# yatisht/usher

Measured on AMD Instinct MI355X. Metric: sample placements/sec on 10M-node MAT; bit-exact parsimony score vs reference, higher is better.
Workload: dtype u16 packed (4-bit allele sets, 4-bit SWAR node counters, 16-bit D/cost); 1 GPU; synthetic random MAT 10000000 nodes / 11429716 mutations / 25000 variable sites, L=29903; 16384 queries per GPU per step; nodes=10000000, queries_per_gpu=16384, queries_total=16384, tile=512, tiles=32, waves_per_tile=2050, query_sets_rotated=4, parallelism=queries sharded x1, MAT replicated, RCCL all-gather of results, rccl_ranks=1, devices_visible=1, seed=1

## Files before the change

include/usher_amd.h:

```cpp
#ifndef USHER_AMD_H
#define USHER_AMD_H

#include <stdint.h>

#ifdef __cplusplus
extern "C" {
#endif

#define UGP_OK               0
#define UGP_ERR_INVALID     -1
#define UGP_ERR_UNSUPPORTED -2
#define UGP_ERR_HIP         -3
#define UGP_ERR_NOMEM       -4

typedef struct ugp_mat ugp_mat;
typedef struct ugp_qset ugp_qset;

typedef struct ugp_tree_desc {
    uint64_t n_nodes;
    const uint32_t *parent;
    const uint64_t *mut_off;
    const int32_t *mut_pos;
    const uint8_t *mut_ref;
    const uint8_t *mut_par;
// ... 62 lines not shown
                   uint8_t *tie_has_unique ,
                   uint32_t *tie_count );

#define UGP_ORDER_BFS 0u
#define UGP_ORDER_DFS 1u
typedef struct ugp_place_opts {
    uint32_t order;
    const uint8_t *node_mask;
    const uint32_t *skip_node;
    const uint32_t *distance;
    int32_t *scores;
} ugp_place_opts;
int ugp_place_batch_ex(ugp_mat *mat, const ugp_queries *q, const ugp_place_opts *opts, ugp_result *out );
int ugp_tied_nodes_ex(ugp_mat *mat, const ugp_queries *q, const ugp_place_opts *opts, uint32_t cap, uint32_t *tie_j,
                      uint8_t *tie_has_unique, uint32_t *tie_count);
typedef struct ugp_ex ugp_ex;
int ugp_ex_prepare(ugp_mat *mat, const ugp_place_opts *opts, ugp_ex **out);
void ugp_ex_destroy(ugp_ex *ex);
int ugp_place_batch_prepared(ugp_mat *mat, const ugp_queries *q, const ugp_ex *ex, const uint32_t *skip_node, ugp_result *out ,
                             int32_t *d_scores );
int ugp_uncertainty_attach(ugp_mat *mat, const ugp_tree_desc *tree);
int ugp_uncertainty(ugp_mat *mat, const uint32_t *nodes , uint64_t n, uint32_t cap, uint32_t *epps, uint32_t *nsize,
                    uint32_t *tie_dfs , uint32_t *tie_count);
int ugp_annotate_attach(ugp_mat *mat, const ugp_tree_desc *tree);
int ugp_clade_alleles(ugp_mat *mat, const uint64_t *clade_off , const uint32_t *nodes , uint64_t n_clades,
                      uint64_t *out_off , uint32_t *out_ent, uint32_t *out_cnt, uint64_t cap, uint64_t *n_out);
int ugp_clade_descendants(ugp_mat *mat, const uint64_t *clade_off, const uint32_t *nodes , uint64_t n_clades,
                          const uint32_t *pair_clade, const uint32_t *pair_node , uint64_t n_pairs, uint32_t *out);
int ugp_annotate_search(ugp_mat *mat, const ugp_queries *q, uint32_t cap, int32_t *best , uint32_t *tie_dfs ,
                        uint32_t *tie_count );
typedef struct ugp_nearest_info {
    uint32_t count;
    uint32_t anc;
    uint32_t last_anc;
    uint32_t cut_dist;
    uint32_t n_at_cut;
} ugp_nearest_info;
int ugp_nearest_attach(ugp_mat *mat, const ugp_tree_desc *tree);
int ugp_nearest_k(ugp_mat *mat, uint64_t n_queries, const uint32_t *nodes , const uint32_t *k, uint32_t out_stride,
                  uint32_t *out_nodes , uint32_t *out_dist ,
                  ugp_nearest_info *info );
int ugp_nearest_k_chunked(ugp_mat *mat, uint64_t n_queries, const uint32_t *nodes, const uint32_t *k, uint32_t out_stride,
                          uint32_t *out_nodes, uint32_t *out_dist, ugp_nearest_info *info, uint32_t chunk_queries);
typedef struct ugp_gt_site {
    int32_t pos;
    uint8_t ref, n_alt;
    uint8_t alt[14];
    uint32_t ac[14];
    uint32_t covered;
} ugp_gt_site;
int ugp_genotypes_attach(ugp_mat *mat, const ugp_tree_desc *tree);
int ugp_genotype_select(ugp_mat *mat, const uint32_t *nodes , uint64_t n, uint32_t *n_cols, uint64_t *n_sites);
int ugp_genotype_columns(ugp_mat *mat, uint32_t *nodes );
int ugp_genotype_sites(ugp_mat *mat, uint64_t lo, uint64_t hi, ugp_gt_site *out );
int ugp_genotype_rows(ugp_mat *mat, uint64_t lo, uint64_t hi, uint8_t *codes );
int ugp_genotype_rows_chunked(ugp_mat *mat, uint64_t lo, uint64_t hi, uint8_t *codes, uint64_t chunk_cells);
int ugp_genotype_rows_time(ugp_mat *mat, uint64_t lo, uint64_t hi, uint32_t reps, double *ms);
typedef struct ugp_sm_mutation {
    int32_t pos;
    uint8_t par, nuc;
    uint8_t pad[2];
    uint32_t count;
} ugp_sm_mutation;
typedef struct ugp_sm_roho {
    uint32_t parent, child;
    uint32_t entry;
    uint32_t child_count;
    uint32_t offspring_with;
    uint32_t median_without;
} ugp_sm_roho;
int ugp_summary_attach(ugp_mat *mat, const ugp_tree_desc *tree);
int ugp_summary_mutations(ugp_mat *mat, ugp_sm_mutation *out, uint64_t cap, uint64_t *n_out);
int ugp_summary_mutations_chunked(ugp_mat *mat, ugp_sm_mutation *out, uint64_t cap, uint64_t *n_out, uint64_t chunk_items);
int ugp_summary_roho(ugp_mat *mat, ugp_sm_roho *out, uint64_t cap, uint64_t *n_out);
int ugp_summary_roho_chunked(ugp_mat *mat, ugp_sm_roho *out, uint64_t cap, uint64_t *n_out, uint64_t chunk_items);
int ugp_summary_clades(ugp_mat *mat, const uint64_t *col_off , const uint32_t *nodes , uint64_t n_cols,
                       uint32_t *incl , uint32_t *excl , uint32_t *leaf_clade );
int ugp_summary_time(ugp_mat *mat, uint32_t reps, double *sort_ms, double *roho_ms);
typedef struct ugp_tr_record {
    uint32_t node;
    uint32_t codon;
    uint8_t before[3], after[3];
    uint8_t pad[2];
    uint32_t ent[3];
} ugp_tr_record;
typedef struct ugp_tr_info {
    uint64_t n_records;
    uint64_t n_nodes;
    uint64_t n_inconsistent, n_duplicate;
    uint32_t first_inconsistent;
    uint32_t first_duplicate;
} ugp_tr_info;
int ugp_translate_attach(ugp_mat *mat, const ugp_tree_desc *tree);
int ugp_translate_codons(ugp_mat *mat, uint64_t n_codons, const int32_t *slot_pos , const uint8_t *slot_init );
int ugp_translate(ugp_mat *mat, ugp_tr_record *out, uint64_t cap, uint64_t *n_out, ugp_tr_info *info);
int ugp_translate_chunked(ugp_mat *mat, ugp_tr_record *out, uint64_t cap, uint64_t *n_out, ugp_tr_info *info, uint64_t chunk_items);
int ugp_translate_time(ugp_mat *mat, uint32_t reps, double *ms);
typedef struct ugp_ripples_opts {
    uint32_t branch_len;
    int32_t min_range, max_range;
    int32_t parsimony_improvement;
    uint32_t num_descendants;
} ugp_ripples_opts;
typedef struct ugp_ripples_event {
    uint64_t branch;
    uint32_t i, j;
    uint32_t donor, acceptor;
    uint32_t donor_count, acceptor_count;
    int32_t donor_score, acceptor_score;
    uint8_t donor_sibling, acceptor_sibling;
    uint8_t pad[6];
} ugp_ripples_event;
int ugp_ripples_attach(ugp_mat *mat, const ugp_tree_desc *tree, const uint32_t *name_rank);
int ugp_ripples(ugp_mat *mat, const ugp_ripples_opts *opts, const uint32_t *branches , uint64_t n, ugp_ripples_event *out,
                uint64_t cap, uint64_t *n_out);
int ugp_node_order(ugp_mat *mat, uint32_t order, uint32_t *bfs_of );
int ugp_subtree_mask(ugp_mat *mat, uint32_t order, uint32_t root_j, uint32_t max_levels, uint8_t *mask_out );

int ugp_qset_upload(ugp_mat *mat, const ugp_queries *q, ugp_qset **out);
void ugp_qset_destroy(ugp_qset *qs);
uint64_t ugp_qset_size(const ugp_qset *qs);
int ugp_place_device(ugp_mat *mat, ugp_qset *qs, void *d_out, void *stream);
int ugp_place_device_overlapped(ugp_mat *mat, ugp_qset *qs, void *d_out, void *stream);
int ugp_pipeline_depth(const ugp_mat *mat);

typedef struct ugp_job ugp_job;
int ugp_place_batch_async(ugp_mat *mat, const ugp_queries *q, ugp_result *out , ugp_job **job);
int ugp_job_wait(ugp_job *job);

#define UGP_T_LEAF   1u
#define UGP_T_MASKED 2u
typedef struct ugp_touched {
    uint64_t n;
    const uint32_t *flat_j;
    const uint8_t *flags;
    const uint32_t *n_path;
    const uint64_t *ent_off;
    const int32_t *pos;
    const uint8_t *allele;
    const uint8_t *prev;
    const uint8_t *ref;
} ugp_touched;
int ugp_mat_update(ugp_mat *mat, const ugp_touched *recs, const uint32_t *retired, uint64_t n_retired, uint32_t *first_id);
int ugp_touched_open(ugp_mat *mat, const ugp_queries *batch);
int ugp_touched_score(ugp_mat *mat, uint32_t first_id, uint64_t first_sample);
int ugp_touched_rescore(ugp_mat *mat, uint64_t sample);
int ugp_touched_fetch(ugp_mat *mat, uint64_t first_sample, uint64_t n, uint32_t cap, int32_t *best, uint32_t *count, uint32_t *ids,
                      uint8_t *has_unique);

int ugp_get_timing(ugp_mat *mat, ugp_timing *out);
int ugp_get_timing_sum(ugp_mat *mat, ugp_timing *sum, uint32_t *n_calls);

int ugp_debug_bound3_tables(ugp_mat *mat, uint32_t tile, uint16_t *over, uint16_t *under, uint64_t cap, uint64_t *n_blocks);

const char *ugp_last_error(void);

typedef struct ugp_sites {
    uint64_t n_sites;
    const uint8_t *ref;
    const uint64_t *var_off;
    const uint32_t *var_node;
    const uint8_t *var_nuc;
} ugp_sites;
typedef struct ugp_fitch ugp_fitch;

int ugp_fitch_sankoff(int device, uint64_t n_nodes, const uint32_t *parent, const ugp_sites *sites, ugp_fitch **out);
uint64_t ugp_fitch_count(const ugp_fitch *f);
int ugp_fitch_get(const ugp_fitch *f, uint32_t *site, uint32_t *node, uint8_t *par_nuc , uint8_t *mut_nuc );
void ugp_fitch_destroy(ugp_fitch *f);
void ugp_fitch_release(int device);


int ugp_mat_reload_knobs(ugp_mat *mat);
int ugp_has_experiments(void);

int ugp_mat_create_chunked(const ugp_tree_desc *tree, int device, uint32_t chunk_nodes, ugp_mat **out);

typedef struct ugp_flat ugp_flat;
enum {
    UGP_FLAT_STREAM = 0,
    UGP_FLAT_PRE_STREAM = 1,
    UGP_FLAT_CHUNK_BODY_OFF = 2,
    UGP_FLAT_CHUNK_PRE_OFF = 3,
    UGP_FLAT_CHUNK_NODE_OFF = 4,
    UGP_FLAT_POS2SITE = 5,
    UGP_FLAT_SITE_REF = 6,
    UGP_FLAT_RANK2BFS = 7,
    UGP_FLAT_DFS2BFS = 8,
    UGP_FLAT_MAX_SLOTS = 9,
    UGP_FLAT_STREAM8 = 10,
    UGP_FLAT_PRE8_STREAM = 11,
    UGP_FLAT_CHUNK8_BODY_OFF = 12,
    UGP_FLAT_CHUNK8_PRE_OFF = 13,
    UGP_FLAT_MAX_PATH_MUTS = 14,
    UGP_FLAT_STREAM_T = 15,
    UGP_FLAT_CHUNK_T_OFF = 16,
    UGP_FLAT_LDS_SLOTS = 17,
    UGP_FLAT_B3_GROUP_OFF = 18,
    UGP_FLAT_B3_EVENTS = 19
};
int ugp_flat_create(const ugp_tree_desc *tree, uint32_t chunk_nodes, ugp_flat **out);
void ugp_flat_destroy(ugp_flat *flat);
int ugp_flat_get(const ugp_flat *flat, int which, const void **ptr, uint64_t *count);

#ifdef __cplusplus
}
#endif
#endif
```

usher_amd/_lib.py:

```python
from __future__ import annotations

import ctypes as C
import os
import subprocess

_HERE = os.path.dirname(os.path.abspath(__file__))
LIB_PATH = os.path.join(_HERE, "libusher_amd.so")
EXP_LIB_PATH = os.path.join(_HERE, "libusher_amd_exp.so")
_lib = None
_lib_exp = None


class ugp_tree_desc(C.Structure):
    _fields_ = [("n_nodes", C.c_uint64), ("parent", C.c_void_p), ("mut_off", C.c_void_p), ("mut_pos", C.c_void_p),
                ("mut_ref", C.c_void_p), ("mut_par", C.c_void_p), ("mut_nuc", C.c_void_p)]


class ugp_ripples_opts(C.Structure):
    _fields_ = [("branch_len", C.c_uint32), ("min_range", C.c_int32), ("max_range", C.c_int32),
                ("parsimony_improvement", C.c_int32), ("num_descendants", C.c_uint32)]


class ugp_queries(C.Structure):
    _fields_ = [("n_queries", C.c_uint64), ("ent_off", C.c_void_p), ("pos", C.c_void_p), ("ref", C.c_void_p),
                ("nuc", C.c_void_p), ("is_missing", C.c_void_p)]


class ugp_result(C.Structure):
    _fields_ = [("best_set_difference", C.c_int32), ("num_best", C.c_uint32), ("best_j", C.c_uint32),
                ("best_has_unique", C.c_uint32)]


class ugp_info(C.Structure):
    _fields_ = [("n_nodes", C.c_uint64), ("n_muts", C.c_uint64), ("n_sites", C.c_uint64), ("stream_bytes", C.c_uint64),
                ("algo_tree_bytes", C.c_uint64), ("algo_tile_bytes", C.c_uint64), ("n_chunks", C.c_uint32),
                ("max_slots", C.c_uint32), ("max_position", C.c_uint32), ("device", C.c_uint32)]


class ugp_timing(C.Structure):
    _fields_ = [("table_ms", C.c_float), ("place_ms", C.c_float), ("merge_ms", C.c_float),
                ("place_launches", C.c_uint32), ("n_tiles", C.c_uint32), ("n_groups", C.c_uint32), ("packed_path", C.c_uint32),
                ("reserved", C.c_uint32), ("words_total", C.c_uint64), ("words_skipped", C.c_uint64), ("coarse_ms", C.c_float), ("bound3", C.c_uint32)]


class ugp_place_opts(C.Structure):
    _fields_ = [("order", C.c_uint32), ("node_mask", C.c_void_p), ("skip_node", C.c_void_p), ("distance", C.c_void_p), ("scores", C.c_void_p)]


class ugp_touched(C.Structure):
    _fields_ = [("n", C.c_uint64), ("flat_j", C.c_void_p), ("flags", C.c_void_p), ("n_path", C.c_void_p), ("ent_off", C.c_void_p), ("pos", C.c_void_p),
                ("allele", C.c_void_p), ("prev", C.c_void_p), ("ref", C.c_void_p)]


class ugp_sites(C.Structure):
    _fields_ = [("n_sites", C.c_uint64), ("ref", C.c_void_p), ("var_off", C.c_void_p), ("var_node", C.c_void_p),
                ("var_nuc", C.c_void_p)]


P = C.c_void_p
SYMBOLS = {
    "ugp_mat_create": (C.c_int, [C.POINTER(ugp_tree_desc), C.c_int, C.POINTER(P)]),
    "ugp_mat_create_multi": (C.c_int, [C.POINTER(ugp_tree_desc), C.POINTER(C.c_int), C.c_int, C.POINTER(P)]),
    "ugp_flat_save": (C.c_int, [C.POINTER(ugp_tree_desc), C.c_char_p]),
    "ugp_mat_create_from_flat": (C.c_int, [C.c_char_p, C.c_int, C.POINTER(P)]),
    "ugp_mat_destroy": (None, [P]),
    "ugp_mat_info": (C.c_int, [P, C.POINTER(ugp_info)]),
    "ugp_place_batch": (C.c_int, [P, C.POINTER(ugp_queries), P]),
    "ugp_scores_per_node": (C.c_int, [P, C.POINTER(ugp_queries), P]),
    "ugp_tied_nodes": (C.c_int, [P, C.POINTER(ugp_queries), C.c_uint32, P, P, P]),
    "ugp_place_batch_ex": (C.c_int, [P, C.POINTER(ugp_queries), C.POINTER(ugp_place_opts), P]),
    "ugp_tied_nodes_ex": (C.c_int, [P, C.POINTER(ugp_queries), C.POINTER(ugp_place_opts), C.c_uint32, P, P, P]),
    "ugp_ex_prepare": (C.c_int, [P, C.POINTER(ugp_place_opts), C.POINTER(P)]),
    "ugp_ex_destroy": (None, [P]),
    "ugp_place_batch_prepared": (C.c_int, [P, C.POINTER(ugp_queries), P, P, P, P]),
    "ugp_device_warmup": (C.c_int, [C.c_int]),
    "ugp_node_order": (C.c_int, [P, C.c_uint32, P]),
    "ugp_uncertainty_attach": (C.c_int, [P, C.POINTER(ugp_tree_desc)]),
    "ugp_uncertainty": (C.c_int, [P, P, C.c_uint64, C.c_uint32, P, P, P, P]),
    "ugp_annotate_attach": (C.c_int, [P, C.POINTER(ugp_tree_desc)]),
    "ugp_clade_alleles": (C.c_int, [P, P, P, C.c_uint64, P, P, P, C.c_uint64, C.POINTER(C.c_uint64)]),
    "ugp_clade_descendants": (C.c_int, [P, P, P, C.c_uint64, P, P, C.c_uint64, P]),
    "ugp_annotate_search": (C.c_int, [P, C.POINTER(ugp_queries), C.c_uint32, P, P, P]),
    "ugp_nearest_attach": (C.c_int, [P, C.POINTER(ugp_tree_desc)]),
    "ugp_nearest_k": (C.c_int, [P, C.c_uint64, P, P, C.c_uint32, P, P, P]),
    "ugp_nearest_k_chunked": (C.c_int, [P, C.c_uint64, P, P, C.c_uint32, P, P, P, C.c_uint32]),
    "ugp_genotypes_attach": (C.c_int, [P, C.POINTER(ugp_tree_desc)]),
    "ugp_genotype_select": (C.c_int, [P, P, C.c_uint64, P, P]),
    "ugp_genotype_columns": (C.c_int, [P, P]),
    "ugp_genotype_sites": (C.c_int, [P, C.c_uint64, C.c_uint64, P]),
    "ugp_genotype_rows": (C.c_int, [P, C.c_uint64, C.c_uint64, P]),
    "ugp_genotype_rows_chunked": (C.c_int, [P, C.c_uint64, C.c_uint64, P, C.c_uint64]),
    "ugp_genotype_rows_time": (C.c_int, [P, C.c_uint64, C.c_uint64, C.c_uint32, P]),
    "ugp_summary_attach": (C.c_int, [P, C.POINTER(ugp_tree_desc)]),
    "ugp_summary_mutations": (C.c_int, [P, P, C.c_uint64, C.POINTER(C.c_uint64)]),
    "ugp_summary_mutations_chunked": (C.c_int, [P, P, C.c_uint64, C.POINTER(C.c_uint64), C.c_uint64]),
    "ugp_summary_roho": (C.c_int, [P, P, C.c_uint64, C.POINTER(C.c_uint64)]),
    "ugp_summary_roho_chunked": (C.c_int, [P, P, C.c_uint64, C.POINTER(C.c_uint64), C.c_uint64]),
    "ugp_summary_clades": (C.c_int, [P, P, P, C.c_uint64, P, P, P]),
    "ugp_summary_time": (C.c_int, [P, C.c_uint32, P, P]),
    "ugp_translate_attach": (C.c_int, [P, C.POINTER(ugp_tree_desc)]),
    "ugp_translate_codons": (C.c_int, [P, C.c_uint64, P, P]),
    "ugp_translate": (C.c_int, [P, P, C.c_uint64, C.POINTER(C.c_uint64), P]),
    "ugp_translate_chunked": (C.c_int, [P, P, C.c_uint64, C.POINTER(C.c_uint64), P, C.c_uint64]),
    "ugp_translate_time": (C.c_int, [P, C.c_uint32, P]),
    "ugp_ripples_attach": (C.c_int, [P, C.POINTER(ugp_tree_desc), P]),
    "ugp_ripples": (C.c_int, [P, C.POINTER(ugp_ripples_opts), P, C.c_uint64, P, C.c_uint64, C.POINTER(C.c_uint64)]),
    "ugp_subtree_mask": (C.c_int, [P, C.c_uint32, C.c_uint32, C.c_uint32, P]),
    "ugp_qset_upload": (C.c_int, [P, C.POINTER(ugp_queries), C.POINTER(P)]),
    "ugp_qset_destroy": (None, [P]),
    "ugp_qset_size": (C.c_uint64, [P]),
    "ugp_place_device": (C.c_int, [P, P, P, P]),
    "ugp_place_device_overlapped": (C.c_int, [P, P, P, P]),
    "ugp_pipeline_depth": (C.c_int, [P]),
    "ugp_mat_update": (C.c_int, [P, C.POINTER(ugp_touched), P, C.c_uint64, C.POINTER(C.c_uint32)]),
    "ugp_touched_open": (C.c_int, [P, C.POINTER(ugp_queries)]),
    "ugp_touched_score": (C.c_int, [P, C.c_uint32, C.c_uint64]),
    "ugp_touched_rescore": (C.c_int, [P, C.c_uint64]),
    "ugp_touched_fetch": (C.c_int, [P, C.c_uint64, C.c_uint64, C.c_uint32, P, P, P, P]),
    "ugp_mat_reload_knobs": (C.c_int, [P]),
    "ugp_has_experiments": (C.c_int, []),
    "ugp_place_batch_async": (C.c_int, [P, C.POINTER(ugp_queries), P, C.POINTER(P)]),
    "ugp_job_wait": (C.c_int, [P]),
    "ugp_get_timing": (C.c_int, [P, C.POINTER(ugp_timing)]),
    "ugp_get_timing_sum": (C.c_int, [P, C.POINTER(ugp_timing), C.POINTER(C.c_uint32)]),
    "ugp_debug_bound3_tables": (C.c_int, [P, C.c_uint32, P, P, C.c_uint64, C.POINTER(C.c_uint64)]),
    "ugp_last_error": (C.c_char_p, []),
    "ugp_fitch_sankoff": (C.c_int, [C.c_int, C.c_uint64, P, C.POINTER(ugp_sites), C.POINTER(P)]),
    "ugp_fitch_count": (C.c_uint64, [P]),
    "ugp_fitch_get": (C.c_int, [P, P, P, P, P]),
    "ugp_fitch_destroy": (None, [P]),
    "ugp_fitch_release": (None, [C.c_int]),
    "ugp_mat_create_chunked": (C.c_int, [C.POINTER(ugp_tree_desc), C.c_int, C.c_uint32, C.POINTER(P)]),
    "ugp_flat_create": (C.c_int, [C.POINTER(ugp_tree_desc), C.c_uint32, C.POINTER(P)]),
    "ugp_flat_destroy": (None, [P]),
    "ugp_flat_get": (C.c_int, [P, C.c_int, C.POINTER(P), C.POINTER(C.c_uint64)]),
}


def build_library(force: bool = False) -> str:
    csrc = os.path.join(_HERE, "csrc")
    cmd = ["make", "-s", "-C", csrc]
    if force:
        cmd.append("-B")
    subprocess.check_call(cmd)
    return LIB_PATH


def _load(path):
    if not os.path.exists(path):
        raise RuntimeError(
            "%s is not built (%s); run `python -c 'import __graft_entry__ as g; g.build()'` "
            "or `make -C usher_amd/csrc`. There is no CPU fallback." % (os.path.basename(path), path))
    L = C.CDLL(path)
    for name, (res, args) in SYMBOLS.items():
        fn = getattr(L, name)
        fn.restype = res
        fn.argtypes = args
    return L


def lib(experiments: bool = False):
    global _lib, _lib_exp
    if experiments:
        if _lib_exp is None:
            _lib_exp = _load(EXP_LIB_PATH)
        return _lib_exp
    if _lib is None:
        _lib = _load(os.environ.get("USHER_AMD_LIB") or LIB_PATH)
    return _lib
```

usher_amd/csrc/ugp_capi.cpp:

```cpp
#include <hip/hip_runtime.h>

#include <algorithm>
#include <atomic>
#include <climits>
#include <chrono>
#include <cstdio>
#include <cstdlib>
#include <cstring>
#include <new>
#include <string>
#include <thread>
#include <mutex>
#include <vector>

#include <unistd.h>

#include "ugp_bound3.hpp"
#include "ugp_dense.hpp"
#include "ugp_tuner.hpp"
#include "ugp_plan.hpp"
#include "ugp_flatten.hpp"
#include "ugp_kernels.hpp"
#include "ugp_knobs.hpp"
#include "ugp_ripples.hpp"
#include "ugp_uncertainty.hpp"
#include "ugp_annotate.hpp"
#include "ugp_nearest.hpp"
#include "ugp_genotypes.hpp"
#include "ugp_summary.hpp"
#include "ugp_translate.hpp"
#include "ugp_update.hpp"
#include "usher_amd.h"

namespace {

thread_local std::string g_err;

int fail(int code, const std::string &msg) {
    g_err = msg;
    return code;
}

#define HIP_TRY(expr)                                                                         \
    do {                                                                                      \
        hipError_t e_ = (expr);                                                               \
        if (e_ != hipSuccess)                                                                 \
            return fail(UGP_ERR_HIP, std::string(#expr) + ": " + hipGetErrorString(e_));      \
    } while (0)

}

namespace ugp {
int set_error(int code, const std::string &msg) { return fail(code, msg); }
}

namespace {

template <typename T>
struct DevBuf {
    T *p = nullptr;
    size_t cap = 0;
    ~DevBuf() { release(); }
    void release() {
        if (p) (void)hipFree(p);
        p = nullptr; cap = 0;
    }
    hipError_t reserve(size_t n) {
        if (n <= cap) return hipSuccess;
        release();
        hipError_t e = hipMalloc((void **)&p, std::max<size_t>(n, 1) * sizeof(T));
        if (e == hipSuccess) cap = n; else p = nullptr;
        return e;
    }
    hipError_t grow_keep(size_t n, size_t used) {
        if (n <= cap) return hipSuccess;
        const size_t want = std::max<size_t>(n, cap * 2);
        T *np = nullptr;
        hipError_t e = hipMalloc((void **)&np, std::max<size_t>(want, 1) * sizeof(T));
        if (e != hipSuccess) return e;
        if (p && used) e = hipMemcpy(np, p, used * sizeof(T), hipMemcpyDeviceToDevice);
        if (e != hipSuccess) { (void)hipFree(np); return e; }
        if (p) (void)hipFree(p);
        p = np; cap = want;
        return hipSuccess;
    }
    template <class V>
    hipError_t upload(const V &v) {
        hipError_t e = reserve(v.size());
        if (e != hipSuccess || v.empty()) return e;
        return hipMemcpy(p, v.data(), v.size() * sizeof(T), hipMemcpyHostToDevice);
    }
};

struct PinBuf {
    void *p = nullptr;
    size_t cap = 0;
    ~PinBuf() { if (p) (void)hipHostFree(p); }
    int reserve(size_t n, bool device_writes = false) {
        if (n <= cap) return UGP_OK;
        if (p) (void)hipHostFree(p);
        p = nullptr; cap = 0;
        if (hipHostMalloc(&p, std::max<size_t>(n, 1), device_writes ? (hipHostMallocMapped | hipHostMallocCoherent) : hipHostMallocDefault) != hipSuccess) { p = nullptr; return fail(UGP_ERR_HIP, "hipHostMalloc (staging buffer)"); }
        cap = n;
        return UGP_OK;
    }
};

int copy_d2h_staged(void *dst, const void *src, size_t bytes) {
    constexpr size_t kPiece = 32u << 20;
    if (bytes < 4 * kPiece) {
        if (bytes && hipMemcpy(dst, src, bytes, hipMemcpyDeviceToHost) != hipSuccess) return fail(UGP_ERR_HIP, "copy to the host");
        return UGP_OK;
    }
    PinBuf pin[2];
    hipStream_t st = nullptr;
    hipEvent_t ev[2] = {nullptr, nullptr};
    int rc = UGP_OK;
    if (pin[0].reserve(kPiece) != UGP_OK || pin[1].reserve(kPiece) != UGP_OK) return UGP_ERR_HIP;
    if (hipStreamCreateWithFlags(&st, hipStreamNonBlocking) != hipSuccess || hipEventCreateWithFlags(&ev[0], hipEventDisableTiming) != hipSuccess ||
        hipEventCreateWithFlags(&ev[1], hipEventDisableTiming) != hipSuccess) rc = fail(UGP_ERR_HIP, "staged copy: stream / events");
    const size_t n_pieces = (bytes + kPiece - 1) / kPiece;
    const unsigned n_thr = std::max(1u, std::min(8u, std::thread::hardware_concurrency() / 2));
    auto drain = [&](size_t i) {
        const size_t off = i * kPiece, n = std::min(kPiece, bytes - off);
        const char *from = (const char *)pin[i & 1].p;
        char *to = (char *)dst + off;
        std::vector<std::thread> th;
        const size_t per = ((n + n_thr - 1) / n_thr + 4095) & ~(size_t)4095;
        for (unsigned t = 1; t < n_thr; t++)
            if ((size_t)t * per < n) th.emplace_back([=]() { memcpy(to + (size_t)t * per, from + (size_t)t * per, std::min(per, n - (size_t)t * per)); });
        memcpy(to, from, std::min(per, n));
        for (auto &x : th) x.join();
    };
    for (size_t i = 0; i <= n_pieces && rc == UGP_OK; i++) {
        if (i < n_pieces) {
            const size_t off = i * kPiece, n = std::min(kPiece, bytes - off);
            if (hipMemcpyAsync(pin[i & 1].p, (const char *)src + off, n, hipMemcpyDeviceToHost, st) != hipSuccess || hipEventRecord(ev[i & 1], st) != hipSuccess)
                rc = fail(UGP_ERR_HIP, "staged copy: hipMemcpyAsync");
        }
        if (i > 0 && rc == UGP_OK) {
            if (hipEventSynchronize(ev[(i - 1) & 1]) != hipSuccess) rc = fail(UGP_ERR_HIP, "staged copy: wait");
            else drain(i - 1);
        }
    }
    if (st) { (void)hipStreamSynchronize(st); (void)hipStreamDestroy(st); }
    for (auto e : ev) if (e) (void)hipEventDestroy(e);
    return rc;
}

struct EventSet {
    hipEvent_t ev[4] = {nullptr, nullptr, nullptr, nullptr};
    bool used = false;
    int b3_class = -1;
    bool b3_used = false;
    uint32_t b3_tiles = 0, b3_pos = 0;
    bool b3_first = false;
    uint64_t b3_seq = 0;
};

using ugp::B3Tuner;

using ugp::kMaxSets;

}

struct ugp_mat {
    int device = 0;
    ugp::Knobs knobs;
    ugp::FlatMat flat;
    uint64_t stream_dwords = 0, pre_dwords = 0;
    DevBuf<uint32_t> d_stream, d_pre, d_chunk_body, d_chunk_pre, d_chunk_node, d_rank2bfs, d_dfs2bfs;
    DevBuf<uint32_t> d_stream8, d_pre8, d_chunk8_body, d_chunk8_pre, d_stream_t, d_chunk_t;
    DevBuf<uint32_t> d_node_pos8, d_rank_dfs;
    DevBuf<uint32_t> d_b3_group_off, d_b3_events;
    uint64_t stream8_dwords = 0;
    DevBuf<int32_t> d_pos2site, d_site_pos;
    DevBuf<uint8_t> d_site_ref;
    ugp_mat *coarse = nullptr;
    DevBuf<uint32_t> d_coarse2bfs, d_node_pair, d_parent;
    bool wide_descent = false;
    DevBuf<uint32_t> d_coarse2dfs, d_coarse_bin;
    uint32_t n_coarse_bins = 0;
    std::vector<uint32_t> h_level_off;
    uint32_t max_level_width = 0;
    std::vector<uint32_t> h_parent, h_dfs2bfs, h_bfs2dfs, h_leaves;
    std::vector<uint32_t> h_flat_chunk_node;
    std::vector<uint32_t> h_flat_bfs2dfs;
    DevBuf<uint32_t> d_dfs2bfs_caller;
    DevBuf<uint32_t> d_dfs_rank, d_dfs_rank2out, d_bfs2dfs;
    bool dfs_rank_ready = false;
    ugp_qset *own_qs = nullptr;
    DevBuf<ugp_result> d_own_out;
    size_t occ_lds = ~(size_t)0;
    int occ_per_cu = 0, n_cu = 0, occ_variant = -1;
    struct Work {
        DevBuf<uint32_t> d_table, d_zero, d_part_best, d_part_cnt, d_part_key;
        DevBuf<uint32_t> d_lpos;
        DevBuf<uint32_t> d_tie_units, d_tie_info;
        DevBuf<uint32_t> d_lbest, d_gbest, d_gbest_part, d_items, d_ub, d_gstart, d_hlen, d_cold, d_list, d_units, d_unit_info;
        DevBuf<uint64_t> d_dyn;
        uint32_t dyn_epoch = 0;
        DevBuf<uint32_t> d_b3_pairmask;
        DevBuf<uint8_t> d_b3_over, d_b3_under, d_b3_l1, d_b3_l2, d_b3_l3;
        DevBuf<ugp::B3Dev> d_b3_dev;
        ugp::B3Dev b3_host = {};
        DevBuf<uint64_t> d_stats, d_trace;
        uint64_t last_words_total = 0;
        const uint32_t *last_nitems = nullptr;
        const uint32_t *last_list_n = nullptr;
        uint32_t last_list_tiles = 0;
        DevBuf<uint32_t> d_dnode, d_dres, d_luniq, d_gcnt, d_gcnt_part;
        DevBuf<uint32_t> d_refined, d_keys, d_keys2, d_idx, d_order, d_slot, d_bins;
        DevBuf<ugp_result> d_coarse_res, d_prev_res;
        uint64_t prev_serial = 0;
        DevBuf<uint8_t> d_sort_tmp;
        bool last_used_best8 = false;
        struct Gen {
            std::vector<EventSet> events;
            hipEvent_t ev_coarse[2] = {nullptr, nullptr};
            bool coarse_timed = false;
            size_t events_used = 0;
            ugp_timing last = {};
            bool timing_pending = false;
        } gens[4];
        uint32_t cur = 0;
        ugp_qset *job_qs = nullptr;
        DevBuf<ugp_result> d_job_out;
        PinBuf job_in, job_out;
        bool job_busy = false;
        hipStream_t aux = nullptr;
        hipEvent_t ev_fork = nullptr, ev_fill = nullptr, ev_join = nullptr;
        bool join_pending = false;
        hipStream_t stream = nullptr;
        hipEvent_t done = nullptr;
        hipStream_t done_on = nullptr;
    } work[kMaxSets];
    ugp_timing tsum = {};
    uint32_t tsum_calls = 0;
    int last_work = 0;
    B3Tuner b3_tuner;
    int next_work = 0;
    int next_job = 0;
    uint64_t n_overlapped = 0;
    hipEvent_t entry_ring[kMaxSets] = {};
    int share_sets = 2;
    int share_n = 1;
    uint32_t tie_lists_filled = 0, tie_sub_batches = 0;
    bool sharing = false;
    bool was_busy = false;
    int was_n = 1;
    struct Upd {
        std::vector<uint32_t> hdr8, rec, post, coarse2bfs, excluded_j;
        DevBuf<uint32_t> d_hdr8, d_rec_pos, d_post;
        DevBuf<ugp::TouchedRec> d_rec;
        DevBuf<ugp::TouchedEnt> d_ent;
        DevBuf<uint8_t> d_alive;
        DevBuf<uint32_t> d_tmp;
        uint64_t n_rec = 0, n_ent = 0, n_excluded = 0;
        ugp_qset *qs = nullptr;
        DevBuf<uint8_t> d_dense, d_hu;
        DevBuf<int32_t> d_dbot, d_best, d_list_best;
        DevBuf<uint32_t> d_cnt, d_ids;
        uint32_t n_pos = 0, qpad = 0;
        uint64_t Q = 0;
        bool open = false;
        PinBuf stage_up;
        PinBuf stage;
    } upd;
    ugp::UncState *unc = nullptr;
    ugp::RipState *rip = nullptr;
    ugp::AnnState *ann = nullptr;
    ugp::NearState *near = nullptr;
    ugp::GtState *gt = nullptr;
    ugp::SmState *sm = nullptr;
    ugp::TrState *tr = nullptr;
    ugp::DfsTables *dfs = nullptr;
    hipEvent_t kb_done = nullptr;
    hipStream_t kb_done_on = nullptr;
};

struct ugp_qset {
    int device = 0;
    uint64_t n_queries = 0, n_ent = 0;
    uint64_t max_rows = 0;
    uint64_t serial = 0;
    DevBuf<int32_t> d_pos;
    DevBuf<uint8_t> d_ref, d_nuc, d_missing;
    DevBuf<uint32_t> d_ent_q;
    DevBuf<uint64_t> d_ent_off;
    DevBuf<unsigned long long> d_err;
    DevBuf<uint32_t> d_nmask[2], d_plain_rows, d_n_plain;
    const ugp_mat *nmask_for[2] = {nullptr, nullptr};
    uint32_t nmask_words[2] = {0, 0};
    std::vector<uint64_t> ent_off;
};

namespace ugp { void fitch_drop_streams(int device); }
namespace {

int validate_offsets(const ugp_queries *q, uint64_t &n_ent, uint64_t &max_rows) {
    if (!q || (q->n_queries && !q->ent_off)) return fail(UGP_ERR_INVALID, "null query arrays");
    if (q->n_queries >= (1ull << 31)) return fail(UGP_ERR_UNSUPPORTED, "more than 2^31 queries in one batch");
    n_ent = q->n_queries ? q->ent_off[q->n_queries] : 0;
    if (n_ent && (!q->pos || !q->ref || !q->nuc || !q->is_missing)) return fail(UGP_ERR_INVALID, "null query entry arrays");
    max_rows = 0;
    for (uint64_t s = 0; s < q->n_queries; s++) {
        const uint64_t b = q->ent_off[s], e = q->ent_off[s + 1];
        if (e < b || e > n_ent) return fail(UGP_ERR_INVALID, "ent_off is not monotone");
        max_rows = std::max(max_rows, e - b);
    }
    if (q->n_queries && q->ent_off[0] != 0) return fail(UGP_ERR_INVALID, "ent_off[0] must be 0");
    return UGP_OK;
}

}
static int harvest_timing(ugp_mat *m, ugp_mat::Work &W, ugp_mat::Work::Gen &G);
static void tuner_poll(ugp_mat *m);
namespace {
int ensure_events(ugp_mat::Work::Gen &G, size_t n) {
    while (G.events.size() < n) {
        EventSet es;
        for (int i = 0; i < 4; i++) HIP_TRY(hipEventCreate(&es.ev[i]));
        G.events.push_back(es);
    }
    return UGP_OK;
}

struct ExDev {
    const uint8_t *mask = nullptr; const uint32_t *skip = nullptr, *alt_rank = nullptr, *out_index = nullptr, *rank2out = nullptr;
    const uint32_t *skip_chunk = nullptr;
    int32_t *scores = nullptr;
    bool packed = false;
};

struct PlaceReq {
    int mode = 0;
    ugp_result *out = nullptr;
    int32_t *scores = nullptr;
    const int32_t *best_in = nullptr;
    uint32_t *tie_count = nullptr, *tie_j = nullptr;
    uint8_t *tie_hu = nullptr;
    uint32_t tie_cap = 0;
    hipStream_t stream = nullptr;
    bool coarse_only = false;
    const ExDev *ex = nullptr;
    int wi = 0;
};

struct Finish {
    ugp_mat::Work &W; hipStream_t s;
    ~Finish() {
        if (W.join_pending) { (void)hipStreamWaitEvent(s, W.ev_join, 0); W.join_pending = false; }
        if (!W.done && hipEventCreateWithFlags(&W.done, hipEventDisableTiming) != hipSuccess) { W.done = nullptr; return; }
        (void)hipEventRecord(W.done, s);
        W.done_on = s;
    }
};

struct PlaceCall {
    ugp_mat *m; ugp_qset *qs; const PlaceReq &r;
    ugp_mat::Work &W;
    hipStream_t s;
    ugp_mat::Work::Gen *TG;
    ugp::PlanTree tree;
    ugp::PlanCall call;
    ugp::CallPlan cp;
    const uint32_t *ex_skip;
};

struct SubBatch {
    uint64_t q0 = 0, nq = 0, e0 = 0, e1 = 0;
    ugp::SubPlan p;
    ugp::ZeroLayout z;
    uint64_t table_dwords = 0, pairs = 0;
    EventSet *es = nullptr;
    uint32_t *d_dbottom = nullptr, *d_active = nullptr, *d_queue = nullptr, *d_list_n = nullptr, *d_nitems = nullptr, *d_cnt = nullptr, *d_key = nullptr,
             *d_useful = nullptr;
    const uint32_t *slot_of = nullptr, *order = nullptr;
    ugp::Phase2Uniq uq{};
    ugp::PlaceArgs a;
    ugp::Best8Args b8;
    uint32_t blocks = 0;
};

int nmask_index(const ugp_qset *qs, const ugp_mat *m) {
    int nmi = -1;
    for (int i = 0; i < 2; i++) if (qs->nmask_for[i] == m) nmi = i;
    return nmi;
}

ugp::PlanTree plan_tree(const ugp_mat *m) {
    const auto &f = m->flat;
    ugp::PlanTree t;
    t.n_nodes = f.n_nodes; t.n_sites = f.n_sites; t.n_chunks = f.n_chunks; t.max_chunk8_words = f.max_chunk8_words;
    t.max_path_muts = f.max_path_muts; t.lds_slots = f.lds_slots; t.mask_not_first = f.mask_not_first;
    t.coarse = m->coarse != nullptr; t.b3_events = m->d_b3_events.p != nullptr; t.wide_descent = m->wide_descent;
    return t;
}

ugp::PlanCall plan_call_facts(const ugp_mat *m, const ugp_qset *qs, const PlaceReq &r) {
    ugp::PlanCall c;
    c.Q = qs->n_queries; c.max_rows = qs->max_rows; c.mode = r.mode; c.coarse_only = r.coarse_only; c.ties = r.tie_count != nullptr;
    c.nmask = nmask_index(qs, m) >= 0; c.sharing = m->sharing; c.share_sets = m->share_sets;
    if (const ExDev *ex = r.ex) {
        c.ex.given = true; c.ex.packed = ex->packed; c.ex.mask = ex->mask != nullptr; c.ex.skip = ex->skip != nullptr;
        c.ex.skip_chunk = ex->skip_chunk != nullptr; c.ex.scores = ex->scores != nullptr;
    }
    return c;
}

int run_place(ugp_mat *m, ugp_qset *qs, const PlaceReq &r);

int open_timing(PlaceCall &c) {
    ugp_mat::Work &W = c.W;
    W.cur = (W.cur + 1u) & 3u;
    c.TG = &W.gens[W.cur];
    if (int rc = harvest_timing(c.m, W, *c.TG)) return rc;
    c.TG->events_used = 0;
    c.TG->last = {};
    c.TG->timing_pending = true;
    return UGP_OK;
}

int side_fill(PlaceCall &c) {
    ugp_mat::Work &W = c.W;
    if (!c.cp.can_fork) return UGP_OK;
    if (!W.aux) {
        HIP_TRY(hipStreamCreateWithFlags(&W.aux, hipStreamNonBlocking));
        HIP_TRY(hipEventCreateWithFlags(&W.ev_fork, hipEventDisableTiming)); HIP_TRY(hipEventCreateWithFlags(&W.ev_fill, hipEventDisableTiming));
        HIP_TRY(hipEventCreateWithFlags(&W.ev_join, hipEventDisableTiming));
    }
    if (!c.cp.fill_ahead) return UGP_OK;
    const uint64_t dw = (uint64_t)((c.call.Q + 511) / 512) * (c.cp.n_sites + ugp::TABLE_CONST_ROWS) * 64;
    HIP_TRY(W.d_table.reserve(dw));
    HIP_TRY(hipEventRecord(W.ev_fork, c.s));
    HIP_TRY(hipStreamWaitEvent(W.aux, W.ev_fork, 0));
    HIP_TRY(ugp::launch_fill_table(W.d_table.p, c.m->d_site_ref.p, c.cp.n_sites, dw, W.aux));
    HIP_TRY(hipEventRecord(W.ev_fill, W.aux));
    return UGP_OK;
}

int coarse_pass(PlaceCall &c) {
    ugp_mat *m = c.m;
    ugp_mat::Work &W = c.W;
    ugp_mat::Work::Gen &TG = *c.TG;
    HIP_TRY(W.d_coarse_res.reserve(c.call.Q));
    if (!TG.ev_coarse[0]) { HIP_TRY(hipEventCreate(&TG.ev_coarse[0])); HIP_TRY(hipEventCreate(&TG.ev_coarse[1])); }
    HIP_TRY(hipEventRecord(TG.ev_coarse[0], c.s));
    m->coarse->sharing = m->sharing; m->coarse->share_n = m->share_n; m->coarse->share_sets = m->share_sets;
    PlaceReq cr;
    cr.out = W.d_coarse_res.p; cr.stream = c.s; cr.wi = c.r.wi;
    cr.coarse_only = m->coarse->d_node_pos8.p && m->coarse->flat.max_chunk8_words < 65536u && !m->knobs.coarse_phase2;
    if (int rc = run_place(m->coarse, c.qs, cr)) return rc;
    HIP_TRY(hipSetDevice(m->device));
    HIP_TRY(hipEventRecord(TG.ev_coarse[1], c.s));
    TG.coarse_timed = true;
    return UGP_OK;
}

int sub_begin(PlaceCall &c, SubBatch &sb, uint64_t q0) {
    ugp_mat *m = c.m;
    ugp_mat::Work &W = c.W;
    ugp_mat::Work::Gen &TG = *c.TG;
    const auto &f = m->flat;
    sb.q0 = q0; sb.nq = std::min<uint64_t>(c.call.Q - q0, c.cp.sub_tiles * 64);
    if (c.r.mode == 0 && c.r.tie_count) m->tie_sub_batches++;
    sb.e0 = c.qs->ent_off[q0]; sb.e1 = c.qs->ent_off[q0 + sb.nq];
    sb.p = ugp::plan_sub(c.tree, m->knobs, c.call, c.cp, sb.nq, sb.e1 - sb.e0);
    const uint32_t n_tiles512 = sb.p.n_tiles512;
    sb.table_dwords = (uint64_t)n_tiles512 * (c.cp.n_sites + ugp::TABLE_CONST_ROWS) * 64;
    HIP_TRY(W.d_table.reserve(sb.table_dwords));
    uint32_t b3_pos = 0;
    uint64_t b3_seq = 0;
    if (sb.p.b3_tuned) { tuner_poll(m); sb.p.b3_want = m->b3_tuner.next(sb.p.b3_class, &b3_pos, &b3_seq); }
    sb.pairs = (uint64_t)f.n_chunks * n_tiles512 * 8;
    sb.z = ugp::zero_layout(n_tiles512, c.cp.active_words, c.cp.useful_words, sb.p.b3_want);
    HIP_TRY(W.d_zero.reserve(sb.z.z_end));
    sb.d_dbottom = W.d_zero.p + sb.z.z_dbottom; sb.d_active = W.d_zero.p + sb.z.z_active; sb.d_queue = W.d_zero.p + sb.z.z_queue;
    sb.d_list_n = W.d_zero.p + sb.z.z_list_n; sb.d_nitems = W.d_zero.p + sb.z.z_nitems; sb.d_cnt = W.d_zero.p + sb.z.z_cnt;
    sb.d_key = W.d_zero.p + sb.z.z_key; sb.d_useful = sb.p.b3_want ? W.d_zero.p + sb.z.z_useful : nullptr;
    if (c.cp.packed_ok) {
        HIP_TRY(W.d_lbest.reserve((size_t)f.n_chunks * n_tiles512 * 256));
        HIP_TRY(W.d_list.reserve((size_t)f.n_chunks * n_tiles512));
        HIP_TRY(W.d_ub.reserve((size_t)n_tiles512 * 256));
        if (!c.r.coarse_only) {
            HIP_TRY(W.d_gbest.reserve((size_t)n_tiles512 * 256));
            HIP_TRY(W.d_gbest_part.reserve((size_t)ugp::GBEST_SLICES * n_tiles512 * 256));
            HIP_TRY(W.d_items.reserve(sb.pairs));
        }
    } else if (c.r.mode == 0) {
        const size_t np = (size_t)sb.p.n_tiles * sb.p.G * 64;
        HIP_TRY(W.d_part_best.reserve(np));
        HIP_TRY(W.d_part_cnt.reserve(np));
        HIP_TRY(W.d_part_key.reserve(np));
    }
    if (int rc = ensure_events(TG, TG.events_used + 1)) return rc;
    EventSet &es = TG.events[TG.events_used++];
    sb.es = &es;
    es.b3_class = -1;
    es.b3_used = sb.p.b3_want; es.b3_tiles = n_tiles512; es.b3_pos = b3_pos; es.b3_seq = b3_seq; es.b3_first = m->b3_tuner.first;
    HIP_TRY(hipEventRecord(es.ev[0], c.s));
    return UGP_OK;
}

int locality_sort(PlaceCall &c, SubBatch &sb) {
    ugp_mat *m = c.m;
    ugp_mat::Work &W = c.W;
    const uint64_t nq = sb.nq;
    HIP_TRY(W.d_keys.reserve(nq)); HIP_TRY(W.d_keys2.reserve(nq)); HIP_TRY(W.d_idx.reserve(nq));
    HIP_TRY(W.d_order.reserve(nq)); HIP_TRY(W.d_slot.reserve(nq)); HIP_TRY(W.d_bins.reserve(std::max<uint32_t>(m->n_coarse_bins, 1)));
    size_t tmp_bytes = 0;
    HIP_TRY(ugp::launch_locality_sort(nullptr, nullptr, (uint32_t)nq, W.d_keys.p, W.d_keys2.p, W.d_idx.p, W.d_order.p,
                                      W.d_slot.p, nullptr, &tmp_bytes, nullptr, 0, nullptr, c.s));
    HIP_TRY(W.d_sort_tmp.reserve(tmp_bytes));
    HIP_TRY(ugp::launch_locality_sort(W.d_coarse_res.p + sb.q0, m->d_coarse2dfs.p, (uint32_t)nq, W.d_keys.p, W.d_keys2.p,
                                      W.d_idx.p, W.d_order.p, W.d_slot.p, W.d_sort_tmp.p, &tmp_bytes, m->knobs.radix_sort ? nullptr : m->d_coarse_bin.p, m->n_coarse_bins, W.d_bins.p, c.s));
    sb.slot_of = W.d_slot.p; sb.order = W.d_order.p;
    return UGP_OK;
}

int build_tiles(PlaceCall &c, SubBatch &sb) {
    ugp_mat *m = c.m;
    ugp_qset *qs = c.qs;
    ugp_mat::Work &W = c.W;
    hipStream_t s = c.s;
    const auto &f = m->flat;
    const uint32_t n_sites = c.cp.n_sites, active_words = c.cp.active_words, useful_words = c.cp.useful_words, n_tiles512 = sb.p.n_tiles512;
    const uint32_t q0 = (uint32_t)sb.q0, nq = (uint32_t)sb.nq;
    HIP_TRY(hipMemsetAsync(W.d_zero.p, 0, sb.z.z_end * sizeof(uint32_t), s));
    if (sb.p.nmask) {
        const int nmi = nmask_index(qs, m);
        HIP_TRY(ugp::launch_ntiles(W.d_table.p, sb.d_active, active_words, n_tiles512, qs->d_nmask[nmi].p, qs->nmask_words[nmi], sb.order, q0, nq,
                                   m->d_site_ref.p, n_sites, s));
        HIP_TRY(ugp::launch_scatter_list(W.d_table.p, sb.d_dbottom, qs->d_pos.p, qs->d_ref.p, qs->d_nuc.p, qs->d_missing.p, qs->d_ent_q.p, m->d_pos2site.p,
                                         f.max_pos, n_sites, q0, nq, sb.d_active, active_words, sb.slot_of, qs->d_plain_rows.p, qs->d_n_plain.p, qs->d_err.p,
                                         sb.d_useful, useful_words, s));
    } else if (sb.p.lds_build)
        HIP_TRY(ugp::launch_build_tiles(W.d_table.p, sb.d_active, active_words, n_tiles512, qs->d_ent_off.p, q0, sb.order, nq, qs->d_pos.p,
                                        qs->d_ref.p, qs->d_nuc.p, qs->d_missing.p, m->d_pos2site.p, m->d_site_pos.p, m->d_site_ref.p, n_sites, f.max_pos,
                                        sb.d_dbottom, qs->d_err.p, s));
    else {
        const uint64_t e0 = sb.e0, e1 = sb.e1;
        if (c.cp.fill_ahead && sb.q0 == 0) HIP_TRY(hipStreamWaitEvent(s, W.ev_fill, 0));
        else HIP_TRY(ugp::launch_fill_table(W.d_table.p, m->d_site_ref.p, n_sites, sb.table_dwords, s));
        HIP_TRY(ugp::launch_scatter(W.d_table.p, sb.d_dbottom, qs->d_pos.p + e0, qs->d_ref.p + e0,
                                    qs->d_nuc.p + e0, qs->d_missing.p + e0, qs->d_ent_q.p + e0, m->d_pos2site.p,
                                    f.max_pos, n_sites, e1 - e0, q0, sb.d_active, active_words, sb.slot_of, qs->d_err.p, sb.d_useful, useful_words, s));
    }
    return UGP_OK;
}

int b3_tables(PlaceCall &c, SubBatch &sb) {
    ugp_mat *m = c.m;
    ugp_mat::Work &W = c.W;
    hipStream_t s = c.s;
    const uint32_t n_sites = c.cp.n_sites, n_tiles512 = sb.p.n_tiles512;
    const uint32_t nb = ugp::b3_blocks(m->stream8_dwords), n_l1 = ugp::b3_div64(nb), n_l2 = ugp::b3_div64(n_l1), n_l3 = ugp::b3_div64(n_l2);
    HIP_TRY(W.d_b3_pairmask.reserve((size_t)((n_tiles512 + 31) / 32) * n_sites * 4));
    HIP_TRY(W.d_b3_over.reserve((size_t)n_tiles512 * nb)); HIP_TRY(W.d_b3_under.reserve((size_t)n_tiles512 * nb));
    HIP_TRY(W.d_b3_l1.reserve((size_t)n_tiles512 * n_l1)); HIP_TRY(W.d_b3_l2.reserve((size_t)n_tiles512 * n_l2)); HIP_TRY(W.d_b3_l3.reserve((size_t)n_tiles512 * n_l3));
    HIP_TRY(W.d_b3_dev.reserve(1));
    const ugp::B3Dev hd{W.d_b3_over.p, W.d_b3_under.p, W.d_b3_l1.p, W.d_b3_l2.p, W.d_b3_l3.p, nb, n_l1, n_l2, n_l3};
    if (memcmp(&hd, &W.b3_host, sizeof hd) != 0) {
        HIP_TRY(hipStreamSynchronize(s));
        HIP_TRY(hipMemcpy(W.d_b3_dev.p, &hd, sizeof hd, hipMemcpyHostToDevice));
        W.b3_host = hd;
    }
    hipStream_t on = s;
    if (c.cp.can_fork) {
        HIP_TRY(hipEventRecord(W.ev_fork, s));
        HIP_TRY(hipStreamWaitEvent(W.aux, W.ev_fork, 0));
        on = W.aux;
    }
    HIP_TRY(ugp::launch_b3_tables(sb.d_useful, c.cp.useful_words, n_sites, n_tiles512, m->d_b3_group_off.p, m->d_b3_events.p, nb, W.d_b3_pairmask.p,
                                  W.d_b3_over.p, W.d_b3_under.p, W.d_b3_l1.p, W.d_b3_l2.p, W.d_b3_l3.p, on));
    if (c.cp.can_fork) { HIP_TRY(hipEventRecord(W.ev_join, W.aux)); W.join_pending = true; }
    return UGP_OK;
}

#ifdef UGP_EXPERIMENTS
int seed_check_report(PlaceCall &c, SubBatch &sb) {
    ugp_mat *m = c.m;
    ugp_mat::Work &W = c.W;
    const uint64_t nq = sb.nq, q0 = sb.q0;
    std::vector<uint32_t> ref(nq), ord(nq);
    std::vector<ugp_result> prev(nq), coarse(nq);
    HIP_TRY(hipStreamSynchronize(c.s));
    HIP_TRY(hipMemcpy(ref.data(), W.d_refined.p, nq * 4, hipMemcpyDeviceToHost));
    HIP_TRY(hipMemcpy(ord.data(), sb.order, nq * 4, hipMemcpyDeviceToHost));
    HIP_TRY(hipMemcpy(prev.data(), W.d_prev_res.p + q0, nq * sizeof(ugp_result), hipMemcpyDeviceToHost));
    HIP_TRY(hipMemcpy(coarse.data(), W.d_coarse_res.p + q0, nq * sizeof(ugp_result), hipMemcpyDeviceToHost));
    uint64_t hist_r[18] = {0}, hist_c[18] = {0}, miss_anc = 0, miss_other = 0, miss_depth = 0;
    std::vector<uint32_t> c2b(m->coarse ? m->coarse->flat.n_nodes : 0);
    if (!c2b.empty()) HIP_TRY(hipMemcpy(c2b.data(), m->d_coarse2bfs.p, c2b.size() * 4, hipMemcpyDeviceToHost));
    for (uint64_t k = 0; k < nq; k++) {
        const int exact = prev[ord[k]].best_set_difference;
        hist_r[std::min(17, std::max(0, (int)ref[k] - exact))]++;
        hist_c[std::min(17, std::max(0, coarse[ord[k]].best_set_difference - exact))]++;
        if ((int)ref[k] > exact && !c2b.empty() && coarse[ord[k]].best_j < c2b.size()) {
            const uint32_t j0 = c2b[coarse[ord[k]].best_j];
            uint32_t x = prev[ord[k]].best_j, depth = 0;
            while (x != UINT32_MAX && x != j0 && x != 0) { x = m->h_parent[x]; depth++; }
            if (x == j0) { miss_anc++; miss_depth += depth; } else {
                miss_other++;
                if (miss_other <= 12) {
                    auto depth_of = [&](uint32_t v) { uint32_t d = 0; while (v != 0 && v != UINT32_MAX) { v = m->h_parent[v]; d++; } return d; };
                    uint32_t a = j0, b = prev[ord[k]].best_j;
// ... 116 lines not shown
    }
    b.ub_every = w.ub_every;
    b.freeze_ub = c.ex_skip ? 1u : 0u;
    b.refill_all_rows = K.refill_all ? 1u : 0u;
    b.heavy_prio = K.heavy_prio;
    b.no_pre_records = w.no_pre_records;
    HIP_TRY(W.d_units.reserve((size_t)n_tiles512 * w.per_tile_cap * 4));
    HIP_TRY(W.d_unit_info.reserve(32 + 96));
    constexpr uint32_t kDynCap = 1u << 17;
    if (!W.d_dyn.p) {
        HIP_TRY(W.d_dyn.reserve(kDynCap));
        W.dyn_epoch = 2047;
    }
    if (++W.dyn_epoch >= 2048u) { HIP_TRY(hipMemsetAsync(W.d_dyn.p, 0, (size_t)kDynCap * 8, s)); W.dyn_epoch = 1; }
    uint32_t *dyn_ctl = W.d_unit_info.p + 32;
    b.dyn_ctl = dyn_ctl; b.dyn_units = (unsigned long long *)W.d_dyn.p; b.dyn_cap = kDynCap; b.dyn_epoch = W.dyn_epoch;
    b.split_cycles = w.split_cycles; b.split_heavy = w.split_heavy; b.split_dense = w.split_dense; b.split_many = w.split_many;
    HIP_TRY(ugp::launch_build_units(hstart, hlen, n_tiles512, f.n_chunks, w.unit_chunks, w.heavy_chunks, w.grow_every, w.unit_max, w.light_order, w.per_tile_cap,
                                    W.d_units.p, W.d_unit_info.p, W.d_unit_info.p + 8, dyn_ctl, s));
    b.units = (const uint4 *)W.d_units.p; b.unit_base = W.d_unit_info.p; b.unit_count = W.d_unit_info.p + 8;
    HIP_TRY(W.d_stats.reserve(96));
    if (sb.q0 == 0) { if (K.stats) HIP_TRY(hipMemsetAsync(W.d_stats.p, 0, 96 * sizeof(uint64_t), s)); W.last_words_total = 0; }
    b.stats = K.stats ? W.d_stats.p : nullptr;
    if (b.stats && !K.trace.empty() && !coarse_only) {
        constexpr size_t kTraceCap = 1u << 20;
        HIP_TRY(W.d_trace.reserve(8 + kTraceCap * 6));
        HIP_TRY(hipMemsetAsync(W.d_trace.p, 0, 64, s));
        b.trace = W.d_trace.p; b.trace_cap = kTraceCap;
    }
    W.last_words_total += (uint64_t)n_tiles512 * m->stream8_dwords;
    b.max_slots = f.max_slots;
    b.lds_slots = f.lds_slots;
    b.lds_bits = w.lds_bits;
    b.b3 = w.b3 ? W.d_b3_dev.p : nullptr;
    if (b.b3) c.TG->last.bound3 = 1;
    if (m->occ_lds != w.lds_bytes || m->occ_variant != w.variant) {
        HIP_TRY(hipDeviceGetAttribute(&m->n_cu, hipDeviceAttributeMultiprocessorCount, m->device));
        HIP_TRY(ugp::best8_occupancy(w.lds_bytes, w.variant, &m->occ_per_cu));
        m->occ_lds = w.lds_bytes; m->occ_variant = w.variant;
    }
    const uint64_t blocks = ugp::plan_grid(c.tree, K, c.call, c.cp, sb.p, m->occ_per_cu, m->n_cu).blocks;
    sb.blocks = (uint32_t)blocks;
    HIP_TRY(W.d_cold.reserve((size_t)blocks * std::max<uint32_t>(f.max_slots - b.lds_slots, 1) * 512));
    b.cold = W.d_cold.p;
    b.active = sb.d_active; b.active_words = c.cp.active_words;
    const bool exclusive = K.kbest_exclusive;
    if (exclusive && !coarse_only && m->kb_done && m->kb_done_on != s) HIP_TRY(hipStreamWaitEvent(s, m->kb_done, 0));
    if (W.join_pending) { HIP_TRY(hipStreamWaitEvent(s, W.ev_join, 0)); W.join_pending = false; }
    HIP_TRY(ugp::launch_best8(b, (uint32_t)blocks, s));
    if (exclusive && !coarse_only) {
        if (!m->kb_done) HIP_TRY(hipEventCreateWithFlags(&m->kb_done, hipEventDisableTiming));
        HIP_TRY(hipEventRecord(m->kb_done, s));
        m->kb_done_on = s;
    }
    HIP_TRY(hipEventRecord(sb.es->ev[2], s));
    return UGP_OK;
}

int packed_result(PlaceCall &c, SubBatch &sb) {
    ugp_mat *m = c.m;
    ugp_mat::Work &W = c.W;
    hipStream_t s = c.s;
    const PlaceReq &r = c.r;
    const auto &f = m->flat;
    const uint32_t n_tiles512 = sb.p.n_tiles512;
    const uint64_t q0 = sb.q0, nq = sb.nq;
    if (c.ex_skip && !r.coarse_only)
        HIP_TRY(ugp::launch_fix_skip(sb.a, W.d_lbest.p, r.ex->skip_chunk + q0, n_tiles512, m->d_rank2bfs.p, sb.order, f.max_slots, s));
    if (r.coarse_only)
        HIP_TRY(ugp::launch_coarse_result(W.d_lbest.p, W.d_lpos.p, W.d_list.p, sb.d_list_n, f.n_chunks, n_tiles512, (uint32_t)nq, m->d_chunk_node.p,
                                          m->d_chunk8_body.p, m->d_node_pos8.p, m->d_dfs2bfs.p, r.out + q0, s));
#ifdef UGP_EXPERIMENTS
    else if (!r.tie_count && m->d_node_pos8.p && m->d_rank_dfs.p && sb.b8.ub && !sb.b8.stats && m->knobs.phase2_packed) {
        HIP_TRY(W.d_tie_units.reserve((size_t)((n_tiles512 + 7) / 8) * 8 * f.n_chunks * 4));
        HIP_TRY(W.d_tie_info.reserve(128));
        HIP_TRY(ugp::launch_phase2_packed(sb.b8, W.d_list.p, sb.d_list_n, W.d_gbest_part.p, W.d_gbest.p, n_tiles512, W.d_tie_units.p, W.d_tie_info.p, sb.d_cnt, sb.d_key,
                                          m->d_node_pos8.p, m->d_rank_dfs.p, m->d_chunk_node.p, m->d_rank2bfs.p, (uint32_t)nq, r.out + q0, sb.order,
                                          sb.blocks, s));
    }
#endif
    else
        HIP_TRY(ugp::launch_phase2(sb.a, W.d_lbest.p, W.d_list.p, sb.d_list_n, W.d_gbest_part.p, W.d_gbest.p, n_tiles512, W.d_items.p, sb.d_nitems,
                                   (uint32_t)std::min<uint64_t>(sb.pairs, 0xFFFFFFFFull), sb.d_cnt, sb.d_key,
                                   m->d_rank2bfs.p, r.ex ? r.ex->rank2out : nullptr, r.out + q0, sb.order, f.max_slots, r.tie_count != nullptr,
                                   sb.uq.luniq ? &sb.uq : nullptr, s));
    if (r.tie_count) m->tie_lists_filled++;
    return UGP_OK;
}

int level_scores(PlaceCall &c, SubBatch &sb) {
    ugp_mat *m = c.m;
    ugp_mat::Work &W = c.W;
    const auto &f = m->flat;
    const uint64_t nq = sb.nq;
    const uint32_t qpad = (uint32_t)((nq + 7) / 8 * 8);
    const bool d16 = c.qs->max_rows + f.max_path_muts + 2 < 0xFFFFull;
    const size_t d_words = ((size_t)m->max_level_width * ((qpad + ugp::SCORES_SB - 1) / ugp::SCORES_SB * ugp::SCORES_SB) * (d16 ? 2 : 4) + 3) / 4;
    HIP_TRY(W.d_part_best.reserve(d_words)); HIP_TRY(W.d_part_cnt.reserve(d_words));
    HIP_TRY(ugp::launch_scores_levels(m->d_node_pair.p, m->d_parent.p, m->d_stream.p, W.d_table.p, c.cp.n_sites, sb.d_dbottom, m->h_level_off.data(),
                                      (uint32_t)m->h_level_off.size() - 1, W.d_part_best.p, W.d_part_cnt.p, d16, m->max_level_width, qpad, (uint32_t)nq, f.n_nodes,
                                      sb.a.scores, m->knobs.scores_block, c.s));
    HIP_TRY(hipEventRecord(sb.es->ev[2], c.s));
    return UGP_OK;
}

int lane_walk(PlaceCall &c, SubBatch &sb) {
    ugp_mat *m = c.m;
    ugp_mat::Work &W = c.W;
    const PlaceReq &r = c.r;
    HIP_TRY(ugp::launch_place(sb.a, r.ex ? r.mode + 4 : r.mode, m->flat.max_slots, c.s));
    HIP_TRY(hipEventRecord(sb.es->ev[2], c.s));
    if (r.mode == 0)
        HIP_TRY(ugp::launch_merge(W.d_part_best.p, W.d_part_cnt.p, W.d_part_key.p, (r.ex && r.ex->rank2out) ? r.ex->rank2out : m->d_rank2bfs.p, sb.p.G,
                                  (uint32_t)sb.nq, r.out + sb.q0, c.s));
    return UGP_OK;
}

int sub_end(PlaceCall &c, SubBatch &sb) {
    ugp_mat *m = c.m;
    ugp_mat::Work &W = c.W;
    ugp_mat::Work::Gen &TG = *c.TG;
    const ugp::Knobs &K = m->knobs;
    const bool packed = c.cp.packed_ok;
    if ((K.seed_prev || K.seed_check) && packed && !c.r.coarse_only && c.r.mode == 0) {
        HIP_TRY(W.d_prev_res.reserve(c.call.Q));
        HIP_TRY(hipMemcpyAsync(W.d_prev_res.p + sb.q0, c.r.out + sb.q0, sb.nq * sizeof(ugp_result), hipMemcpyDeviceToDevice, c.s));
        W.prev_serial = (sb.q0 + sb.nq >= c.call.Q) ? c.qs->serial : 0;
    }
    HIP_TRY(hipEventRecord(sb.es->ev[3], c.s));
    if (sb.p.b3_tuned) sb.es->b3_class = sb.p.b3_class;
    W.last_used_best8 = packed;
    TG.last.packed_path = packed ? 1u : 0u;
    sb.es->used = true;
    TG.last.place_launches++;
    TG.last.n_tiles += packed ? sb.p.n_tiles512 : sb.p.n_tiles;
    TG.last.n_groups = sb.p.G;
    return UGP_OK;
}

int run_place(ugp_mat *m, ugp_qset *qs, const PlaceReq &r) {
    HIP_TRY(hipSetDevice(m->device));
    hipStream_t s = r.stream;
    PlaceCall c{m, qs, r, m->work[r.wi], s, nullptr, {}, {}, {}, nullptr};
    m->last_work = r.wi;
    if (c.W.done && c.W.done_on != s) HIP_TRY(hipStreamWaitEvent(s, c.W.done, 0));
    Finish finish{c.W, s};
    if (int rc = open_timing(c)) return rc;
    if (qs->n_queries == 0) return UGP_OK;
    c.tree = plan_tree(m);
    c.call = plan_call_facts(m, qs, r);
    c.cp = ugp::plan_call(c.tree, m->knobs, c.call);
    c.ex_skip = c.cp.ex_skip ? r.ex->skip : nullptr;
    c.TG->coarse_timed = false;
    if (int rc = side_fill(c)) return rc;
    if (c.cp.sorted) if (int rc = coarse_pass(c)) return rc;
    for (uint64_t q0 = 0; q0 < c.call.Q; q0 += c.cp.sub_tiles * 64) {
        SubBatch sb;
        if (int rc = sub_begin(c, sb, q0)) return rc;
        if (c.cp.sorted) if (int rc = locality_sort(c, sb)) return rc;
        if (int rc = build_tiles(c, sb)) return rc;
        if (sb.p.b3_want) if (int rc = b3_tables(c, sb)) return rc;
        if (c.cp.packed_ok) if (int rc = seed_bounds(c, sb)) return rc;
        HIP_TRY(hipEventRecord(sb.es->ev[1], s));
        place_args(c, sb);
        if (c.cp.packed_ok) {
            if (int rc = packed_walk(c, sb)) return rc;
            if (int rc = packed_result(c, sb)) return rc;
        } else if (r.mode == 1 && !r.ex && !m->h_level_off.empty() && !m->knobs.scores_dfs) {
            if (int rc = level_scores(c, sb)) return rc;
        } else if (int rc = lane_walk(c, sb)) return rc;
        if (int rc = sub_end(c, sb)) return rc;
    }
    return UGP_OK;
}

}

extern "C" {

const char *ugp_last_error(void) { return g_err.c_str(); }

int ugp_device_warmup(int device) {
    HIP_TRY(hipSetDevice(device));
    HIP_TRY(hipFree(nullptr));
    return UGP_OK;
}

struct HostFlat {
    ugp::FlatMat f;
    std::vector<uint32_t> parent;
    std::vector<uint32_t> coarse2dfs, coarse2bfs;
    ugp::UVec<uint32_t> node_pair;
    bool wide_descent = false;
    HostFlat *coarse = nullptr;
    ~HostFlat() { delete coarse; }
};

static int host_flatten(const ugp_tree_desc *tree, const ugp::Options &opt, bool with_coarse, HostFlat &hf);

static int build_coarse(const ugp_tree_desc *t, const ugp::Options &opt, ugp::FlatExtras &ex, HostFlat &hf) {
    const uint64_t N = t->n_nodes;
    uint64_t min_nodes = 1u << 18;
    if (const char *e = getenv("UGP_COARSE_MIN_NODES")) min_nodes = (uint64_t)atoll(e);
    if (N < min_nodes || N < 64 || getenv("UGP_NO_SORT")) return UGP_OK;
    const uint32_t *sub = ex.sub.data();
    uint64_t div = 4096;
    if (const char *e = getenv("UGP_COARSE_DIV")) div = (uint64_t)std::max(2, atoi(e));
    uint64_t floor_n = 4096;
    if (const char *e = getenv("UGP_COARSE_FLOOR")) floor_n = (uint64_t)std::max(16, atoi(e));
    const uint64_t target = std::min<uint64_t>(N / 2, std::max<uint64_t>(N / div, std::min<uint64_t>(floor_n, N / 4)));
    uint32_t S = 0;
    {
        constexpr uint32_t CAP = 1u << 16;
        const ugp::Par par = ugp::flatten_par(opt);
        std::vector<uint64_t> hist((size_t)par.T * (CAP + 1), 0);
        par.run(N, [&](uint64_t b, uint64_t e, unsigned tid) {
            uint64_t *h = &hist[(size_t)tid * (CAP + 1)];
            for (uint64_t j = b; j < e; j++) h[std::min<uint32_t>(sub[j], CAP)]++;
        }, 1u << 16);
        uint64_t below = 0;
        uint32_t v = 0;
        for (; v < CAP; v++) {
            uint64_t c = 0;
            for (unsigned th = 0; th < par.T; th++) c += hist[(size_t)th * (CAP + 1) + v];
            if (below + c > N - target) break;
            below += c;
        }
        if (v < CAP) S = v;
        else {
            std::vector<uint32_t> sorted_sub(sub, sub + N);
            std::nth_element(sorted_sub.begin(), sorted_sub.begin() + (N - target), sorted_sub.end());
            S = sorted_sub[N - target];
        }
        S = std::max<uint32_t>(2, S);
    }
    std::vector<uint32_t> keep;
    for (uint64_t j = 0; j < N; j++) if (sub[j] >= S || j == 0) keep.push_back((uint32_t)j);
    std::vector<uint32_t> parent(keep.size());
    std::vector<uint64_t> mut_off(keep.size() + 1, 0);
    std::vector<int32_t> pos; std::vector<uint8_t> ref, par, nuc;
    for (size_t k = 0; k < keep.size(); k++) {
        const uint32_t j = keep[k];
        parent[k] = j ? (uint32_t)(std::lower_bound(keep.begin(), keep.begin() + k, t->parent[j]) - keep.begin()) : UINT32_MAX;
        for (uint64_t i = t->mut_off[j]; i < t->mut_off[j + 1]; i++) {
            pos.push_back(t->mut_pos[i]); ref.push_back(t->mut_ref[i]);
            par.push_back(t->mut_par ? t->mut_par[i] : 0); nuc.push_back(t->mut_nuc[i]);
        }
        mut_off[k + 1] = pos.size();
    }
    ugp_tree_desc d{keep.size(), parent.data(), mut_off.data(), pos.data(), ref.data(), par.data(), nuc.data()};
    ugp::Options copt;
    copt.chunk_nodes = 256;
    copt.keep_node_pos8 = true;
    copt.keep_update_maps = opt.keep_update_maps;
    copt.keep_b3_events = false;
    if (const char *e = getenv("UGP_LDS_SLOTS")) copt.lds_slots = (uint32_t)std::max(1, std::min(60, atoi(e)));
    if (const char *e = getenv("UGP_COARSE_CHUNK_NODES")) copt.chunk_nodes = (uint32_t)std::max(1, atoi(e));
    hf.coarse = new HostFlat();
    if (int rc = host_flatten(&d, copt, false, *hf.coarse)) return rc;
    hf.coarse2dfs.resize(keep.size());
    for (size_t k = 0; k < keep.size(); k++) hf.coarse2dfs[k] = ex.dfsidx[keep[k]];
    hf.coarse2bfs = keep;
    return UGP_OK;
}

static int host_flatten(const ugp_tree_desc *tree, const ugp::Options &opt, bool with_coarse, HostFlat &hf) {
    std::string err;
    int rc;
    try {
        ugp::FlatExtras ex;
        rc = ugp::flatten(*tree, opt, hf.f, err, with_coarse ? &ex : nullptr);
        if (rc == UGP_OK && with_coarse) hf.parent.assign(tree->parent, tree->parent + tree->n_nodes);
        if (rc == UGP_OK && with_coarse) {
            rc = build_coarse(tree, opt, ex, hf);
            if (rc != UGP_OK) return rc;
            hf.node_pair.swap(ex.node_pair);
            if (hf.coarse) hf.wide_descent = ex.children_of_wide_nodes * 20 > tree->n_nodes;
        }
    } catch (const std::bad_alloc &) {
        return fail(UGP_ERR_NOMEM, "out of host memory while flattening the tree");
    }
    if (rc != UGP_OK) return fail(rc, err);
    return UGP_OK;
}

static int upload_flat(const HostFlat &hf, int device, ugp_mat **out) {
    *out = nullptr;
    ugp_mat *m = new (std::nothrow) ugp_mat();
    if (!m) return fail(UGP_ERR_NOMEM, "out of host memory");
    m->device = device;
    m->knobs = ugp::Knobs::from_env();
    auto bail = [&](hipError_t e, const char *what) {
        std::string msg = std::string(what) + ": " + hipGetErrorString(e);
        ugp_mat_destroy(m);
        return fail(UGP_ERR_HIP, msg);
    };
    hipError_t e;
    if ((e = hipSetDevice(device)) != hipSuccess) return bail(e, "hipSetDevice");
    const auto &f = hf.f;
    {
        auto &g = m->flat;
        g.n_nodes = f.n_nodes; g.n_muts = f.n_muts; g.n_sites = f.n_sites; g.max_pos = f.max_pos; g.max_slots = f.max_slots;
        g.n_chunks = f.n_chunks; g.max_path_muts = f.max_path_muts; g.max_chunk8_words = f.max_chunk8_words; g.mask_not_first = f.mask_not_first; g.lds_slots = f.lds_slots;
    }
    m->upd.hdr8.assign(f.hdr8_of_bfs.begin(), f.hdr8_of_bfs.end());
    m->upd.rec.assign(f.rec_of_bfs.begin(), f.rec_of_bfs.end());
    m->upd.post.assign(f.post_of_bfs.begin(), f.post_of_bfs.end());
    m->upd.coarse2bfs = hf.coarse2bfs;
    if ((e = m->d_stream.upload(f.stream)) != hipSuccess) return bail(e, "upload stream");
    if ((e = m->d_pre.upload(f.pre_stream)) != hipSuccess) return bail(e, "upload preambles");
    if ((e = m->d_chunk_body.upload(f.chunk_body_off)) != hipSuccess) return bail(e, "upload chunk table");
    if ((e = m->d_chunk_pre.upload(f.chunk_pre_off)) != hipSuccess) return bail(e, "upload chunk table");
    if ((e = m->d_chunk_node.upload(f.chunk_node_off)) != hipSuccess) return bail(e, "upload chunk table");
    if ((e = m->d_rank2bfs.upload(f.rank2bfs)) != hipSuccess) return bail(e, "upload rank table");
    if ((e = m->d_dfs2bfs.upload(f.dfs2bfs)) != hipSuccess) return bail(e, "upload dfs table");
    if ((e = m->d_pos2site.upload(f.pos2site)) != hipSuccess) return bail(e, "upload site table");
    {
        std::vector<int32_t> sp(std::max<size_t>(f.n_sites, 1), 0);
        for (size_t p = 0; p < f.pos2site.size(); p++) if (f.pos2site[p] >= 0) sp[(size_t)f.pos2site[p]] = (int32_t)p;
        if ((e = m->d_site_pos.upload(sp)) != hipSuccess) return bail(e, "upload site table");
    }
    {
        std::vector<uint8_t> sr(f.site_ref);
        if (sr.empty()) sr.push_back(1);
        if ((e = m->d_site_ref.upload(sr)) != hipSuccess) return bail(e, "upload site table");
    }
    if ((e = m->d_stream8.upload(f.stream8)) != hipSuccess) return bail(e, "upload packed stream");
    if ((e = m->d_pre8.upload(f.pre8_stream)) != hipSuccess) return bail(e, "upload packed preambles");
    if ((e = m->d_chunk8_body.upload(f.chunk8_body_off)) != hipSuccess) return bail(e, "upload chunk table");
    if ((e = m->d_chunk8_pre.upload(f.chunk8_pre_off)) != hipSuccess) return bail(e, "upload chunk table");
    if ((e = m->d_stream_t.upload(f.stream_t)) != hipSuccess) return bail(e, "upload tie stream");
    if ((e = m->d_chunk_t.upload(f.chunk_t_off)) != hipSuccess) return bail(e, "upload chunk table");
    if (!f.node_pos8.empty() && (e = m->d_node_pos8.upload(f.node_pos8)) != hipSuccess) return bail(e, "upload node positions");
    if (!f.rank_dfs.empty() && (e = m->d_rank_dfs.upload(f.rank_dfs)) != hipSuccess) return bail(e, "upload node ranks");
    if (!f.b3_events.empty()) {
        if ((e = m->d_b3_group_off.upload(f.b3_group_off)) != hipSuccess) return bail(e, "upload event lists");
        if ((e = m->d_b3_events.upload(f.b3_events)) != hipSuccess) return bail(e, "upload event lists");
    }
    m->stream8_dwords = f.stream8.size();
    m->stream_dwords = f.stream.size();
    m->pre_dwords = f.pre_stream.size();
    m->h_parent = hf.parent;
    if (!hf.node_pair.empty()) {
        if ((e = m->d_node_pair.upload(hf.node_pair)) != hipSuccess) return bail(e, "upload node table");
        if ((e = m->d_parent.upload(hf.parent)) != hipSuccess) return bail(e, "upload parent table");
        const uint64_t N = f.n_nodes;
        std::vector<uint32_t> level(N, 0);
        m->h_level_off.assign(1, 0);
        for (uint64_t j = 1; j < N; j++) {
            level[j] = level[hf.parent[j]] + 1;
            if (level[j] != level[j - 1]) m->h_level_off.push_back((uint32_t)j);
        }
        m->h_level_off.push_back((uint32_t)N);
        m->max_level_width = 0;
        for (size_t l = 0; l + 1 < m->h_level_off.size(); l++) m->max_level_width = std::max(m->max_level_width, m->h_level_off[l + 1] - m->h_level_off[l]);
    }
    if (hf.coarse) {
        if (int rc = upload_flat(*hf.coarse, device, &m->coarse)) { ugp_mat_destroy(m); return rc; }
        if ((e = m->d_coarse2dfs.upload(hf.coarse2dfs)) != hipSuccess) return bail(e, "upload coarse table");
        {
            std::vector<uint32_t> by_rank(hf.coarse2dfs.size()), bin(hf.coarse2dfs.size());
            for (uint32_t i = 0; i < by_rank.size(); i++) by_rank[i] = i;
            std::sort(by_rank.begin(), by_rank.end(), [&](uint32_t a, uint32_t b) { return hf.coarse2dfs[a] < hf.coarse2dfs[b]; });
            for (uint32_t i = 0; i < by_rank.size(); i++) bin[by_rank[i]] = i;
            if ((e = m->d_coarse_bin.upload(bin)) != hipSuccess) return bail(e, "upload coarse table");
            m->n_coarse_bins = (uint32_t)bin.size();
        }
        if ((e = m->d_coarse2bfs.upload(hf.coarse2bfs)) != hipSuccess) return bail(e, "upload coarse table");
        if (!hf.node_pair.empty()) {
            m->wide_descent = getenv("UGP_DESCENT_LANES") ? atoi(getenv("UGP_DESCENT_LANES")) > 16 : hf.wide_descent;
        }
    }
    *out = m;
    return UGP_OK;
}

static ugp::Options default_options() {
    ugp::Options opt;
    opt.keep_update_maps = !getenv("UGP_NO_UPDATE_MAPS");
    if (const char *e = getenv("UGP_CHUNK_NODES")) opt.chunk_nodes = (uint32_t)std::max(1, atoi(e));
    if (const char *e = getenv("UGP_PRUNE_MIN_WORDS")) opt.prune_min_words = (uint32_t)std::max(1, atoi(e));
    if (getenv("UGP_NO_SIB")) opt.sibling_records = false;
#ifdef UGP_EXPERIMENTS
    opt.keep_node_pos8 = getenv("UGP_PHASE2_PACKED") != nullptr;
#endif
    if (getenv("UGP_NO_BOUND2")) opt.second_bound = false;
    opt.keep_b3_events = !getenv("UGP_NO_BOUND3");
    if (const char *e = getenv("UGP_LDS_SLOTS")) opt.lds_slots = (uint32_t)std::max(1, std::min(60, atoi(e)));
    if (const char *e = getenv("UGP_PRE_WEIGHT")) opt.pre_weight = (uint32_t)std::max(0, atoi(e));
    return opt;
}

static int mat_create_impl(const ugp_tree_desc *tree, int device, const ugp::Options &opt, ugp_mat **out) {
    if (!tree || !out) return fail(UGP_ERR_INVALID, "null argument");
    *out = nullptr;
    HostFlat hf;
    const bool verbose = getenv("UGP_FLATTEN_VERBOSE") != nullptr;
    const auto t0 = std::chrono::steady_clock::now();
    if (int rc = host_flatten(tree, opt, true, hf)) return rc;
    const auto t1 = std::chrono::steady_clock::now();
    const int rc = upload_flat(hf, device, out);
    if (verbose)
        fprintf(stderr, "[ugp mat_create] flatten + coarse MAT %.1f ms, upload %.1f ms\n", std::chrono::duration<double, std::milli>(t1 - t0).count(),
                std::chrono::duration<double, std::milli>(std::chrono::steady_clock::now() - t1).count());
    return rc;
}

int ugp_mat_create_multi(const ugp_tree_desc *tree, const int *devices, int n_devices, ugp_mat **out) {
    if (!tree || !devices || !out || n_devices < 1) return fail(UGP_ERR_INVALID, "null argument");
    for (int i = 0; i < n_devices; i++) out[i] = nullptr;
    HostFlat hf;
    if (int rc = host_flatten(tree, default_options(), true, hf)) return rc;
    for (int i = 0; i < n_devices; i++) {
        if (int rc = upload_flat(hf, devices[i], &out[i])) {
            const std::string msg = g_err;
            for (int k = 0; k < i; k++) { ugp_mat_destroy(out[k]); out[k] = nullptr; }
            return fail(rc, msg);
        }
    }
    return UGP_OK;
}

int ugp_mat_create(const ugp_tree_desc *tree, int device, ugp_mat **out) {
    return mat_create_impl(tree, device, default_options(), out);
}

}
namespace {
constexpr uint64_t kFlatMagic = 0x3154414C46504755ull;
uint64_t flat_signature() {
    uint64_t h = 1469598103934665603ull;
    auto mix = [&](const char *p) { for (; p && *p; p++) { h ^= (uint8_t)*p; h *= 1099511628211ull; } h ^= 0xFF; h *= 1099511628211ull; };
    mix(__DATE__ " " __TIME__);
    const uint64_t fmt[] = {ugp::FLAT_FORMAT_VERSION, ugp::B3_BLOCK_SHIFT, ugp::B3_GROUP_SHIFT, ugp::T_PRUNE_MIN_DWORDS, ugp::PRUNE_MIN_WORDS, ugp::LDS_SLOTS, ugp::MAX_HOT_SLOTS,
                            ugp::INFO_JUMP_MASK, sizeof(ugp::FlatMat), sizeof(HostFlat), sizeof(ugp_result)};
    for (uint64_t v : fmt) { h ^= v; h *= 1099511628211ull; }
    for (const char *k : {"UGP_CHUNK_NODES", "UGP_PRUNE_MIN_WORDS", "UGP_NO_SIB", "UGP_NO_BOUND2", "UGP_LDS_SLOTS", "UGP_PRE_WEIGHT", "UGP_NO_UPDATE_MAPS",
                          "UGP_COARSE_MIN_NODES", "UGP_NO_SORT", "UGP_COARSE_DIV", "UGP_COARSE_FLOOR", "UGP_COARSE_CHUNK_NODES", "UGP_NO_BOUND3"}) { mix(k); mix(getenv(k)); }
    return h;
}
struct FlatWriter {
    FILE *f; bool ok = true;
    void raw(const void *p, size_t n) { if (ok && n && fwrite(p, 1, n, f) != n) ok = false; }
    template <class T> void pod(const T &v) { raw(&v, sizeof v); }
    template <class V> void vec(const V &v) { const uint64_t n = v.size(); pod(n); raw(v.data(), n * sizeof(typename V::value_type)); }
};
struct FlatReader {
    const uint8_t *p, *e; bool ok = true;
    void raw(void *d, size_t n) { if (!ok || (size_t)(e - p) < n) { ok = false; return; } memcpy(d, p, n); p += n; }
    template <class T> void pod(T &v) { raw(&v, sizeof v); }
    template <class V> void vec(V &v) {
        uint64_t n = 0; pod(n);
        if (!ok || n > (uint64_t)(e - p) / sizeof(typename V::value_type)) { ok = false; return; }
        v.resize(n); raw(v.data(), n * sizeof(typename V::value_type));
    }
};
template <class IO> void flat_io(IO &io, HostFlat &hf) {
    auto &f = hf.f;
    io.pod(f.n_nodes); io.pod(f.n_muts); io.pod(f.n_sites); io.pod(f.max_pos); io.pod(f.max_slots); io.pod(f.n_chunks);
    io.pod(f.max_path_muts); io.pod(f.max_chunk8_words); io.pod(f.lds_slots); io.pod(f.mask_not_first);
    io.vec(f.stream); io.vec(f.pre_stream); io.vec(f.chunk_body_off); io.vec(f.chunk_pre_off); io.vec(f.chunk_node_off); io.vec(f.pos2site);
    io.vec(f.site_ref); io.vec(f.rank2bfs); io.vec(f.dfs2bfs); io.vec(f.stream8); io.vec(f.pre8_stream); io.vec(f.chunk8_body_off); io.vec(f.chunk8_pre_off);
    io.vec(f.stream_t); io.vec(f.chunk_t_off); io.vec(f.rank_dfs); io.vec(f.node_pos8); io.vec(f.hdr8_of_bfs); io.vec(f.rec_of_bfs); io.vec(f.post_of_bfs);
    io.vec(f.b3_group_off); io.vec(f.b3_events);
    io.vec(hf.parent); io.vec(hf.coarse2dfs); io.vec(hf.coarse2bfs); io.vec(hf.node_pair); io.pod(hf.wide_descent);
}
}
extern "C" {

int ugp_flat_save(const ugp_tree_desc *tree, const char *path) {
    if (!tree || !path) return fail(UGP_ERR_INVALID, "null argument");
    HostFlat hf;
    if (int rc = host_flatten(tree, default_options(), true, hf)) return rc;
    const std::string tmp = std::string(path) + ".tmp." + std::to_string((unsigned long long)getpid());
    FILE *fp = fopen(tmp.c_str(), "wb");
    if (!fp) return fail(UGP_ERR_INVALID, std::string("cannot write ") + tmp);
    FlatWriter w{fp};
    w.pod(kFlatMagic); const uint64_t sig = flat_signature(); w.pod(sig);
    const uint8_t has_coarse = hf.coarse ? 1 : 0;
    w.pod(has_coarse);
    flat_io(w, hf);
    if (hf.coarse) flat_io(w, *hf.coarse);
    const bool ok = (fclose(fp) == 0) && w.ok;
    if (!ok || rename(tmp.c_str(), path) != 0) { (void)remove(tmp.c_str()); return fail(UGP_ERR_INVALID, std::string("short write to ") + path); }
    return UGP_OK;
}

int ugp_mat_create_from_flat(const char *path, int device, ugp_mat **out) {
    if (!path || !out) return fail(UGP_ERR_INVALID, "null argument");
    *out = nullptr;
    FILE *fp = fopen(path, "rb");
    if (!fp) return fail(UGP_ERR_INVALID, std::string("cannot read ") + path);
    std::vector<uint8_t> buf;
    try {
        if (fseek(fp, 0, SEEK_END) != 0) { fclose(fp); return fail(UGP_ERR_INVALID, "cannot size the flattening file"); }
        const long sz = ftell(fp);
        rewind(fp);
        buf.resize(sz > 0 ? (size_t)sz : 0);
        const bool ok = buf.empty() || fread(buf.data(), 1, buf.size(), fp) == buf.size();
        fclose(fp);
        if (!ok) return fail(UGP_ERR_INVALID, std::string("short read from ") + path);
        FlatReader r{buf.data(), buf.data() + buf.size()};
        uint64_t magic = 0, sig = 0; uint8_t has_coarse = 0;
        r.pod(magic); r.pod(sig); r.pod(has_coarse);
        if (!r.ok || magic != kFlatMagic) return fail(UGP_ERR_INVALID, "not a flattening written by ugp_flat_save");
        if (sig != flat_signature()) return fail(UGP_ERR_UNSUPPORTED, "the flattening was written by another library build or under other flattening switches");
        HostFlat hf;
        flat_io(r, hf);
        if (has_coarse) { hf.coarse = new HostFlat(); flat_io(r, *hf.coarse); }
        if (!r.ok || r.p != r.e) return fail(UGP_ERR_INVALID, "truncated or oversized flattening file");
        for (const HostFlat *x : {(const HostFlat *)&hf, (const HostFlat *)hf.coarse}) {
            if (!x) continue;
            const auto &g = x->f;
            if (g.site_ref.size() != g.n_sites || g.pos2site.size() != (size_t)g.max_pos + 1 || g.chunk8_body_off.size() != (size_t)g.n_chunks + 1 ||
                g.chunk_body_off.size() != (size_t)g.n_chunks + 1 || g.rank2bfs.size() != g.n_nodes || g.dfs2bfs.size() != g.n_nodes)
                return fail(UGP_ERR_INVALID, "inconsistent flattening file (array sizes)");
            for (int32_t v : g.pos2site) if (v >= (int64_t)g.n_sites) return fail(UGP_ERR_INVALID, "inconsistent flattening file (site index out of range)");
        }
        return upload_flat(hf, device, out);
    } catch (const std::bad_alloc &) { return fail(UGP_ERR_NOMEM, "out of host memory"); }
}

void ugp_mat_destroy(ugp_mat *m) {
    if (!m) return;
    (void)hipSetDevice(m->device);
    if (m->knobs.stats || getenv("UGP_BOUND3_VERBOSE"))
        for (int c = 0; c < B3Tuner::kClasses; c++)
            if (m->b3_tuner.blocks[c])
                fprintf(stderr, "[ugp stats] third bound, batches of class %d: %u blocks; ms per tile with %.5f (%u blocks measured), without %.5f (%u)\n", c, m->b3_tuner.blocks[c],
                        m->b3_tuner.ema[c][1], m->b3_tuner.n[c][1], m->b3_tuner.ema[c][0], m->b3_tuner.n[c][0]);
    for (auto &W : m->work) {
        if (W.aux) { (void)hipStreamSynchronize(W.aux); (void)hipStreamDestroy(W.aux); }
        for (hipEvent_t e : {W.ev_fork, W.ev_fill, W.ev_join}) if (e) (void)hipEventDestroy(e);
        if (W.stream) { (void)hipStreamSynchronize(W.stream); (void)hipStreamDestroy(W.stream); }
        if (W.done) { (void)hipEventSynchronize(W.done); (void)hipEventDestroy(W.done); }
        for (auto &G : W.gens) {
            for (auto &es : G.events)
                for (int i = 0; i < 4; i++)
                    if (es.ev[i]) (void)hipEventDestroy(es.ev[i]);
            for (int i = 0; i < 2; i++) if (G.ev_coarse[i]) (void)hipEventDestroy(G.ev_coarse[i]);
        }
    }
    for (auto &W : m->work) delete W.job_qs;
    delete m->upd.qs;
    for (hipEvent_t e : m->entry_ring) if (e) (void)hipEventDestroy(e);
    if (m->kb_done) (void)hipEventDestroy(m->kb_done);
    if (m->coarse) ugp_mat_destroy(m->coarse);
    delete m->own_qs;
    ugp::unc_free(m->unc);
    ugp::rip_free(m->rip);
    ugp::ann_free(m->ann);
    ugp::nk_free(m->near);
    ugp::gt_free(m->gt);
    ugp::sm_free(m->sm);
    ugp::tr_free(m->tr);
    ugp::dfs_tables_free(m->dfs);
    delete m;
}

int ugp_mat_info(const ugp_mat *m, ugp_info *out) {
    if (!m || !out) return fail(UGP_ERR_INVALID, "null argument");
    const auto &f = m->flat;
    out->n_nodes = f.n_nodes;
    out->n_muts = f.n_muts;
    out->n_sites = f.n_sites;
    out->stream_bytes = m->stream8_dwords * 4;
    out->algo_tree_bytes = 4 * f.n_muts + 8 * f.n_nodes;
    out->algo_tile_bytes = (uint64_t)f.max_pos / 2 + 16;
    out->n_chunks = f.n_chunks;
    out->max_slots = f.max_slots;
    out->max_position = f.max_pos;
    out->device = (uint32_t)m->device;
    return UGP_OK;
}

static int rows_error(const ugp_qset *qs, const ugp_queries *q, unsigned long long err) {
    if (err == ~0ull) return UGP_OK;
    const uint64_t row = err >> 3;
    const uint64_t smp = (uint64_t)(std::upper_bound(qs->ent_off.begin(), qs->ent_off.end(), row) - qs->ent_off.begin()) - 1;
    switch ((int)(err & 7)) {
        case ugp::ROWS_UNSORTED:
            return fail(UGP_ERR_UNSUPPORTED, "rows of sample " + std::to_string(smp) + " are not sorted by position / contain a duplicate position");
        case ugp::ROWS_BAD_REF: return fail(UGP_ERR_UNSUPPORTED, "VCF REF base of a row is not one of A,C,G,T");
        case ugp::ROWS_BAD_MASK: return fail(UGP_ERR_INVALID, "allele mask out of range");
        default:
            return fail(UGP_ERR_UNSUPPORTED, "VCF REF differs from the tree's reference base at position " + (q ? std::to_string(q->pos[row]) : std::string("of row ") + std::to_string(row)));
    }
}

static int qset_fill(ugp_mat *m, const ugp_queries *q, ugp_qset *qs, hipStream_t s = nullptr, PinBuf *stage = nullptr) {
    uint64_t n_ent = 0, max_rows = 0;
    if (int rc = validate_offsets(q, n_ent, max_rows)) return rc;
    HIP_TRY(hipSetDevice(m->device));
    qs->device = m->device;
    qs->n_queries = q->n_queries;
    qs->n_ent = n_ent;
    qs->max_rows = max_rows;
    {
        static std::atomic<uint64_t> next_serial{0};
        qs->serial = ++next_serial;
    }
    try {
        if (q->n_queries) qs->ent_off.assign(q->ent_off, q->ent_off + q->n_queries + 1);
        else qs->ent_off.assign(1, 0);
    } catch (const std::bad_alloc &) {
        return fail(UGP_ERR_NOMEM, "out of host memory");
    }
    if (n_ent == 0) return UGP_OK;
    const auto &f = m->flat;
    HIP_TRY(qs->d_pos.reserve(n_ent)); HIP_TRY(qs->d_ref.reserve(n_ent)); HIP_TRY(qs->d_nuc.reserve(n_ent));
    HIP_TRY(qs->d_missing.reserve(n_ent)); HIP_TRY(qs->d_ent_q.reserve(n_ent));
    HIP_TRY(qs->d_ent_off.reserve(q->n_queries + 1)); HIP_TRY(qs->d_err.reserve(1));
    const void *h_pos = q->pos, *h_ref = q->ref, *h_nuc = q->nuc, *h_mis = q->is_missing, *h_off = q->ent_off;
    if (stage) {
        const size_t o_ref = n_ent * 4, o_nuc = o_ref + n_ent, o_mis = o_nuc + n_ent, o_off = (o_mis + n_ent + 7) & ~(size_t)7,
                     total = o_off + (q->n_queries + 1) * 8;
        if (int rc = stage->reserve(total)) return rc;
        char *b = (char *)stage->p;
        memcpy(b, q->pos, n_ent * 4); memcpy(b + o_ref, q->ref, n_ent); memcpy(b + o_nuc, q->nuc, n_ent); memcpy(b + o_mis, q->is_missing, n_ent);
        memcpy(b + o_off, q->ent_off, (q->n_queries + 1) * 8);
        h_pos = b; h_ref = b + o_ref; h_nuc = b + o_nuc; h_mis = b + o_mis; h_off = b + o_off;
    }
    HIP_TRY(hipMemcpyAsync(qs->d_pos.p, h_pos, n_ent * 4, hipMemcpyHostToDevice, s));
    HIP_TRY(hipMemcpyAsync(qs->d_ref.p, h_ref, n_ent, hipMemcpyHostToDevice, s));
    HIP_TRY(hipMemcpyAsync(qs->d_nuc.p, h_nuc, n_ent, hipMemcpyHostToDevice, s));
    HIP_TRY(hipMemcpyAsync(qs->d_missing.p, h_mis, n_ent, hipMemcpyHostToDevice, s));
    HIP_TRY(hipMemcpyAsync(qs->d_ent_off.p, h_off, (q->n_queries + 1) * 8, hipMemcpyHostToDevice, s));
    HIP_TRY(hipMemsetAsync(qs->d_err.p, 0xFF, sizeof(unsigned long long), s));
    HIP_TRY(ugp::launch_rows_prepare(qs->d_ent_off.p, (uint32_t)q->n_queries, n_ent, qs->d_pos.p, qs->d_ref.p, qs->d_nuc.p, qs->d_missing.p,
                                     m->d_pos2site.p, m->d_site_ref.p, f.max_pos, (uint32_t)f.n_sites, qs->d_ent_q.p, qs->d_err.p, s));
    qs->nmask_for[0] = qs->nmask_for[1] = nullptr;
    {
        bool want = n_ent >= (uint64_t)q->n_queries * 128 && n_ent < (1ull << 32) && q->n_queries < (1ull << 32);
        if (m->knobs.nmask >= 0) want = m->knobs.nmask != 0 && n_ent < (1ull << 32);
        const ugp_mat *trees[2] = {m, m->coarse};
        for (int i = 0; want && i < 2; i++) {
            const ugp_mat *t = trees[i];
            if (!t || !t->flat.n_sites) continue;
            const uint32_t words = (uint32_t)(((t->flat.n_sites + 31) / 32 + 15) & ~(uint64_t)15);
            if ((size_t)words * 4 > 65536) continue;
            HIP_TRY(qs->d_nmask[i].reserve((size_t)q->n_queries * words));
            if (i == 0) { HIP_TRY(qs->d_plain_rows.reserve(n_ent)); HIP_TRY(qs->d_n_plain.reserve(1)); HIP_TRY(hipMemsetAsync(qs->d_n_plain.p, 0, 4, s)); }
            HIP_TRY(ugp::launch_nmask_build(qs->d_ent_off.p, (uint32_t)q->n_queries, qs->d_pos.p, qs->d_missing.p, t->d_pos2site.p, t->flat.max_pos, words,
                                            qs->d_nmask[i].p, i == 0 ? qs->d_plain_rows.p : nullptr, qs->d_n_plain.p, s));
            qs->nmask_for[i] = t; qs->nmask_words[i] = words;
        }
        if (!qs->nmask_for[0]) qs->nmask_for[1] = nullptr;
    }
    if (stage) return UGP_OK;
    unsigned long long err = ~0ull;
    HIP_TRY(hipMemcpy(&err, qs->d_err.p, sizeof err, hipMemcpyDeviceToHost));
    if (int rc = rows_error(qs, q, err)) return rc;
    return UGP_OK;
}

int ugp_qset_upload(ugp_mat *m, const ugp_queries *q, ugp_qset **out) {
    if (!m || !q || !out) return fail(UGP_ERR_INVALID, "null argument");
    *out = nullptr;
    ugp_qset *qs = new (std::nothrow) ugp_qset();
    if (!qs) return fail(UGP_ERR_NOMEM, "out of host memory");
    if (int rc = qset_fill(m, q, qs)) { (void)hipSetDevice(m->device); delete qs; return rc; }
    *out = qs;
    return UGP_OK;
}

void ugp_qset_destroy(ugp_qset *qs) {
    if (!qs) return;
    (void)hipSetDevice(qs->device);
    delete qs;
}

// ... 418 lines not shown

int ugp_translate(ugp_mat *m, ugp_tr_record *out, uint64_t cap, uint64_t *n_out, ugp_tr_info *info) {
    return ugp_translate_chunked(m, out, cap, n_out, info, 0);
}

int ugp_translate_time(ugp_mat *m, uint32_t reps, double *ms) {
    if (!m) return fail(UGP_ERR_INVALID, "null argument");
    return ugp::tr_time(m->tr, reps, ms);
}


int ugp_ripples_attach(ugp_mat *m, const ugp_tree_desc *tree, const uint32_t *name_rank) {
    if (!m || !tree || !tree->parent || !name_rank) return fail(UGP_ERR_INVALID, "null argument");
    if (int rc = check_handle_tree(m, tree)) return rc;
    return ugp::rip_attach(tree, name_rank, m->h_bfs2dfs, m->device, &m->rip);
}

int ugp_ripples(ugp_mat *m, const ugp_ripples_opts *opts, const uint32_t *branches, uint64_t n, ugp_ripples_event *out, uint64_t cap,
                uint64_t *n_out) {
    if (!m) return fail(UGP_ERR_INVALID, "null argument");
    return ugp::rip_run(m->rip, opts, branches, n, out, cap, n_out);
}

namespace {
struct ExHost {
    DevBuf<uint8_t> d_mask;
    DevBuf<uint32_t> d_skip, d_skip_chunk, d_rank, d_rank2out, d_out_index;
    DevBuf<int32_t> d_scores;
    ExDev dev;
};

int prepare_samples(ugp_mat *m, uint64_t Q, uint32_t order, const uint32_t *skip_node, ExHost &x) {
    const uint64_t N = m->flat.n_nodes;
    const bool dfs = order == UGP_ORDER_DFS;
    HIP_TRY(hipSetDevice(m->device));
    try {
        if (dfs) ensure_dfs_order(m);
        auto to_bfs = [&](uint64_t k) -> uint32_t { return dfs ? m->h_dfs2bfs[k] : (uint32_t)k; };
        const ugp_place_opts oo{order, nullptr, skip_node, nullptr, nullptr};
        const ugp_place_opts *o = &oo;
        if (o->skip_node) {
            std::vector<uint32_t> sk(Q);
            for (uint64_t i = 0; i < Q; i++) {
                if (o->skip_node[i] != UINT32_MAX && o->skip_node[i] >= N) return fail(UGP_ERR_INVALID, "skip_node out of range");
                sk[i] = o->skip_node[i] == UINT32_MAX ? UINT32_MAX : to_bfs(o->skip_node[i]);
            }
            HIP_TRY(x.d_skip.upload(sk));
            x.dev.skip = x.d_skip.p;
            if (m->d_dfs2bfs.p && m->d_chunk_node.p) {
                if (m->h_flat_bfs2dfs.size() != N) {
                    std::vector<uint32_t> d2b(N);
                    m->h_flat_chunk_node.resize((size_t)m->flat.n_chunks + 1);
                    HIP_TRY(hipMemcpy(d2b.data(), m->d_dfs2bfs.p, N * sizeof(uint32_t), hipMemcpyDeviceToHost));
                    HIP_TRY(hipMemcpy(m->h_flat_chunk_node.data(), m->d_chunk_node.p, m->h_flat_chunk_node.size() * sizeof(uint32_t), hipMemcpyDeviceToHost));
                    m->h_flat_bfs2dfs.resize(N);
                    for (uint64_t d = 0; d < N; d++) m->h_flat_bfs2dfs[d2b[d]] = (uint32_t)d;
                }
                std::vector<uint32_t> sc(Q, UINT32_MAX);
                const auto &cno = m->h_flat_chunk_node;
                for (uint64_t i = 0; i < Q; i++)
                    if (sk[i] != UINT32_MAX) sc[i] = (uint32_t)(std::upper_bound(cno.begin(), cno.end(), m->h_flat_bfs2dfs[sk[i]]) - cno.begin()) - 1u;
                HIP_TRY(x.d_skip_chunk.upload(sc));
                x.dev.skip_chunk = x.d_skip_chunk.p;
            }
        }
    } catch (const std::bad_alloc &) { return fail(UGP_ERR_NOMEM, "out of host memory"); }
    return UGP_OK;
}

int prepare_nodes(ugp_mat *m, const ugp_place_opts *o, ExHost &x) {
    const uint64_t N = m->flat.n_nodes;
    if (o->order > UGP_ORDER_DFS) return fail(UGP_ERR_INVALID, "unknown node order");
    if (m->h_parent.size() != N) return fail(UGP_ERR_INVALID, "this handle has no host topology (created from a coarse tree?)");
    const bool dfs = o->order == UGP_ORDER_DFS;
    HIP_TRY(hipSetDevice(m->device));
    try {
        if (dfs) ensure_dfs_order(m);
        auto to_bfs = [&](uint64_t k) -> uint32_t { return dfs ? m->h_dfs2bfs[k] : (uint32_t)k; };
        if (o->node_mask) {
            std::vector<uint8_t> mk(N);
            for (uint64_t k = 0; k < N; k++) mk[to_bfs(k)] = o->node_mask[k] ? 1 : 0;
            HIP_TRY(x.d_mask.upload(mk));
            x.dev.mask = x.d_mask.p;
        }
        if (dfs || o->distance) {
            const bool cached = dfs && !o->distance && m->dfs_rank_ready;
            if (!cached) {
                if (m->h_leaves.size() != N) {
                    std::vector<uint32_t> nch(N, 0);
                    m->h_leaves.assign(N, 0);
                    for (uint64_t j = 1; j < N; j++) nch[m->h_parent[j]]++;
                    for (uint64_t j = N; j-- > 0;) { if (!nch[j]) m->h_leaves[j] = 1; if (j) m->h_leaves[m->h_parent[j]] += m->h_leaves[j]; }
                }
                const std::vector<uint32_t> &leaves = m->h_leaves;
                const uint32_t *dist = o->distance;
                std::vector<uint64_t> keys(N);
                for (uint64_t k = 0; k < N; k++) keys[k] = ((uint64_t)(dist ? 0xFFFFFFFFu - dist[k] : 0u) << 32) | leaves[to_bfs(k)];
                DevBuf<uint32_t> &dr = (dfs && !dist) ? m->d_dfs_rank : x.d_rank, &d2o = (dfs && !dist) ? m->d_dfs_rank2out : x.d_rank2out;
                DevBuf<uint64_t> d_keys, d_keys2;
                DevBuf<uint32_t> d_iota;
                DevBuf<uint8_t> d_tmp;
                HIP_TRY(d_keys.upload(keys)); HIP_TRY(d_keys2.reserve(N)); HIP_TRY(d_iota.reserve(N)); HIP_TRY(dr.reserve(N)); HIP_TRY(d2o.reserve(N));
                if (dfs && !m->d_dfs2bfs_caller.p) HIP_TRY(m->d_dfs2bfs_caller.upload(m->h_dfs2bfs));
                size_t tmp_bytes = 0;
                HIP_TRY(ugp::launch_rank_sort(nullptr, &tmp_bytes, d_keys.p, d_keys2.p, d_iota.p, d2o.p, (uint32_t)N, nullptr, nullptr, nullptr));
                HIP_TRY(d_tmp.reserve(tmp_bytes));
                HIP_TRY(ugp::launch_rank_sort(d_tmp.p, &tmp_bytes, d_keys.p, d_keys2.p, d_iota.p, d2o.p, (uint32_t)N, dfs ? m->d_dfs2bfs_caller.p : nullptr, dr.p, nullptr));
                HIP_TRY(hipStreamSynchronize(nullptr));
                if (dfs && !dist) m->dfs_rank_ready = true;
            }
            const bool use_cache = dfs && !o->distance;
            x.dev.alt_rank = use_cache ? m->d_dfs_rank.p : x.d_rank.p;
            x.dev.rank2out = use_cache ? m->d_dfs_rank2out.p : x.d_rank2out.p;
        }
        if (dfs) {
            if (!m->d_bfs2dfs.p) HIP_TRY(m->d_bfs2dfs.upload(m->h_bfs2dfs));
            x.dev.out_index = m->d_bfs2dfs.p;
        }
    } catch (const std::bad_alloc &) { return fail(UGP_ERR_NOMEM, "out of host memory"); }
    return UGP_OK;
}

int prepare_ex(ugp_mat *m, const ugp_queries *q, const ugp_place_opts *o, ExHost &x, bool want_scores) {
    const uint64_t N = m->flat.n_nodes, Q = q->n_queries;
    if (int rc = prepare_nodes(m, o, x)) return rc;
    if (int rc = prepare_samples(m, Q, o->order, o->skip_node, x)) return rc;
    if (want_scores && o->scores && Q) {
        HIP_TRY(x.d_scores.reserve((size_t)Q * N));
        HIP_TRY(hipMemset(x.d_scores.p, 0, (size_t)Q * N * sizeof(int32_t)));
        x.dev.scores = x.d_scores.p;
    }
    return UGP_OK;
}
}

namespace {
int drain(ugp_mat *m);
bool ex_packs(const ugp_mat *m, const ugp_place_opts *o) {
    if (o->scores || m->knobs.ex_slow) return false;
    if (o->node_mask && (!o->node_mask[0] || m->upd.rec.size() != m->flat.n_nodes || m->upd.n_excluded || m->flat.n_nodes >= (1ull << 30))) return false;
    return true;
}
int mask_words(ugp_mat *m, const uint8_t *d_mask, bool set) {
    if (m->upd.n_excluded) return fail(UGP_ERR_UNSUPPORTED, "node masks on the packed path need a handle without ugp_mat_update exclusions");
    ugp_mat *trees[2] = {m, m->coarse};
    for (ugp_mat *t : trees) {
        if (!t) continue;
        auto &U = t->upd;
        if (U.rec.size() != t->flat.n_nodes) { if (t == m) return fail(UGP_ERR_UNSUPPORTED, "no update maps"); continue; }
        if (!U.d_rec_pos.p) { HIP_TRY(U.d_hdr8.upload(U.hdr8)); HIP_TRY(U.d_rec_pos.upload(U.rec)); HIP_TRY(U.d_post.upload(U.post)); }
        HIP_TRY(ugp::launch_mask_words(d_mask, t == m ? nullptr : m->d_coarse2bfs.p, (uint32_t)t->flat.n_nodes, U.d_hdr8.p, U.d_rec_pos.p, U.d_post.p,
                                       t->d_stream8.p, t->d_stream.p, t->d_stream_t.p, ugp::H_NOSCORE, set, nullptr));
    }
    return UGP_OK;
}
}

int ugp_place_batch_ex(ugp_mat *m, const ugp_queries *q, const ugp_place_opts *opts, ugp_result *out) {
    if (!m || !q || !opts || (!out && q->n_queries)) return fail(UGP_ERR_INVALID, "null argument");
    if (q->n_queries == 0) return UGP_OK;
    ugp_qset *qs = nullptr;
    if (int rc = ugp_qset_upload(m, q, &qs)) return rc;
    ExHost x;
    DevBuf<ugp_result> d_out;
    int rc = prepare_ex(m, q, opts, x, true);
    if (rc == UGP_OK && d_out.reserve(q->n_queries) != hipSuccess) rc = fail(UGP_ERR_HIP, "hipMalloc results");
    ugp_place_opts no_scores = *opts;
    no_scores.scores = nullptr;
    const bool scores_by_levels = rc == UGP_OK && opts->scores && opts->order == UGP_ORDER_BFS && !m->h_level_off.empty() && !m->knobs.scores_dfs &&
                                  !m->knobs.ex_slow && !m->knobs.force_v1 && !m->upd.n_excluded;
    const ugp_place_opts *popts = scores_by_levels ? &no_scores : opts;
    const bool pack = rc == UGP_OK && ex_packs(m, popts) && (!m->coarse || m->d_coarse2bfs.p || !opts->node_mask);
    if (pack) {
        if (rc == UGP_OK) rc = drain(m);
        ExDev xd = x.dev;
        if (rc == UGP_OK && xd.mask) rc = mask_words(m, xd.mask, true);
        const uint8_t *masked = xd.mask;
        xd.mask = nullptr; xd.packed = true; xd.scores = nullptr;
        PlaceReq r;
        r.out = d_out.p; r.ex = &xd;
        if (rc == UGP_OK) rc = run_place(m, qs, r);
        if (masked) { const int rc2 = mask_words(m, masked, false); if (rc == UGP_OK) rc = rc2; }
        if (rc == UGP_OK && scores_by_levels) {
            PlaceReq sr;
            sr.mode = 1; sr.scores = x.d_scores.p;
            rc = run_place(m, qs, sr);
            if (rc == UGP_OK && ugp::launch_scores_mask(x.d_scores.p, q->n_queries, m->flat.n_nodes, x.dev.mask, x.dev.skip, nullptr) != hipSuccess)
                rc = fail(UGP_ERR_HIP, "masking the scores");
        }
    } else if (rc == UGP_OK) {
        PlaceReq r;
        r.out = d_out.p; r.ex = &x.dev;
        rc = run_place(m, qs, r);
    }
    if (rc == UGP_OK && hipMemcpy(out, d_out.p, q->n_queries * sizeof(ugp_result), hipMemcpyDeviceToHost) != hipSuccess)
        rc = fail(UGP_ERR_HIP, "copy results");
    if (rc == UGP_OK && opts->scores) rc = copy_d2h_staged(opts->scores, x.d_scores.p, (size_t)q->n_queries * m->flat.n_nodes * sizeof(int32_t));
    if (rc == UGP_OK) {
        for (uint64_t i = 0; i < q->n_queries; i++)
            if (out[i].num_best == 0) { out[i].best_set_difference = INT32_MAX; out[i].best_j = UINT32_MAX; out[i].best_has_unique = 0; }
    }
    ugp_qset_destroy(qs);
    return rc;
}

struct ugp_ex {
    ugp_mat *m = nullptr;
    uint32_t order = UGP_ORDER_BFS;
    bool has_mask = false, mask_keeps_root = true;
    ExHost x;
};

int ugp_ex_prepare(ugp_mat *m, const ugp_place_opts *opts, ugp_ex **out) {
    if (!m || !opts || !out) return fail(UGP_ERR_INVALID, "null argument");
    *out = nullptr;
    ugp_ex *e = new (std::nothrow) ugp_ex();
    if (!e) return fail(UGP_ERR_NOMEM, "out of host memory");
    e->m = m; e->order = opts->order;
    e->has_mask = opts->node_mask != nullptr;
    e->mask_keeps_root = !opts->node_mask || opts->node_mask[0] != 0;
    if (int rc = prepare_nodes(m, opts, e->x)) { delete e; return rc; }
    *out = e;
    return UGP_OK;
}
void ugp_ex_destroy(ugp_ex *e) { delete e; }

int ugp_place_batch_prepared(ugp_mat *m, const ugp_queries *q, const ugp_ex *e, const uint32_t *skip_node, ugp_result *out, int32_t *d_scores) {
    if (!m || !q || !e || (!out && q->n_queries)) return fail(UGP_ERR_INVALID, "null argument");
    if (e->m != m) return fail(UGP_ERR_INVALID, "the prepared options belong to another handle");
    if (q->n_queries == 0) return UGP_OK;
    const uint64_t N = m->flat.n_nodes, Q = q->n_queries;
    if (!m->own_qs) { m->own_qs = new (std::nothrow) ugp_qset(); if (!m->own_qs) return fail(UGP_ERR_NOMEM, "out of host memory"); }
    ugp_qset *qs = m->own_qs;
    if (int rc = qset_fill(m, q, qs)) return rc;
    HIP_TRY(m->d_own_out.reserve(Q));
    ExHost y;
    if (int rc = prepare_samples(m, Q, e->order, skip_node, y)) return rc;
    ExDev xd = e->x.dev;
    xd.skip = y.dev.skip; xd.skip_chunk = y.dev.skip_chunk; xd.scores = nullptr;
    const bool by_levels = d_scores && e->order == UGP_ORDER_BFS && !m->h_level_off.empty() && !m->knobs.scores_dfs && !m->knobs.ex_slow && !m->knobs.force_v1 &&
                           !m->upd.n_excluded;
    const bool packs = !m->knobs.ex_slow && (!d_scores || by_levels) &&
                       (!e->has_mask || (e->mask_keeps_root && m->upd.rec.size() == N && !m->upd.n_excluded && N < (1ull << 30) && (!m->coarse || m->d_coarse2bfs.p)));
    int rc = UGP_OK;
    if (packs) {
        rc = drain(m);
        const uint8_t *masked = xd.mask;
        if (rc == UGP_OK && masked) rc = mask_words(m, masked, true);
        ExDev xp = xd;
        xp.mask = nullptr; xp.packed = true;
        PlaceReq r;
        r.out = m->d_own_out.p; r.ex = &xp;
        if (rc == UGP_OK) rc = run_place(m, qs, r);
        if (masked) { const int rc2 = mask_words(m, masked, false); if (rc == UGP_OK) rc = rc2; }
        if (rc == UGP_OK && d_scores) {
            PlaceReq sr;
            sr.mode = 1; sr.scores = d_scores;
            rc = run_place(m, qs, sr);
            if (rc == UGP_OK && ugp::launch_scores_mask(d_scores, Q, N, xd.mask, xd.skip, nullptr) != hipSuccess) rc = fail(UGP_ERR_HIP, "masking the scores");
        }
    } else {
        if (d_scores) { HIP_TRY(hipMemsetAsync(d_scores, 0, (size_t)Q * N * sizeof(int32_t), nullptr)); xd.scores = d_scores; }
        PlaceReq r;
        r.out = m->d_own_out.p; r.ex = &xd;
        rc = run_place(m, qs, r);
    }
    if (rc == UGP_OK && hipMemcpy(out, m->d_own_out.p, Q * sizeof(ugp_result), hipMemcpyDeviceToHost) != hipSuccess) rc = fail(UGP_ERR_HIP, "copy results");
    if (rc == UGP_OK)
        for (uint64_t i = 0; i < Q; i++)
            if (out[i].num_best == 0) { out[i].best_set_difference = INT32_MAX; out[i].best_j = UINT32_MAX; out[i].best_has_unique = 0; }
    return rc;
}

int ugp_tied_nodes_ex(ugp_mat *m, const ugp_queries *q, const ugp_place_opts *opts, uint32_t cap, uint32_t *tie_j, uint8_t *tie_has_unique,
                      uint32_t *tie_count) {
    if (!m || !q || !opts || !tie_count || (cap && (!tie_j || !tie_has_unique))) return fail(UGP_ERR_INVALID, "null argument");
    const uint64_t Q = q->n_queries;
    if (Q == 0) return UGP_OK;
    ugp_qset *qs = nullptr;
    if (int rc = ugp_qset_upload(m, q, &qs)) return rc;
    ExHost x;
    DevBuf<ugp_result> d_res;
    DevBuf<int32_t> d_best;
    DevBuf<uint32_t> d_cnt, d_j;
    DevBuf<uint8_t> d_hu;
    const uint64_t padded = ((Q + 63) / 64) * 64;
    int rc = prepare_ex(m, q, opts, x, false);
    auto chk = [&](hipError_t e, const char *what) {
        if (rc == UGP_OK && e != hipSuccess) rc = fail(UGP_ERR_HIP, std::string(what) + ": " + hipGetErrorString(e));
    };
    chk(d_res.reserve(Q), "hipMalloc"); chk(d_best.reserve(Q), "hipMalloc"); chk(d_cnt.reserve(padded), "hipMalloc");
    chk(d_j.reserve((size_t)Q * std::max<uint32_t>(cap, 1)), "hipMalloc"); chk(d_hu.reserve((size_t)Q * std::max<uint32_t>(cap, 1)), "hipMalloc");
    bool listed = false;
    if (rc == UGP_OK && ex_packs(m, opts) && (!m->coarse || m->d_coarse2bfs.p || !opts->node_mask)) {
        rc = drain(m);
        ExDev xd = x.dev;
        if (rc == UGP_OK && xd.mask) rc = mask_words(m, xd.mask, true);
        const uint8_t *masked = xd.mask;
        xd.mask = nullptr; xd.packed = true;
        if (rc == UGP_OK) chk(hipMemsetAsync(d_cnt.p, 0, padded * sizeof(uint32_t), nullptr), "memset");
        m->tie_lists_filled = m->tie_sub_batches = 0;
        PlaceReq r;
        r.out = d_res.p; r.tie_count = d_cnt.p; r.tie_j = d_j.p; r.tie_hu = d_hu.p; r.tie_cap = cap; r.ex = &xd;
        if (rc == UGP_OK) rc = run_place(m, qs, r);
        listed = rc == UGP_OK && m->tie_sub_batches > 0 && m->tie_lists_filled == m->tie_sub_batches;
        if (masked) { const int rc2 = mask_words(m, masked, false); if (rc == UGP_OK) rc = rc2; }
// ... 228 lines not shown
        if (k == cap) { memcpy(ids, st + o_ids, n * (size_t)k * 4); memcpy(has_unique, st + o_hu, n * (size_t)k); }
        else for (uint64_t i = 0; i < n; i++) {
            memcpy(ids + i * cap, st + o_ids + i * (size_t)k * 4, (size_t)k * 4);
            memcpy(has_unique + i * cap, st + o_hu + i * (size_t)k, k);
        }
    }
    return UGP_OK;
}

static void tuner_poll(ugp_mat *m) {
    B3Tuner &T = m->b3_tuner;
    for (;;) {
        EventSet *hit = nullptr;
        for (auto &W : m->work)
            for (auto &G : W.gens)
                if (G.timing_pending)
                    for (size_t i = 0; i < G.events_used; i++)
                        if (G.events[i].b3_class >= 0 && G.events[i].b3_seq == T.next_seq) hit = &G.events[i];
        if (!hit && T.seq > T.next_seq + 16) { T.resync(T.next_seq + 1); continue; }
        if (!hit || hipEventQuery(hit->ev[3]) != hipSuccess) break;
        if (hit->b3_pos == 0) { T.acc = 0; T.acc_n = 0; }
        float gap = 0;
        if (T.prev_done && hit->b3_pos >= B3Tuner::kSkip && hit->b3_tiles && hipEventElapsedTime(&gap, (hipEvent_t)T.prev_done, hit->ev[3]) == hipSuccess && gap > 0) {
            T.acc += (double)gap / hit->b3_tiles; T.acc_n++;
        }
        if (hit->b3_pos == B3Tuner::kBlock - 1 && T.acc_n && !hit->b3_first) T.record(hit->b3_class, hit->b3_used, T.acc / T.acc_n);
        T.prev_done = (void *)hit->ev[3];
        T.next_seq++;
        hit->b3_class = -1;
    }
    (void)hipGetLastError();
}
static void tuner_release(ugp_mat *m, ugp_mat::Work::Gen &G) {
    tuner_poll(m);
    B3Tuner &T = m->b3_tuner;
    for (size_t i = 0; i < G.events_used; i++) {
        EventSet &es = G.events[i];
        if (es.b3_class >= 0) { T.resync(es.b3_seq + 1); es.b3_class = -1; }
        if (T.prev_done == (void *)es.ev[3]) T.prev_done = nullptr;
    }
}

static int harvest_timing(ugp_mat *m, ugp_mat::Work &W, ugp_mat::Work::Gen &G) {
    if (G.timing_pending) {
        float table = 0, place = 0, merge = 0;
        for (size_t i = 0; i < G.events_used; i++) {
            EventSet &es = G.events[i];
            HIP_TRY(hipEventSynchronize(es.ev[3]));
            float t;
            HIP_TRY(hipEventElapsedTime(&t, es.ev[0], es.ev[1])); table += t;
            HIP_TRY(hipEventElapsedTime(&t, es.ev[1], es.ev[2])); place += t;
            HIP_TRY(hipEventElapsedTime(&t, es.ev[2], es.ev[3])); merge += t;
        }
        G.last.table_ms = table; G.last.place_ms = place; G.last.merge_ms = merge;
        G.last.coarse_ms = 0;
        if (G.coarse_timed) { HIP_TRY(hipEventSynchronize(G.ev_coarse[1])); HIP_TRY(hipEventElapsedTime(&G.last.coarse_ms, G.ev_coarse[0], G.ev_coarse[1])); }
        G.last.words_total = W.last_words_total;
        G.last.words_skipped = 0;
        if (W.last_used_best8 && W.d_stats.p && m->knobs.stats) {
            uint64_t v[96] = {0};
            HIP_TRY(hipMemcpy(v, W.d_stats.p, sizeof v, hipMemcpyDeviceToHost));
            G.last.words_skipped = v[0];
            G.last.reserved = (uint32_t)std::min<uint64_t>(v[1], 0xFFFFFFFFull);
            if (const char *tf = m->knobs.trace.empty() ? nullptr : m->knobs.trace.c_str()) {
                if (W.d_trace.p) {
                    uint64_t n = 0;
                    HIP_TRY(hipMemcpy(&n, W.d_trace.p, 8, hipMemcpyDeviceToHost));
                    n = std::min<uint64_t>(n, 1u << 20);
                    std::vector<uint64_t> rec(n * 6);
                    if (n) HIP_TRY(hipMemcpy(rec.data(), W.d_trace.p + 8, n * 48, hipMemcpyDeviceToHost));
                    if (FILE *fp = fopen(tf, "wb")) { fwrite(rec.data(), 8, rec.size(), fp); fclose(fp); }
                    fprintf(stderr, "[ugp stats] %llu unit records written to %s\n", (unsigned long long)n, tf);
                }
            }
            {
                fprintf(stderr, "[ugp stats] restarts=%llu restart_cycles=%llu wave_cycles=%llu max_wave=%llu hist:", (unsigned long long)v[1],
                        (unsigned long long)v[2], (unsigned long long)v[3], (unsigned long long)v[4]);
                for (int i = 0; i < 16; i++) fprintf(stderr, " %llu", (unsigned long long)v[5 + i]);
                fprintf(stderr, "\n[ugp stats] jumps decided by the first node after a restart=%llu", (unsigned long long)v[26]);
                fprintf(stderr, "\n[ugp stats] own-region units=%llu cycles=%llu   other units=%llu cycles=%llu\n", (unsigned long long)v[29],
                        (unsigned long long)v[27], (unsigned long long)v[30], (unsigned long long)v[28]);
                fprintf(stderr, "[ugp stats] other units by what the preamble records decided: whole unit skipped %llu (cycles %llu), body entered late %llu (cycles %llu), "
                                "nothing %llu (cycles %llu)\n[ugp stats] units skipped whole: cycles pulling %llu, replaying the preamble %llu, closing %llu\n", (unsigned long long)v[32], (unsigned long long)v[33],
                        (unsigned long long)v[34], (unsigned long long)v[35], (unsigned long long)v[36], (unsigned long long)v[37], (unsigned long long)v[38],
                        (unsigned long long)v[39], (unsigned long long)v[40]);
                fprintf(stderr, "[ugp stats] restarts by cause (own-region / other units): jump %llu / %llu, sibling jump %llu / %llu, chunk end %llu / %llu, slow header %llu / %llu\n",
                        (unsigned long long)v[48], (unsigned long long)v[49], (unsigned long long)v[50], (unsigned long long)v[51], (unsigned long long)v[52],
                        (unsigned long long)v[53], (unsigned long long)v[54], (unsigned long long)v[55]);
                fprintf(stderr, "[ugp stats] units split while running: %llu\n", (unsigned long long)v[31]);
                fprintf(stderr, "[ugp stats] nodes evaluated: %llu in unit bodies = %.3f %% of nodes x tiles (%llu x %u), %llu in preamble replays\n", (unsigned long long)v[66],
                        G.last.n_tiles ? 100.0 * (double)v[66] / ((double)m->flat.n_nodes * G.last.n_tiles) : 0.0, (unsigned long long)m->flat.n_nodes, G.last.n_tiles,
                        (unsigned long long)v[67]);
                fprintf(stderr, "[ugp stats] third bound: asked at a restart %llu times, decided the jump %llu times\n", (unsigned long long)v[64], (unsigned long long)v[65]);
                fprintf(stderr, "[ugp stats] third bound by the record's hsub - hsec (1 2 3 more), decided/asked: %llu/%llu %llu/%llu %llu/%llu %llu/%llu\n", (unsigned long long)v[92],
                        (unsigned long long)v[88], (unsigned long long)v[93], (unsigned long long)v[89], (unsigned long long)v[94], (unsigned long long)v[90], (unsigned long long)v[95],
                        (unsigned long long)v[91]);
                fprintf(stderr, "[ugp stats] third bound by jump length (<16 <32 <64 <128 <256 <512 <1024 more), decided/asked:");
                for (int i = 0; i < 8; i++) fprintf(stderr, " %llu/%llu", (unsigned long long)v[80 + i], (unsigned long long)v[72 + i]);
                fprintf(stderr, "\n");
                fprintf(stderr, "[ugp stats] jump lengths in words (<8 <16 <32 <64 <128 <512 <4096 more):");
                for (int i = 0; i < 8; i++) fprintf(stderr, " %llu", (unsigned long long)v[56 + i]);
                fprintf(stderr, "\n");
                if (W.last_nitems) {
                    uint32_t ni = 0;
                    HIP_TRY(hipMemcpy(&ni, W.last_nitems, 4, hipMemcpyDeviceToHost));
                    fprintf(stderr, "[ugp stats] phase 2: %u (chunk, 64-sample sub-tile) pairs walked by k_ties\n", ni);
                }
                if (W.last_list_n && W.last_list_tiles) {
                    std::vector<uint32_t> ln(W.last_list_tiles);
                    HIP_TRY(hipMemcpy(ln.data(), W.last_list_n, ln.size() * sizeof(uint32_t), hipMemcpyDeviceToHost));
                    uint64_t rec = 0;
                    for (uint32_t x : ln) rec += x;
                    fprintf(stderr, "[ugp stats] chunk records stored by phase 1: %llu of %llu (chunk, tile) pairs = %.1f MB\n", (unsigned long long)rec,
                            (unsigned long long)m->flat.n_chunks * W.last_list_tiles, rec * 1024.0 / 1e6);
                }
            }
        }
        m->tsum.table_ms += G.last.table_ms; m->tsum.place_ms += G.last.place_ms; m->tsum.merge_ms += G.last.merge_ms;
        m->tsum.coarse_ms += G.last.coarse_ms; m->tsum.place_launches += G.last.place_launches; m->tsum.bound3 += G.last.bound3;
        m->tsum_calls++;
        tuner_release(m, G);
        G.timing_pending = false;
    }
    return UGP_OK;
}

int ugp_get_timing(ugp_mat *m, ugp_timing *out) {
    if (!m || !out) return fail(UGP_ERR_INVALID, "null argument");
    HIP_TRY(hipSetDevice(m->device));
    ugp_mat::Work &W = m->work[m->last_work];
    if (int rc = harvest_timing(m, W, W.gens[W.cur])) return rc;
    *out = W.gens[W.cur].last;
    return UGP_OK;
}

int ugp_debug_bound3_tables(ugp_mat *m, uint32_t tile, uint16_t *over, uint16_t *under, uint64_t cap, uint64_t *n_blocks) {
    if (!m || !n_blocks) return fail(UGP_ERR_INVALID, "null argument");
    HIP_TRY(hipSetDevice(m->device));
    ugp_mat::Work &W = m->work[m->last_work];
    *n_blocks = W.b3_host.n_blocks;
    if (!W.b3_host.over) { *n_blocks = 0; return UGP_OK; }
    if (!over || !under) return UGP_OK;
    if (cap < W.b3_host.n_blocks) return fail(UGP_ERR_INVALID, "buffer too small");
    HIP_TRY(hipDeviceSynchronize());
    const size_t nb = W.b3_host.n_blocks;
    std::vector<uint8_t> tmp(nb);
    HIP_TRY(hipMemcpy(tmp.data(), W.b3_host.over + (uint64_t)tile * nb, nb, hipMemcpyDeviceToHost));
    for (size_t i = 0; i < nb; i++) over[i] = tmp[i];
    HIP_TRY(hipMemcpy(tmp.data(), W.b3_host.under + (uint64_t)tile * nb, nb, hipMemcpyDeviceToHost));
    for (size_t i = 0; i < nb; i++) under[i] = tmp[i];
    return UGP_OK;
}

int ugp_get_timing_sum(ugp_mat *m, ugp_timing *sum, uint32_t *n_calls) {
    if (!m || !sum || !n_calls) return fail(UGP_ERR_INVALID, "null argument");
    HIP_TRY(hipSetDevice(m->device));
    for (auto &W : m->work)
        for (auto &G : W.gens)
            if (int rc = harvest_timing(m, W, G)) return rc;
    const ugp_timing &l = m->work[m->last_work].gens[m->work[m->last_work].cur].last;
    *sum = l;
    sum->table_ms = m->tsum.table_ms; sum->place_ms = m->tsum.place_ms; sum->merge_ms = m->tsum.merge_ms; sum->coarse_ms = m->tsum.coarse_ms;
    sum->place_launches = m->tsum.place_launches;
    sum->bound3 = m->tsum.bound3;
    *n_calls = m->tsum_calls;
    m->tsum = {};
    m->tsum_calls = 0;
    return UGP_OK;
}

int ugp_mat_reload_knobs(ugp_mat *m) {
    if (!m) return fail(UGP_ERR_INVALID, "null argument");
    m->knobs = ugp::Knobs::from_env();
    if (m->coarse) m->coarse->knobs = m->knobs;
    return UGP_OK;
}

int ugp_has_experiments(void) {
#ifdef UGP_EXPERIMENTS
    return 1;
#else
    return 0;
#endif
}

int ugp_mat_create_chunked(const ugp_tree_desc *tree, int device, uint32_t chunk_nodes, ugp_mat **out) {
    ugp::Options opt = default_options();
    opt.chunk_nodes = chunk_nodes;
    return mat_create_impl(tree, device, opt, out);
}

struct ugp_flat { ugp::FlatMat f; };

int ugp_flat_create(const ugp_tree_desc *tree, uint32_t chunk_nodes, ugp_flat **out) {
    if (!tree || !out) return fail(UGP_ERR_INVALID, "null argument");
    *out = nullptr;
    ugp_flat *fl = new (std::nothrow) ugp_flat();
    if (!fl) return fail(UGP_ERR_NOMEM, "out of host memory");
    ugp::Options opt = default_options();
    opt.chunk_nodes = chunk_nodes;
    std::string err;
    int rc;
    try {
        rc = ugp::flatten(*tree, opt, fl->f, err);
    } catch (const std::bad_alloc &) {
        delete fl;
        return fail(UGP_ERR_NOMEM, "out of host memory while flattening the tree");
    }
    if (rc != UGP_OK) { delete fl; return fail(rc, err); }
    *out = fl;
    return UGP_OK;
}

void ugp_flat_destroy(ugp_flat *fl) { delete fl; }

int ugp_flat_get(const ugp_flat *fl, int which, const void **ptr, uint64_t *count) {
    if (!fl || !ptr || !count) return fail(UGP_ERR_INVALID, "null argument");
    const auto &f = fl->f;
    switch (which) {
        case UGP_FLAT_STREAM: *ptr = f.stream.data(); *count = f.stream.size(); break;
        case UGP_FLAT_PRE_STREAM: *ptr = f.pre_stream.data(); *count = f.pre_stream.size(); break;
        case UGP_FLAT_CHUNK_BODY_OFF: *ptr = f.chunk_body_off.data(); *count = f.chunk_body_off.size(); break;
        case UGP_FLAT_CHUNK_PRE_OFF: *ptr = f.chunk_pre_off.data(); *count = f.chunk_pre_off.size(); break;
        case UGP_FLAT_CHUNK_NODE_OFF: *ptr = f.chunk_node_off.data(); *count = f.chunk_node_off.size(); break;
        case UGP_FLAT_POS2SITE: *ptr = f.pos2site.data(); *count = f.pos2site.size(); break;
        case UGP_FLAT_SITE_REF: *ptr = f.site_ref.data(); *count = f.site_ref.size(); break;
        case UGP_FLAT_RANK2BFS: *ptr = f.rank2bfs.data(); *count = f.rank2bfs.size(); break;
        case UGP_FLAT_DFS2BFS: *ptr = f.dfs2bfs.data(); *count = f.dfs2bfs.size(); break;
        case UGP_FLAT_MAX_SLOTS: *ptr = nullptr; *count = f.max_slots; break;
        case UGP_FLAT_STREAM8: *ptr = f.stream8.data(); *count = f.stream8.size(); break;
        case UGP_FLAT_PRE8_STREAM: *ptr = f.pre8_stream.data(); *count = f.pre8_stream.size(); break;
        case UGP_FLAT_CHUNK8_BODY_OFF: *ptr = f.chunk8_body_off.data(); *count = f.chunk8_body_off.size(); break;
        case UGP_FLAT_CHUNK8_PRE_OFF: *ptr = f.chunk8_pre_off.data(); *count = f.chunk8_pre_off.size(); break;
        case UGP_FLAT_STREAM_T: *ptr = f.stream_t.data(); *count = f.stream_t.size(); break;
        case UGP_FLAT_CHUNK_T_OFF: *ptr = f.chunk_t_off.data(); *count = f.chunk_t_off.size(); break;
        case UGP_FLAT_MAX_PATH_MUTS: *ptr = nullptr; *count = f.max_path_muts; break;
        case UGP_FLAT_LDS_SLOTS: *ptr = nullptr; *count = f.lds_slots; break;
        case UGP_FLAT_B3_GROUP_OFF: *ptr = f.b3_group_off.data(); *count = f.b3_group_off.size(); break;
        case UGP_FLAT_B3_EVENTS: *ptr = f.b3_events.data(); *count = f.b3_events.size(); break;
        default: return fail(UGP_ERR_INVALID, "unknown array id");
    }
    return UGP_OK;
}

}
```

usher_amd/csrc/ugp_flatten.hpp:

```cpp
#pragma once
#include <cstdint>
#include <memory>
#include <new>
#include <algorithm>
#include <string>
#include <thread>
#include <utility>
#include <vector>

#include "usher_amd.h"

namespace ugp {

constexpr uint32_t RS_REG = 63, RS_BOTTOM = 62, WS_NONE = 63;
constexpr uint32_t F_LEAF = 1u << 28, F_NOSCORE = 1u << 29, F_ROOT = 1u << 30, F_MASKED = 1u << 31;
constexpr uint32_t M_AFTER_MASK = 1u << 31;
constexpr uint32_t MAX_SLOTS = 40;

constexpr uint32_t T_INFO_MARK = 0xFFFFu;
constexpr uint32_t T_PRUNE_MIN_DWORDS = 8;

constexpr uint32_t H_TAG = 1u << 31, H_INFO = 1u << 30, H_RARE = 1u << 29, H_SIB = 1u << 21;
constexpr uint32_t H_REG = 1u << 0, H_STORE = 1u << 1, H_NOSCORE = 1u << 2, H_END = 1u << 3, H_FREE = 1u << 4,
                   H_SKIPD = 1u << 5,  H_SLOW = 1u << 7, H_CHUNK_END = 1u << 8, H_NOP = 1u << 9;
constexpr uint32_t H_RSLOT_SHIFT = 10, H_WSLOT_SHIFT = 20;
constexpr uint32_t CE_LEN_SHIFT = 10, CE_LEN_MASK = (1u << 19) - 1u;
constexpr uint32_t INFO_JUMP_MASK = (1u << 18) - 1u, INFO_HS_SHIFT = 22, INFO_HS_MAX = 127;
constexpr uint32_t INFO_HR_SHIFT = 18, INFO_HR_NONE = 7;
constexpr uint32_t PRE_HS_NONE = 127;
constexpr uint32_t PRUNE_MIN_WORDS = 4;
#ifndef UGP_HOT_SLOTS
#define UGP_HOT_SLOTS 16
#endif
constexpr uint32_t MAX_HOT_SLOTS = UGP_HOT_SLOTS;
constexpr uint32_t LDS_SLOTS = 9;
constexpr uint32_t M_FLUSH = 1u << 28, M_END = 1u << 30;
constexpr uint32_t B3_BLOCK_SHIFT = 4, B3_BLOCK_WORDS = 1u << B3_BLOCK_SHIFT;
constexpr uint32_t B3_GROUP_SHIFT = 8, B3_GROUP_BLOCKS = 1u << B3_GROUP_SHIFT;
inline uint32_t b3_blocks(uint64_t stream8_words) { return (uint32_t)((((stream8_words + B3_BLOCK_WORDS - 1) >> B3_BLOCK_SHIFT) + 1u + B3_GROUP_BLOCKS - 1u) & ~(uint64_t)(B3_GROUP_BLOCKS - 1u)); }
constexpr uint32_t MAX_SITES = 1u << 22;
constexpr uint32_t FLAT_FORMAT_VERSION = 6;
constexpr uint32_t MAX_NODE_MUTS = 65534;

struct Options {
    uint32_t chunk_nodes = 0;
    uint32_t prune_min_words = PRUNE_MIN_WORDS;
    bool sibling_records = true;
    bool second_bound = true;
    bool keep_node_pos8 = false;
    uint32_t lds_slots = LDS_SLOTS;
    uint32_t pre_weight = 32;
    bool keep_update_maps = false;
    bool keep_b3_events = false;
    uint32_t threads = 0;
};

template <class T>
struct DefaultInit : std::allocator<T> {
    template <class U> struct rebind { using other = DefaultInit<U>; };
    using std::allocator<T>::allocator;
    template <class U> void construct(U *p) noexcept { ::new (static_cast<void *>(p)) U; }
    template <class U, class... A> void construct(U *p, A &&...a) { ::new (static_cast<void *>(p)) U(std::forward<A>(a)...); }
};
template <class T> using UVec = std::vector<T, DefaultInit<T>>;

struct FlatMat {
    uint64_t n_nodes = 0, n_muts = 0, n_sites = 0;
    uint32_t max_pos = 0, max_slots = 0, n_chunks = 0;
    UVec<uint32_t> stream;
    UVec<uint32_t> pre_stream;
    std::vector<uint32_t> chunk_body_off;
    std::vector<uint32_t> chunk_pre_off;
    std::vector<uint32_t> chunk_node_off;
    std::vector<int32_t> pos2site;
    std::vector<uint8_t> site_ref;
    UVec<uint32_t> rank2bfs;
    UVec<uint32_t> dfs2bfs;
    UVec<uint32_t> stream8, pre8_stream;
    std::vector<uint32_t> chunk8_body_off, chunk8_pre_off;
    UVec<uint32_t> stream_t, chunk_t_off;
    uint32_t max_path_muts = 0;
    std::vector<uint32_t> rank_dfs;
    std::vector<uint32_t> node_pos8;
    UVec<uint32_t> hdr8_of_bfs, rec_of_bfs, post_of_bfs;
    std::vector<uint32_t> b3_group_off;
    UVec<uint32_t> b3_events;
    uint32_t max_chunk8_words = 0;
    uint32_t lds_slots = 0;
    bool mask_not_first = false;
};

struct FlatExtras {
    UVec<uint32_t> sub, dfsidx;
    UVec<uint32_t> node_pair;
    uint64_t children_of_wide_nodes = 0;
};

int flatten(const ugp_tree_desc &t, const Options &opt, FlatMat &out, std::string &err, FlatExtras *extras = nullptr);

struct Par {
    unsigned T;
    uint64_t grain = 0;
    template <class F>
    void run(uint64_t n, F fn, uint64_t min_per_thread = 8192) const;
    uint64_t exclusive_scan(uint32_t *a, uint64_t n) const;
};
unsigned flatten_threads(const Options &opt);
Par flatten_par(const Options &opt);

template <class F>
void Par::run(uint64_t n, F fn, uint64_t min_per_thread) const {
    if (grain) min_per_thread = grain;
    const unsigned t = (unsigned)std::min<uint64_t>(T, std::max<uint64_t>(1, n / std::max<uint64_t>(1, min_per_thread)));
    if (t <= 1) { fn((uint64_t)0, n, 0u); return; }
    std::vector<std::thread> th;
    th.reserve(t - 1);
    for (unsigned i = 1; i < t; i++) th.emplace_back([&fn, n, t, i] { fn(n * i / t, n * (i + 1) / t, i); });
    fn((uint64_t)0, n / t, 0u);
    for (auto &x : th) x.join();
}

}
```

usher_amd/csrc/ugp_kernels.hpp:

```cpp
#pragma once
#include <hip/hip_runtime.h>
#include <stdint.h>

#include "ugp_flatten.hpp"
#include "usher_amd.h"

namespace ugp {

constexpr uint32_t TABLE_CONST_ROWS = 4;

struct PlaceArgs {
    const uint32_t *stream, *pre_stream;
    const uint32_t *chunk_body_off, *chunk_pre_off, *chunk_node_off;
    const uint32_t *stream_t, *chunk_t_off;
    const uint32_t *table;
    const uint32_t *dbottom;
    uint32_t n_sites, n_chunks, n_groups, n_tiles, n_queries;
    uint32_t *part_best, *part_cnt, *part_key;
    const uint32_t *dfs2bfs;
    uint64_t n_nodes;
    int32_t *scores;
    const int32_t *best_in;
    uint32_t *tie_count;
    uint32_t *tie_j;
    uint8_t *tie_hu;
    uint32_t tie_cap;
    const uint8_t *node_mask;
    const uint32_t *skip;
    const uint32_t *alt_rank;
    const uint32_t *out_index;
};

struct Best8Args {
    const uint32_t *stream8, *pre8;
    const uint32_t *chunk8_body_off, *chunk8_pre_off;
    const uint32_t *table;
    const uint32_t *dbottom;
    uint32_t n_sites, n_chunks, n_groups, n_tiles;
    uint32_t max_slots;
    uint32_t lds_slots;
    uint32_t *cold;
    const uint32_t *active;
    uint32_t active_words;
    uint32_t *lbest;
    uint32_t *luniq;
    uint32_t *lpos;
    uint32_t *list, *list_n;
    uint32_t *queue;
    const uint4 *units;
    const uint32_t *unit_base, *unit_count;
    uint32_t *dyn_ctl;
    unsigned long long *dyn_units;
    uint32_t dyn_cap, dyn_epoch;
    uint32_t lds_bits;
    uint32_t no_pre_records;
    uint32_t split_heavy;
    uint32_t split_dense;
    uint32_t split_many;
    uint32_t split_cycles;
    uint32_t ub_every;
    uint32_t freeze_ub;
    uint32_t refill_all_rows;
    uint32_t heavy_prio;
    uint64_t *trace;
    uint64_t trace_cap;
    uint64_t *stats;
    uint32_t *ub;
    uint32_t *tie_cnt, *tie_key;
    const uint32_t *node_pos8;
    const uint32_t *rank_dfs;
    const uint32_t *chunk_node_off;
    uint32_t n_queries;
    const struct B3Dev *b3;
};

hipError_t launch_build_units(const uint32_t *hstart, const uint32_t *hlen, uint32_t n_tiles512, uint32_t n_chunks, uint32_t unit_chunks, uint32_t heavy_chunks,
                              uint32_t grow_every, uint32_t unit_max, uint32_t light_order, uint32_t per_tile_cap, void *units, uint32_t *unit_base,
                              uint32_t *unit_count, uint32_t *dyn_ctl, hipStream_t s);
constexpr uint32_t SCORES_SB = 32;
hipError_t launch_scores_levels(const uint32_t *node_pair, const uint32_t *parent, const uint32_t *stream, const uint32_t *table, uint32_t n_sites,
                                const uint32_t *dbottom, const uint32_t *level_off, uint32_t n_levels, void *d_a, void *d_b, bool d16, uint32_t d_stride,
                                uint32_t qpad, uint32_t n_queries, uint64_t n_nodes, int32_t *scores, uint32_t block , hipStream_t s);
hipError_t best8_occupancy(size_t lds_bytes, int variant , int *per_cu);
hipError_t launch_best8(const Best8Args &a, uint32_t blocks, hipStream_t s);
constexpr uint32_t GBEST_SLICES = 64;
hipError_t launch_coarse_result(const uint32_t *lbest, const uint32_t *lpos, const uint32_t *list, const uint32_t *list_n, uint32_t n_chunks, uint32_t n_tiles512,
                                uint32_t n_queries, const uint32_t *chunk_node_off, const uint32_t *chunk8_body_off, const uint32_t *node_pos8,
                                const uint32_t *dfs2bfs, ugp_result *out, hipStream_t s);
hipError_t launch_phase2_packed(const Best8Args &b1, const uint32_t *list, const uint32_t *list_n, uint32_t *gbest_part, uint32_t *gbest, uint32_t n_tiles512,
                                void *units, uint32_t *info, uint32_t *cnt, uint32_t *key, const uint32_t *node_pos8, const uint32_t *rank_dfs,
                                const uint32_t *chunk_node_off, const uint32_t *rank2bfs, uint32_t n_queries, ugp_result *out, const uint32_t *order,
                                uint32_t blocks, hipStream_t s);
struct Phase2Uniq {
    const uint32_t *luniq, *dnode, *refined, *dres;
    uint32_t *gcnt , *gcnt_part ;
};
hipError_t launch_phase2(const PlaceArgs &a, const uint32_t *lbest, const uint32_t *list, const uint32_t *list_n, uint32_t *gbest_part,
                         uint32_t *gbest, uint32_t n_tiles512,
                         uint32_t *items, uint32_t *n_items, uint32_t cap, uint32_t *cnt, uint32_t *key,
                         const uint32_t *rank2bfs, const uint32_t *rank2out ,
                         ugp_result *out, const uint32_t *order, uint32_t max_slots, bool lists ,
                         const Phase2Uniq *uniq , hipStream_t s);

enum { ROWS_UNSORTED = 1, ROWS_BAD_REF = 2, ROWS_BAD_MASK = 3, ROWS_REF_MISMATCH = 4 };
hipError_t launch_rows_prepare(const uint64_t *ent_off, uint32_t n_queries, uint64_t n_ent, const int32_t *pos, const uint8_t *ref,
                               const uint8_t *nuc, const uint8_t *is_missing, const int32_t *pos2site, const uint8_t *site_ref,
                               uint32_t max_pos, uint32_t n_sites, uint32_t *ent_q, unsigned long long *err, hipStream_t s);
hipError_t launch_fill_table(uint32_t *table, const uint8_t *site_ref, uint32_t n_sites, uint64_t total_dwords,
                             hipStream_t s);
hipError_t launch_build_tiles(uint32_t *table, uint32_t *active, uint32_t active_words, uint32_t n_tiles512, const uint64_t *ent_off, uint32_t q0,
                              const uint32_t *order , uint32_t nq, const int32_t *pos, const uint8_t *ref,
                              const uint8_t *nuc, const uint8_t *is_missing, const int32_t *pos2site, const int32_t *site_pos, const uint8_t *site_ref,
                              uint32_t n_sites, uint32_t max_pos, uint32_t *dbottom, const unsigned long long *err ,
                              hipStream_t s);
hipError_t launch_scatter(uint32_t *table, uint32_t *dbottom, const int32_t *pos, const uint8_t *ref,
                          const uint8_t *nuc, const uint8_t *is_missing, const uint32_t *ent_q,
                          const int32_t *pos2site, uint32_t max_pos, uint32_t n_sites, uint64_t n_ent, uint32_t q_base,
                          uint32_t *active, uint32_t active_words, const uint32_t *slot_of, const unsigned long long *err,
                          uint32_t *useful , uint32_t useful_words, hipStream_t s);
hipError_t launch_nmask_build(const uint64_t *ent_off, uint32_t n_queries, const int32_t *pos, const uint8_t *is_missing, const int32_t *pos2site,
                              uint32_t max_pos, uint32_t words, uint32_t *nmask, uint32_t *plain_rows , uint32_t *n_plain, hipStream_t s);
hipError_t launch_ntiles(uint32_t *table, uint32_t *active, uint32_t active_words, uint32_t n_tiles512, const uint32_t *nmask, uint32_t words,
                         const uint32_t *order, uint32_t q0, uint32_t nq, const uint8_t *site_ref, uint32_t n_sites, hipStream_t s);
hipError_t launch_scatter_list(uint32_t *table, uint32_t *dbottom, const int32_t *pos, const uint8_t *ref, const uint8_t *nuc, const uint8_t *is_missing,
                               const uint32_t *ent_q, const int32_t *pos2site, uint32_t max_pos, uint32_t n_sites, uint32_t q_base, uint32_t n_q,
                               uint32_t *active, uint32_t active_words, const uint32_t *slot_of, const uint32_t *row_list, const uint32_t *n_listed,
                               const unsigned long long *err, uint32_t *useful, uint32_t useful_words, hipStream_t s);
hipError_t launch_tile_ranges(const uint32_t *keys_sorted, uint32_t n_queries, uint32_t n_tiles512, const uint32_t *chunk_node_off,
                              uint32_t n_chunks, uint32_t align, uint32_t *hstart, uint32_t *hlen, hipStream_t s);
hipError_t launch_descend(const ugp_result *coarse_res, const uint32_t *order, uint32_t n_queries, const uint32_t *coarse2bfs,
                          const uint32_t *node_pair , const uint32_t *parent, const uint32_t *stream,
                          const uint32_t *table, uint32_t n_sites, uint32_t *refined, bool wide ,
                          uint32_t max_expansions , int slack, const uint32_t *skip ,
                          uint32_t *dnode ,
                          hipStream_t s);
hipError_t launch_seed_ub(const ugp_result *coarse_res, const uint32_t *order, uint32_t n_queries, uint32_t n_tiles512, uint32_t *ub,
                          const uint32_t *refined ,
                          uint32_t *dbottom , uint32_t pad_d,
                          const uint32_t *skip , const uint32_t *coarse2bfs,
                          const uint32_t *dnode , uint32_t *dres ,
                          hipStream_t s);
hipError_t launch_fix_skip(const PlaceArgs &a, uint32_t *lbest, const uint32_t *skip_chunk , uint32_t n_tiles512, const uint32_t *rank2bfs,
                           const uint32_t *order, uint32_t max_slots, hipStream_t s);
hipError_t launch_locality_sort(const ugp_result *coarse_res, const uint32_t *coarse2dfs, uint32_t n, uint32_t *keys,
                                uint32_t *keys_sorted, uint32_t *idx, uint32_t *order, uint32_t *slot_of, void *temp,
                                size_t *temp_bytes, const uint32_t *coarse_bin, uint32_t n_bins, uint32_t *bins, hipStream_t s);
hipError_t launch_extract_best(const ugp_result *res, uint32_t n, int32_t *best, hipStream_t s);
hipError_t launch_place(const PlaceArgs &a, int mode, uint32_t max_slots, hipStream_t s);
hipError_t launch_merge(const uint32_t *part_best, const uint32_t *part_cnt, const uint32_t *part_key,
                        const uint32_t *rank2bfs, uint32_t n_groups, uint32_t n_queries, ugp_result *out,
                        hipStream_t s);

}
```

usher_amd/csrc/ugp_plan.hpp:

```cpp
#pragma once
#include <stdint.h>

#include <algorithm>

#include "ugp_flatten.hpp"
#include "ugp_knobs.hpp"
#include "ugp_tuner.hpp"

namespace ugp {

constexpr uint32_t kMaxTilesPerLaunch = 4096;

struct PlanTree {
    uint64_t n_nodes = 0, n_sites = 0;
    uint32_t n_chunks = 0, max_chunk8_words = 0, max_path_muts = 0, lds_slots = 0;
    bool mask_not_first = false;
    bool coarse = false;
    bool b3_events = false;
    bool wide_descent = false;
};
struct PlanEx {
    bool given = false, packed = false, mask = false, skip = false, skip_chunk = false, scores = false;
};
struct PlanCall {
    uint64_t Q = 0, max_rows = 0;
    int mode = 0;
    bool coarse_only = false;
    bool ties = false;
    bool nmask = false;
    bool sharing = false;
    int share_sets = 2;
    PlanEx ex;
};

struct CallPlan {
    uint32_t n_sites = 1, active_words = 1, useful_words = 1;
    bool ex_packable = false, ex_skip = false, packed_ok = false, sorted = false, can_fork = false, fill_ahead = false;
    uint64_t sub_tiles = kMaxTilesPerLaunch;
};

inline CallPlan plan_call(const PlanTree &t, const Knobs &K, const PlanCall &c) {
    CallPlan p;
    p.n_sites = std::max<uint32_t>((uint32_t)t.n_sites, 1u);
    p.active_words = (p.n_sites + 31) / 32;
    p.useful_words = (p.n_sites + 7) / 8;
    p.ex_packable = c.ex.given && c.ex.packed && !c.ex.mask && (!c.ex.skip || c.ex.skip_chunk) && !c.ex.scores;
    p.ex_skip = p.ex_packable && c.ex.skip;
    p.packed_ok = (c.mode == 0) && (!c.ex.given || p.ex_packable) && !K.force_v1 && !t.mask_not_first && (c.max_rows + t.max_path_muts + 2 < 0x7F7Full);
    p.sorted = p.packed_ok && t.coarse && c.Q > 512 && !K.no_sort && !K.no_prune;
    p.can_fork = p.sorted && !c.coarse_only && !K.no_fork && !c.sharing;
    p.fill_ahead = p.can_fork && !(c.nmask && p.n_sites) && K.tile_build <= 0 && t.n_sites && std::min<uint64_t>(c.Q, (uint64_t)kMaxTilesPerLaunch * 64) == c.Q;
    if (t.n_chunks) p.sub_tiles = std::min<uint64_t>(p.sub_tiles, std::max<uint64_t>(8, ((K.lbest_gib ? (uint64_t)K.lbest_gib : 24ull) << 30) / ((uint64_t)t.n_chunks * 128) & ~7ull));
    return p;
}

inline uint32_t pick_groups(const PlanTree &t, const Knobs &K, uint32_t n_tiles, uint32_t target_waves = 4096) {
    if (K.target_waves) target_waves = K.target_waves;
    uint32_t g = (target_waves + n_tiles - 1) / n_tiles;
    if (K.groups) g = K.groups;
    g = std::min<uint32_t>(g, t.n_chunks);
    g = std::max<uint32_t>(g, 1);
    if (g >= 8) g &= ~7u;
    return g;
}

struct SubPlan {
    uint32_t n_tiles = 0, n_tiles512 = 0, G = 1;
    bool nmask = false;
    bool lds_build = false;
    uint32_t lds_bits_plan = 0;
    bool b3_can = false, b3_tuned = false;
    bool b3_want = false;
    int b3_class = 0;
    bool uniq_ok = false;
};

inline SubPlan plan_sub(const PlanTree &t, const Knobs &K, const PlanCall &c, const CallPlan &cp, uint64_t nq, uint64_t rows) {
    SubPlan p;
    p.n_tiles = (uint32_t)((nq + 63) / 64);
    p.n_tiles512 = (uint32_t)((nq + 511) / 512);
    p.G = pick_groups(t, K, p.n_tiles);
    if (cp.packed_ok) {
        uint32_t unit_chunks = 16;
        if (K.unit_chunks) unit_chunks = K.unit_chunks;
        p.G = std::max<uint32_t>(1, (t.n_chunks + unit_chunks - 1) / unit_chunks);
        while (p.G < t.n_chunks && (uint64_t)p.G * p.n_tiles512 < 4096) p.G = std::min<uint32_t>(t.n_chunks, p.G * 2);
        if (K.groups) p.G = std::min<uint32_t>(t.n_chunks, K.groups);
    }
    p.nmask = c.nmask && cp.packed_ok && cp.n_sites;
    p.lds_build = cp.packed_ok && cp.n_sites && !cp.sorted && rows >= (uint64_t)nq * 128;
    if (K.tile_build >= 0) p.lds_build = cp.packed_ok && cp.n_sites && K.tile_build != 0;
    if (cp.packed_ok) {
        const bool stats_on = K.stats;
        p.lds_bits_plan = (!stats_on && (size_t)cp.active_words * 4 <= 4096 && p.n_tiles512 >= 64 && !c.sharing) ? 1u : 0u;
        if (p.nmask && !stats_on) p.lds_bits_plan = 2u;
        if (K.lds_bits >= 0) p.lds_bits_plan = stats_on ? 0u : (K.lds_bits == 2 ? 2u : (((size_t)cp.active_words * 4 <= 4096 && K.lds_bits != 0) ? 1u : 0u));
    }
    p.b3_can = cp.packed_ok && !c.coarse_only && cp.sorted && t.b3_events && !K.no_bound3 && K.bound3 != 0 && !K.no_prune && p.n_tiles512 <= 256 && K.tile_build <= 0 &&
               p.lds_bits_plan != 1u && !(p.lds_build && !p.nmask);
    p.b3_want = p.b3_can;
    p.b3_class = B3Tuner::class_of(rows, nq);
    p.b3_tuned = p.b3_can && K.bound3 == -1;
    if (!p.b3_tuned && p.b3_can && K.bound3 < -1) p.b3_want = b3_static_choice(t.wide_descent, p.b3_class, t.n_nodes);
    p.uniq_ok = cp.packed_ok && cp.sorted && !c.coarse_only && c.mode == 0 && !c.ex.given && !c.ties && t.n_nodes < (1ull << 31) && !K.no_uniq;
    return p;
}

struct ZeroLayout {
    size_t z_dbottom = 0, z_active = 0, z_queue = 0, z_list_n = 0, z_nitems = 0, z_cnt = 0, z_key = 0, z_useful = 0, z_end = 0;
};
inline ZeroLayout zero_layout(uint32_t n_tiles512, uint32_t active_words, uint32_t useful_words, bool b3_want) {
    ZeroLayout z;
    z.z_dbottom = 0; z.z_active = z.z_dbottom + (size_t)n_tiles512 * 512; z.z_queue = z.z_active + (size_t)n_tiles512 * active_words;
    z.z_list_n = z.z_queue + 8; z.z_nitems = z.z_list_n + n_tiles512; z.z_cnt = z.z_nitems + 8; z.z_key = z.z_cnt + (size_t)n_tiles512 * 512;
    z.z_useful = z.z_key + (size_t)n_tiles512 * 512; z.z_end = z.z_useful + (b3_want ? (size_t)n_tiles512 * useful_words : 0);
    return z;
}

inline uint32_t seed_pad_d(const PlanTree &t, const Knobs &K) {
    return K.no_pad_fix ? 0u : (uint32_t)std::min<uint64_t>(4096, 0x7F7Eu - 2u - std::min<uint64_t>(t.max_path_muts, 0x7F00u));
}

struct UnitCaps { uint32_t n_side = 0, per_tile_cap = 0; };
inline UnitCaps unit_caps(uint32_t n_chunks, uint32_t unit_chunks, uint32_t heavy_chunks, uint32_t grow_every, uint32_t unit_max) {
    auto len_of = [&](uint32_t i) -> uint64_t {
        if (!grow_every) return unit_chunks;
        return std::min<uint64_t>((uint64_t)unit_chunks << std::min<uint32_t>(i / grow_every, 16u), std::max(unit_max, unit_chunks));
    };
    UnitCaps u;
    for (uint64_t done = 0; done < n_chunks; u.n_side++) done += len_of(u.n_side);
    u.per_tile_cap = (n_chunks + heavy_chunks - 1) / heavy_chunks + 2u * u.n_side + 2u;
    return u;
}

struct WalkPlan {
    bool tile_ranges = false;
    bool bounds = false;
    uint32_t unit_chunks = 1, heavy_chunks = 16, light_order = 0, grow_every = 0, unit_max = 0, no_pre_records = 0;
    uint32_t n_side = 0, per_tile_cap = 0;
    uint32_t split_cycles = 0, split_heavy = 0, split_dense = 0, split_many = 0, ub_every = 128;
    uint32_t lds_bits = 0;
    size_t lds_bytes = 0;
    bool b3 = false;
    int variant = 0;
};

inline WalkPlan plan_walk(const PlanTree &t, const Knobs &K, const PlanCall &c, const CallPlan &cp, const SubPlan &sp) {
    WalkPlan w;
    w.bounds = !K.no_prune;
    w.tile_ranges = cp.sorted && !K.no_lpt;
    w.unit_chunks = std::max<uint32_t>(1, (t.n_chunks + sp.G - 1) / sp.G);
    if (K.ub_every) w.ub_every = K.ub_every;
    w.light_order = K.light_order >= 0 ? (uint32_t)K.light_order : (t.wide_descent ? 1u : 0u);
    if (K.heavy_chunks) w.heavy_chunks = K.heavy_chunks;
    w.grow_every = (w.tile_ranges && w.bounds) ? 8u : 0u; w.unit_max = w.unit_chunks * 16u;
    if (K.unit_grow >= 0) w.grow_every = (w.tile_ranges && w.bounds) ? (uint32_t)K.unit_grow : 0u;
    if (K.unit_max) w.unit_max = K.unit_max;
    {
        const uint64_t reach = INFO_JUMP_MASK - 1u, cw = std::max<uint32_t>(1, t.max_chunk8_words);
        w.unit_max = (uint32_t)std::max<uint64_t>(w.unit_chunks, std::min<uint64_t>(w.unit_max, reach / cw));
        w.no_pre_records = ((uint64_t)std::max(w.unit_chunks, w.heavy_chunks) * cw > reach) ? 1u : 0u;
    }
    const UnitCaps u = unit_caps(t.n_chunks, w.unit_chunks, w.heavy_chunks, w.grow_every, w.unit_max);
    w.n_side = u.n_side; w.per_tile_cap = u.per_tile_cap;
    w.split_cycles = 400000; w.split_heavy = 400000;
    if (K.split_cycles >= 0) w.split_cycles = (uint32_t)K.split_cycles;
    if (K.split_heavy >= 0) w.split_heavy = (uint32_t)K.split_heavy;
    if (!w.split_heavy) w.split_heavy = 0xFFFFFFFFu;
    if (!w.split_cycles || t.n_chunks >= (1u << 20) || sp.n_tiles512 > 4096) w.split_cycles = w.split_heavy = 0xFFFFFFFFu;
    w.split_dense = K.split_dense >= 0 ? (uint32_t)K.split_dense : 0xFFFFFFFFu;
    w.split_many = K.split_many ? ((K.split_many & 0xFFFFu) | (std::max(1u, K.split_many_heavy ? K.split_many_heavy : K.split_many) << 16)) : 0u;
    w.lds_bits = sp.lds_bits_plan;
    w.lds_bytes = (size_t)t.lds_slots * 64 * 16 + (w.lds_bits == 1 ? (((size_t)cp.active_words * 4 + 15) & ~(size_t)15) : 0);
    w.b3 = sp.b3_want && w.bounds && w.lds_bits != 1;
    w.variant = c.coarse_only ? (w.lds_bits == 2 ? 4 : 2) : (w.b3 ? (w.lds_bits == 2 ? 6 : 5) : (w.lds_bits == 2 ? 3 : (w.lds_bits ? 1 : 0)));
    return w;
}

struct GridPlan { int waves_cu = 1; uint64_t blocks = 8; };
inline GridPlan plan_grid(const PlanTree &t, const Knobs &K, const PlanCall &c, const CallPlan &cp, const SubPlan &sp, int occ_per_cu, int n_cu) {
    GridPlan g;
    g.waves_cu = std::max(occ_per_cu, 1);
    if (c.sharing) g.waves_cu = std::max(1, K.shared_waves ? (int)K.shared_waves : (c.share_sets >= 3 ? g.waves_cu * 5 / 16 : g.waves_cu / 2));
    else if (!c.coarse_only && cp.sorted && sp.b3_class == 0 && sp.n_tiles512 <= 32 && !t.wide_descent && g.waves_cu >= 16) g.waves_cu = g.waves_cu * 3 / 4;
    if (K.waves_per_cu) g.waves_cu = std::max(1, std::min(std::max(occ_per_cu, 1), (int)K.waves_per_cu));
    g.blocks = (uint64_t)g.waves_cu * std::max(n_cu, 1);
    g.blocks = std::min<uint64_t>(g.blocks, (uint64_t)sp.n_tiles512 * sp.G);
    g.blocks = ((g.blocks + 7) / 8) * 8;
    return g;
}

constexpr int kMaxSets = 4;
inline int pipeline_depth(const Knobs &K) { return std::max(2, std::min(kMaxSets, (int)K.depth)); }
inline int sets_in_use(const Knobs &K, uint64_t n_queries, uint64_t n_rows) {
    return (n_queries > 32768 || n_rows > n_queries * 128) ? 2 : pipeline_depth(K);
}

}
```

usher_amd/placement.py:

```python
from __future__ import annotations

import ctypes as C
from typing import Dict, List, Optional, Sequence

import numpy as np

from . import _lib
from ._lib import build_library

RESULT_DTYPE = np.dtype([("best_set_difference", np.int32), ("num_best", np.uint32), ("best_j", np.uint32),
                         ("best_has_unique", np.uint32)])


class UgpError(RuntimeError):
    def __init__(self, code: int, msg: str):
        super().__init__("ugp error %d: %s" % (code, msg))
        self.code = code


def _check(rc: int) -> None:
    if rc != 0:
        raise UgpError(rc, (_lib.lib().ugp_last_error() or b"").decode())


# ... 367 lines not shown
        return self._sm_records(self._L.ugp_summary_roho_chunked, self.SM_ROHO, chunk_items, cap)

    def summary_clades(self, columns):
        if not getattr(self, "_sm_ready", False):
            self.summary_attach()
        off, nodes = self._clades_csr(columns)
        n_leaves = self._t.n - len(np.unique(self._t.parent[1:]))
        per = np.zeros(len(nodes), self.SM_CLADE)
        per["column"] = np.repeat(np.arange(len(columns), dtype=np.uint32), np.diff(off).astype(np.int64))
        per["node"] = nodes
        incl = np.zeros(len(nodes), np.uint32); excl = np.zeros(len(nodes), np.uint32)
        leaf_clade = np.zeros((len(columns), n_leaves), np.uint32)
        self._ck(self._L.ugp_summary_clades(self._h, _ptr(off), _ptr(nodes), len(columns), _ptr(incl), _ptr(excl), _ptr(leaf_clade)))
        per["inclusive"] = incl
        per["exclusive"] = excl
        return per, leaf_clade

    def summary_time(self, reps: int = 5):
        if not getattr(self, "_sm_ready", False):
            self.summary_attach()
        a, b = C.c_double(0), C.c_double(0)
        self._ck(self._L.ugp_summary_time(self._h, int(reps), C.byref(a), C.byref(b)))
        return float(a.value), float(b.value)

    TR_RECORD = np.dtype([("node", np.uint32), ("codon", np.uint32), ("before", np.uint8, (3,)), ("after", np.uint8, (3,)),
                          ("pad", np.uint8, (2,)), ("ent", np.uint32, (3,))])
    TR_INFO = np.dtype([("n_records", np.uint64), ("n_nodes", np.uint64), ("n_inconsistent", np.uint64), ("n_duplicate", np.uint64),
                        ("first_inconsistent", np.uint32), ("first_duplicate", np.uint32)])

    def translate_attach(self, arrays: Optional[Dict] = None):
        t = self._t if arrays is None else _TreeArrays(arrays)
        self._ck(self._L.ugp_translate_attach(self._h, C.byref(t.desc)))
        self._tr_ready = True

    def translate_codons(self, slot_pos, slot_init):
        if not getattr(self, "_tr_ready", False):
            self.translate_attach()
        pos = np.ascontiguousarray(slot_pos, dtype=np.int32).reshape(-1)
        if isinstance(slot_init, str):
            slot_init = slot_init.encode()
        init = (np.frombuffer(slot_init, np.uint8) if isinstance(slot_init, (bytes, bytearray))
                else np.ascontiguousarray(slot_init, dtype=np.uint8).reshape(-1))
        init = np.ascontiguousarray(init)
        if len(pos) % 3 or len(pos) != len(init):
            raise UgpError(-1, "slot_pos and slot_init hold three values per codon")
        self._ck(self._L.ugp_translate_codons(self._h, len(pos) // 3, _ptr(pos), _ptr(init)))

    def translate(self, chunk_items: int = 0, cap: Optional[int] = None):
        info = np.zeros(1, self.TR_INFO)
        self._tr_info = None
        n_out = C.c_uint64(0)
        fn = self._L.ugp_translate_chunked

        def call(buf, room):
            rc = fn(self._h, _ptr(buf) if room else None, int(room), C.byref(n_out), _ptr(info), int(chunk_items))
            if rc != -1:
                self._tr_info = info[0].copy()
            self._ck(rc)

        if cap is None:
            call(None, 0)
            cap = int(n_out.value)
        out = np.zeros(int(cap), self.TR_RECORD)
        call(out, cap)
        self._tr_n_out = int(n_out.value)
        return out[:min(int(cap), self._tr_n_out)], info[0].copy()

    def translate_time(self, reps: int = 5) -> float:
        ms = C.c_double(0)
        self._ck(self._L.ugp_translate_time(self._h, int(reps), C.byref(ms)))
        return float(ms.value)

    RIPPLES_EVENT = np.dtype([("branch", np.uint64), ("i", np.uint32), ("j", np.uint32), ("donor", np.uint32), ("acceptor", np.uint32),
                              ("donor_count", np.uint32), ("acceptor_count", np.uint32), ("donor_score", np.int32),
                              ("acceptor_score", np.int32), ("donor_sibling", np.uint8), ("acceptor_sibling", np.uint8),
                              ("pad", np.uint8, 6)])

    def ripples_attach(self, name_rank, arrays: Optional[Dict] = None):
        rank = np.ascontiguousarray(name_rank, dtype=np.uint32)
        t = getattr(self, "_rip_t", self._t) if arrays is None else _TreeArrays(arrays)
        self._ck(self._L.ugp_ripples_attach(self._h, C.byref(t.desc), _ptr(rank)))
        self._rip_t = t
        self._rip_rank = rank.copy()

    def ripples(self, branches, name_rank, branch_len: int = 3, min_range: int = 1000, max_range: int = 10 ** 7,
                parsimony_improvement: int = 3, num_descendants: int = 10) -> np.ndarray:
        rank = np.ascontiguousarray(name_rank, dtype=np.uint32)
        if getattr(self, "_rip_rank", None) is None or not np.array_equal(self._rip_rank, rank):
            self.ripples_attach(rank)
        br = np.ascontiguousarray(branches, dtype=np.uint32)
        opts = _lib.ugp_ripples_opts(int(branch_len), int(min_range), int(max_range), int(parsimony_improvement), int(num_descendants))
        n_out = C.c_uint64(0)
        cap = max(16, 4 * len(br))
        while True:
            out = np.zeros(cap, self.RIPPLES_EVENT)
            self._ck(self._L.ugp_ripples(self._h, C.byref(opts), _ptr(br), len(br), _ptr(out), cap, C.byref(n_out)))
            if n_out.value <= cap:
                return out[:n_out.value]
            cap = int(n_out.value)

    def node_order(self, order: str) -> np.ndarray:
        out = np.zeros(self.n_nodes, dtype=np.uint32)
        self._ck(self._L.ugp_node_order(self._h, {"bfs": 0, "dfs": 1}[order], _ptr(out)))
        return out

    def subtree_mask(self, root_j: int, max_levels: int, order: str = "bfs") -> np.ndarray:
        out = np.zeros(self.n_nodes, dtype=np.uint8)
        self._ck(self._L.ugp_subtree_mask(self._h, {"bfs": 0, "dfs": 1}[order], int(root_j), int(max_levels), _ptr(out)))
        return out

    def update(self, records: Sequence[Dict] = (), retired: Sequence[int] = ()) -> int:
        n = len(records)
        flat_j = np.array([0xFFFFFFFF if r.get("flat_j") is None else r["flat_j"] for r in records], np.uint32)
        flags = np.array([(1 if r.get("leaf") else 0) | (2 if r.get("masked") else 0) for r in records], np.uint8)
        n_path = np.array([len(r["path"]) for r in records], np.uint32)
        off = np.zeros(n + 1, np.uint64)
        pos, al, pv, rf = [], [], [], []
        for i, r in enumerate(records):
            for (p, a, f) in r["path"]:
                pos.append(p); al.append(a); pv.append(0); rf.append(f)
            for (p, m, pr, f) in r["own"]:
                pos.append(p); al.append(m); pv.append(pr); rf.append(f)
            off[i + 1] = len(pos)
        pos = np.array(pos, np.int32); al = np.array(al, np.uint8); pv = np.array(pv, np.uint8); rf = np.array(rf, np.uint8)
        t = _lib.ugp_touched(n, _ptr(flat_j), _ptr(flags), _ptr(n_path), _ptr(off), _ptr(pos), _ptr(al), _ptr(pv), _ptr(rf))
        ret = np.ascontiguousarray(list(retired), dtype=np.uint32)
        first = C.c_uint32()
        self._ck(self._L.ugp_mat_update(self._h, C.byref(t), _ptr(ret), len(ret), C.byref(first)))
        return int(first.value)

    def touched_open(self, batch: QueryBatch) -> None:
        self._ck(self._L.ugp_touched_open(self._h, C.byref(batch.desc)))

    def touched_score(self, first_id: int, first_sample: int) -> None:
        self._ck(self._L.ugp_touched_score(self._h, first_id, first_sample))

    def touched_rescore(self, sample: int) -> None:
        self._ck(self._L.ugp_touched_rescore(self._h, sample))

    def touched_fetch(self, first_sample: int, n: int, cap: int = 64):
        best = np.zeros(n, np.int32); cnt = np.zeros(n, np.uint32)
        ids = np.zeros((n, max(cap, 1)), np.uint32); hu = np.zeros((n, max(cap, 1)), np.uint8)
        self._ck(self._L.ugp_touched_fetch(self._h, first_sample, n, cap, _ptr(best), _ptr(cnt), _ptr(ids), _ptr(hu)))
        return best, cnt, ids, hu

    def upload(self, batch: QueryBatch):
        h = C.c_void_p()
        self._ck(self._L.ugp_qset_upload(self._h, C.byref(batch.desc), C.byref(h)))
        return h

    def free_qset(self, h) -> None:
        self._L.ugp_qset_destroy(h)

    def place_device(self, qset, d_out_ptr: int, stream: int = 0) -> None:
        self._ck(self._L.ugp_place_device(self._h, qset, C.c_void_p(d_out_ptr), C.c_void_p(stream)))

    def place_device_overlapped(self, qset, d_out_ptr: int, stream: int = 0) -> None:
        self._ck(self._L.ugp_place_device_overlapped(self._h, qset, C.c_void_p(d_out_ptr), C.c_void_p(stream)))

    def pipeline_depth(self) -> int:
        return int(self._L.ugp_pipeline_depth(self._h))

    def timing(self) -> Dict:
        out = _lib.ugp_timing()
        self._ck(self._L.ugp_get_timing(self._h, C.byref(out)))
        return {k: getattr(out, k) for k, _ in out._fields_}

    def timing_sum(self) -> Dict:
        out = _lib.ugp_timing()
        n = C.c_uint32()
        self._ck(self._L.ugp_get_timing_sum(self._h, C.byref(out), C.byref(n)))
        d = {k: getattr(out, k) for k, _ in out._fields_}
        d["calls"] = int(n.value)
        return d


class MultiPlacer:

    def __init__(self, arrays: Dict, devices: Sequence[int]):
        L = _lib.lib()
        self._t = _TreeArrays(arrays)
        self.n_nodes = self._t.n
        self.devices = list(devices)
        n = len(self.devices)
        devs = (C.c_int * n)(*self.devices)
        hs = (C.c_void_p * n)()
        _check(L.ugp_mat_create_multi(C.byref(self._t.desc), devs, n, hs))
        self._hs = [C.c_void_p(h) for h in hs]

    def close(self) -> None:
        for h in getattr(self, "_hs", []):
            if h.value:
                _lib.lib().ugp_mat_destroy(h)
        self._hs = []

    def __del__(self):
        try:
            self.close()
        except Exception:
            pass

    def place(self, batch: QueryBatch) -> np.ndarray:
        import threading
        from .dist import shard_bounds
        n = len(self._hs)
        out = np.zeros(len(batch), dtype=RESULT_DTYPE)
        errs: List[Optional[BaseException]] = [None] * n

        def work(d: int):
            try:
                lo, hi = shard_bounds(len(batch), n, d)
                if hi > lo:
                    part = batch.slice(lo, hi)
                    res = np.zeros(hi - lo, dtype=RESULT_DTYPE)
                    _check(_lib.lib().ugp_place_batch(self._hs[d], C.byref(part.desc), _ptr(res)))
                    out[lo:hi] = res
            except BaseException as e:
                errs[d] = e

        ts = [threading.Thread(target=work, args=(d,)) for d in range(n)]
        for t in ts:
            t.start()
        for t in ts:
            t.join()
        for e in errs:
            if e is not None:
                raise e
        return out
```

Measured before the change: 14.27 million placements/s.

## Add sparse event-based coarse pre-pass replacing the walked coarse placement

After: 15.78 million placements/s, median of 6. 1.11x the previous value.

```diff
diff --git a/include/usher_amd.h b/include/usher_amd.h
--- a/include/usher_amd.h
+++ b/include/usher_amd.h
@@ -238,6 +238,8 @@
 int ugp_get_timing_sum(ugp_mat *mat, ugp_timing *sum, uint32_t *n_calls);
 
 int ugp_debug_bound3_tables(ugp_mat *mat, uint32_t tile, uint16_t *over, uint16_t *under, uint64_t cap, uint64_t *n_blocks);
+int ugp_debug_coarse_pass(ugp_mat *mat, ugp_qset *qs, int method, int32_t *cost, uint32_t *coarse_node, uint32_t *kept_bfs, uint64_t kept_cap, uint64_t *n_kept);
+int ugp_debug_last_prepass(const ugp_mat *mat);
 
 const char *ugp_last_error(void);
 
diff --git a/usher_amd/_lib.py b/usher_amd/_lib.py
--- a/usher_amd/_lib.py
+++ b/usher_amd/_lib.py
@@ -124,6 +124,8 @@
     "ugp_get_timing": (C.c_int, [P, C.POINTER(ugp_timing)]),
     "ugp_get_timing_sum": (C.c_int, [P, C.POINTER(ugp_timing), C.POINTER(C.c_uint32)]),
     "ugp_debug_bound3_tables": (C.c_int, [P, C.c_uint32, P, P, C.c_uint64, C.POINTER(C.c_uint64)]),
+    "ugp_debug_coarse_pass": (C.c_int, [P, P, C.c_int, P, P, P, C.c_uint64, C.POINTER(C.c_uint64)]),
+    "ugp_debug_last_prepass": (C.c_int, [P]),
     "ugp_last_error": (C.c_char_p, []),
     "ugp_fitch_sankoff": (C.c_int, [C.c_int, C.c_uint64, P, C.POINTER(ugp_sites), C.POINTER(P)]),
     "ugp_fitch_count": (C.c_uint64, [P]),
diff --git a/usher_amd/csrc/ugp_capi.cpp b/usher_amd/csrc/ugp_capi.cpp
--- a/usher_amd/csrc/ugp_capi.cpp
+++ b/usher_amd/csrc/ugp_capi.cpp
@@ -18,6 +18,7 @@
 #include "ugp_bound3.hpp"
 #include "ugp_dense.hpp"
 #include "ugp_tuner.hpp"
+#include "ugp_coarse.hpp"
 #include "ugp_plan.hpp"
 #include "ugp_flatten.hpp"
 #include "ugp_kernels.hpp"
@@ -181,6 +182,10 @@
     bool wide_descent = false;
     DevBuf<uint32_t> d_coarse2dfs, d_coarse_bin;
     uint32_t n_coarse_bins = 0;
+    DevBuf<uint32_t> d_cs_node, d_cs_rmq, d_cs_site_off, d_cs_events;
+    uint32_t cs_nodes = 0, cs_max_per_pos = 0;
+    int last_prepass = 0;
+    bool mask_in_force = false;
     std::vector<uint32_t> h_level_off;
     uint32_t max_level_width = 0;
     std::vector<uint32_t> h_parent, h_dfs2bfs, h_bfs2dfs, h_leaves;
@@ -395,6 +400,11 @@
     t.n_nodes = f.n_nodes; t.n_sites = f.n_sites; t.n_chunks = f.n_chunks; t.max_chunk8_words = f.max_chunk8_words;
     t.max_path_muts = f.max_path_muts; t.lds_slots = f.lds_slots; t.mask_not_first = f.mask_not_first;
     t.coarse = m->coarse != nullptr; t.b3_events = m->d_b3_events.p != nullptr; t.wide_descent = m->wide_descent;
+    if (m->coarse && m->cs_nodes) {
+        t.coarse_nodes = m->cs_nodes; t.coarse_max_per_pos = m->cs_max_per_pos;
+        t.coarse_excluded = m->upd.n_excluded != 0;
+        t.coarse_masked = m->mask_in_force;
+    }
     return t;
 }
 
@@ -440,6 +450,28 @@
     return UGP_OK;
 }
 
+int coarse_sparse(ugp_mat *m, const ugp_qset *qs, uint32_t cap, ugp_result *out, hipStream_t s) {
+    const ugp_mat *t = m->coarse;
+    ugp::CoarseSparseArgs a{};
+    a.ent_off = (const uint64_t *)qs->d_ent_off.p; a.pos = qs->d_pos.p; a.ref = qs->d_ref.p; a.nuc = qs->d_nuc.p; a.is_missing = qs->d_missing.p;
+    a.err = qs->d_err.p; a.pos2site = t->d_pos2site.p; a.max_pos = (uint32_t)t->flat.max_pos; a.n_nodes = m->cs_nodes; a.n_queries = (uint32_t)qs->n_queries;
+    a.cap = cap; a.site_off = m->d_cs_site_off.p; a.events = (const uint2 *)m->d_cs_events.p; a.node = (const uint2 *)m->d_cs_node.p; a.rmq = m->d_cs_rmq.p;
+    a.dfs2bfs = t->d_dfs2bfs.p; a.out = out;
+    a.n_ent = qs->n_ent; a.max_rows = qs->max_rows; a.max_per_pos = m->cs_max_per_pos;
+    HIP_TRY(ugp::launch_coarse_sparse(a, s));
+    return UGP_OK;
+}
+
+int coarse_walked(ugp_mat *m, ugp_qset *qs, ugp_result *out, hipStream_t s, int wi) {
+    m->coarse->sharing = m->sharing; m->coarse->share_n = m->share_n; m->coarse->share_sets = m->share_sets;
+    PlaceReq cr;
+    cr.out = out; cr.stream = s; cr.wi = wi;
+    cr.coarse_only = m->coarse->d_node_pos8.p && m->coarse->flat.max_chunk8_words < 65536u && !m->knobs.coarse_phase2;
+    if (int rc = run_place(m->coarse, qs, cr)) return rc;
+    HIP_TRY(hipSetDevice(m->device));
+    return UGP_OK;
+}
+
 int coarse_pass(PlaceCall &c) {
     ugp_mat *m = c.m;
     ugp_mat::Work &W = c.W;
@@ -447,12 +479,14 @@
     HIP_TRY(W.d_coarse_res.reserve(c.call.Q));
     if (!TG.ev_coarse[0]) { HIP_TRY(hipEventCreate(&TG.ev_coarse[0])); HIP_TRY(hipEventCreate(&TG.ev_coarse[1])); }
     HIP_TRY(hipEventRecord(TG.ev_coarse[0], c.s));
-    m->coarse->sharing = m->sharing; m->coarse->share_n = m->share_n; m->coarse->share_sets = m->share_sets;
-    PlaceReq cr;
-    cr.out = W.d_coarse_res.p; cr.stream = c.s; cr.wi = c.r.wi;
-    cr.coarse_only = m->coarse->d_node_pos8.p && m->coarse->flat.max_chunk8_words < 65536u && !m->knobs.coarse_phase2;
-    if (int rc = run_place(m->coarse, c.qs, cr)) return rc;
-    HIP_TRY(hipSetDevice(m->device));
+    m->last_prepass = c.cp.coarse_sparse ? 2 : 1;
+    if (c.cp.coarse_sparse) {
+        if (int rc = coarse_sparse(m, c.qs, c.cp.coarse_cap, W.d_coarse_res.p, c.s)) return rc;
+        HIP_TRY(hipEventRecord(TG.ev_coarse[1], c.s));
+        TG.coarse_timed = true;
+        return UGP_OK;
+    }
+    if (int rc = coarse_walked(m, c.qs, W.d_coarse_res.p, c.s, c.r.wi)) return rc;
     HIP_TRY(hipEventRecord(TG.ev_coarse[1], c.s));
     TG.coarse_timed = true;
     return UGP_OK;
@@ -875,6 +909,7 @@
     c.cp = ugp::plan_call(c.tree, m->knobs, c.call);
     c.ex_skip = c.cp.ex_skip ? r.ex->skip : nullptr;
     c.TG->coarse_timed = false;
+    m->last_prepass = 0;
     if (int rc = side_fill(c)) return rc;
     if (c.cp.sorted) if (int rc = coarse_pass(c)) return rc;
     for (uint64_t q0 = 0; q0 < c.call.Q; q0 += c.cp.sub_tiles * 64) {
@@ -913,6 +948,7 @@
     ugp::FlatMat f;
     std::vector<uint32_t> parent;
     std::vector<uint32_t> coarse2dfs, coarse2bfs;
+    ugp::CoarseTables ctab;
     ugp::UVec<uint32_t> node_pair;
     bool wide_descent = false;
     HostFlat *coarse = nullptr;
@@ -984,6 +1020,11 @@
     hf.coarse2dfs.resize(keep.size());
     for (size_t k = 0; k < keep.size(); k++) hf.coarse2dfs[k] = ex.dfsidx[keep[k]];
     hf.coarse2bfs = keep;
+    {
+        const auto &cf = hf.coarse->f;
+        ugp::build_coarse_tables(keep.size(), parent.data(), mut_off.data(), pos.data(), ref.data(), nuc.data(), cf.dfs2bfs.data(), cf.pos2site.data(), cf.max_pos,
+                                 cf.n_sites, hf.ctab);
+    }
     return UGP_OK;
 }
 
@@ -1090,6 +1131,12 @@
             m->n_coarse_bins = (uint32_t)bin.size();
         }
         if ((e = m->d_coarse2bfs.upload(hf.coarse2bfs)) != hipSuccess) return bail(e, "upload coarse table");
+        if (hf.ctab.usable() && hf.ctab.n_nodes == hf.coarse->f.n_nodes) {
+            if ((e = m->d_cs_node.upload(hf.ctab.node)) != hipSuccess || (e = m->d_cs_rmq.upload(hf.ctab.rmq)) != hipSuccess ||
+                (e = m->d_cs_site_off.upload(hf.ctab.site_off)) != hipSuccess || (e = m->d_cs_events.upload(hf.ctab.events)) != hipSuccess)
+                return bail(e, "upload coarse table");
+            m->cs_nodes = hf.ctab.n_nodes; m->cs_max_per_pos = hf.ctab.max_per_pos;
+        }
         if (!hf.node_pair.empty()) {
             m->wide_descent = getenv("UGP_DESCENT_LANES") ? atoi(getenv("UGP_DESCENT_LANES")) > 16 : hf.wide_descent;
         }
@@ -1187,6 +1234,8 @@
     io.vec(f.stream_t); io.vec(f.chunk_t_off); io.vec(f.rank_dfs); io.vec(f.node_pos8); io.vec(f.hdr8_of_bfs); io.vec(f.rec_of_bfs); io.vec(f.post_of_bfs);
     io.vec(f.b3_group_off); io.vec(f.b3_events);
     io.vec(hf.parent); io.vec(hf.coarse2dfs); io.vec(hf.coarse2bfs); io.vec(hf.node_pair); io.pod(hf.wide_descent);
+    io.pod(hf.ctab.n_nodes); io.pod(hf.ctab.max_per_pos);
+    io.vec(hf.ctab.node); io.vec(hf.ctab.rmq); io.vec(hf.ctab.site_off); io.vec(hf.ctab.events);
 }
 }
 extern "C" {
@@ -1240,6 +1289,8 @@
                 return fail(UGP_ERR_INVALID, "inconsistent flattening file (array sizes)");
             for (int32_t v : g.pos2site) if (v >= (int64_t)g.n_sites) return fail(UGP_ERR_INVALID, "inconsistent flattening file (site index out of range)");
         }
+        if (hf.ctab.n_nodes && (!hf.coarse || !ugp::coarse_tables_consistent(hf.ctab, hf.coarse->f.n_nodes, hf.coarse->f.n_sites)))
+            return fail(UGP_ERR_INVALID, "inconsistent flattening file (coarse tables)");
         return upload_flat(hf, device, out);
     } catch (const std::bad_alloc &) { return fail(UGP_ERR_NOMEM, "out of host memory"); }
 }
@@ -1964,6 +2015,7 @@
         HIP_TRY(ugp::launch_mask_words(d_mask, t == m ? nullptr : m->d_coarse2bfs.p, (uint32_t)t->flat.n_nodes, U.d_hdr8.p, U.d_rec_pos.p, U.d_post.p,
                                        t->d_stream8.p, t->d_stream.p, t->d_stream_t.p, ugp::H_NOSCORE, set, nullptr));
     }
+    m->mask_in_force = set;
     return UGP_OK;
 }
 }
@@ -2498,6 +2550,41 @@
     return UGP_OK;
 }
 
+int ugp_debug_coarse_pass(ugp_mat *m, ugp_qset *qs, int method, int32_t *cost, uint32_t *coarse_node, uint32_t *kept_bfs, uint64_t kept_cap, uint64_t *n_kept) {
+    if (!m || !qs || !n_kept || (qs->n_queries && (!cost || !coarse_node))) return fail(UGP_ERR_INVALID, "null argument");
+    if (!m->coarse) return fail(UGP_ERR_UNSUPPORTED, "this handle has no coarse tree");
+    if (method != 0 && method != 1) return fail(UGP_ERR_INVALID, "method must be 0 (walked) or 1 (sparse)");
+    HIP_TRY(hipSetDevice(m->device));
+    *n_kept = m->upd.coarse2bfs.size();
+    if (kept_bfs) {
+        if (kept_cap < *n_kept) return fail(UGP_ERR_INVALID, "buffer too small");
+        std::copy(m->upd.coarse2bfs.begin(), m->upd.coarse2bfs.end(), kept_bfs);
+    }
+    if (!qs->n_queries) return UGP_OK;
+    if (int rc = drain(m)) return rc;
+    HIP_TRY(hipDeviceSynchronize());
+    PlaceReq r;
+    const ugp::PlanTree tree = plan_tree(m);
+    ugp::PlanCall call = plan_call_facts(m, qs, r);
+    call.Q = std::max<uint64_t>(call.Q, 513);
+    const ugp::CallPlan cp = ugp::plan_call(tree, m->knobs, call);
+    ugp_mat::Work &W = m->work[0];
+    HIP_TRY(W.d_coarse_res.reserve(qs->n_queries));
+    if (method == 1) {
+        if (!cp.coarse_sparse) return fail(UGP_ERR_UNSUPPORTED, "the plan does not take the sparse pre-pass for this batch");
+        if (int rc = coarse_sparse(m, qs, cp.coarse_cap, W.d_coarse_res.p, nullptr)) return rc;
+    } else {
+        if (int rc = coarse_walked(m, qs, W.d_coarse_res.p, nullptr, 0)) return rc;
+    }
+    HIP_TRY(hipDeviceSynchronize());
+    std::vector<ugp_result> res(qs->n_queries);
+    HIP_TRY(hipMemcpy(res.data(), W.d_coarse_res.p, res.size() * sizeof(ugp_result), hipMemcpyDeviceToHost));
+    for (size_t i = 0; i < res.size(); i++) { cost[i] = res[i].best_set_difference; coarse_node[i] = res[i].best_j; }
+    return UGP_OK;
+}
+
+int ugp_debug_last_prepass(const ugp_mat *m) { return m ? m->last_prepass : 0; }
+
 int ugp_get_timing_sum(ugp_mat *m, ugp_timing *sum, uint32_t *n_calls) {
     if (!m || !sum || !n_calls) return fail(UGP_ERR_INVALID, "null argument");
     HIP_TRY(hipSetDevice(m->device));
diff --git a/usher_amd/csrc/ugp_coarse.hip b/usher_amd/csrc/ugp_coarse.hip
--- /dev/null
+++ b/usher_amd/csrc/ugp_coarse.hip
@@ -0,0 +1,120 @@
+#include <hip/hip_runtime.h>
+
+#include "ugp_coarse.hpp"
+#include "ugp_kernels.hpp"
+
+namespace ugp {
+
+namespace {
+constexpr int CS_LANES = 16;
+constexpr int CS_GROUPS = 64 / CS_LANES;
+
+__device__ __forceinline__ uint32_t group_min(uint32_t v) {
+#pragma unroll
+    for (int m = CS_LANES / 2; m >= 1; m >>= 1) v = min(v, (uint32_t)__shfl_xor((int)v, m, CS_LANES));
+    return v;
+}
+__device__ __forceinline__ int group_sum(int v) {
+#pragma unroll
+    for (int m = CS_LANES / 2; m >= 1; m >>= 1) v += __shfl_xor(v, m, CS_LANES);
+    return v;
+}
+}
+
+__global__ void __launch_bounds__(64) k_coarse_sparse(CoarseSparseArgs a) {
+    extern __shared__ __attribute__((aligned(16))) uint32_t cs_lds[];
+    __shared__ uint32_t cs_count[CS_GROUPS];
+    const uint32_t lane = threadIdx.x, g = lane / CS_LANES, gl = lane % CS_LANES;
+    uint32_t *rec = cs_lds + (size_t)g * a.cap;
+    int16_t *pre = (int16_t *)(cs_lds + (size_t)CS_GROUPS * a.cap) + (size_t)g * a.cap;
+    const uint32_t q = blockIdx.x * CS_GROUPS + g;
+    const bool live = q < a.n_queries;
+    if (gl == 0) cs_count[g] = 0;
+    __syncthreads();
+
+    const bool no_rows = a.n_ent == 0 || !a.ent_off || (a.err && *a.err != ~0ull);
+    const uint64_t rb = (live && !no_rows) ? a.ent_off[q] : 0, re = (live && !no_rows) ? min((uint64_t)a.ent_off[q + 1], a.n_ent) : rb;
+    int mism = 0;
+    for (uint64_t r = rb + gl; r < re; r += CS_LANES) {
+        const int32_t p = a.pos[r];
+        const uint32_t miss = a.is_missing[r], S = miss ? 15u : (uint32_t)a.nuc[r];
+        if (!miss && (S & a.ref[r]) == 0) mism++;
+        const int32_t site = (p >= 0 && (uint32_t)p <= a.max_pos) ? a.pos2site[p] : -1;
+        if (site < 0) continue;
+        const uint32_t e0 = a.site_off[site], e1 = a.site_off[site + 1];
+        if (e0 == e1) continue;
+        uint32_t at = atomicAdd(&cs_count[g], 2u * (e1 - e0));
+        for (uint32_t e = e0; e < e1; e++, at += 2) {
+            const uint2 ev = a.events[e];
+            uint32_t s, en;
+            coarse_boundaries(ev.x, ev.y, S, s, en);
+            if (at + 2 <= a.cap) { rec[at] = s; rec[at + 1] = en; }
+        }
+    }
+    const int d_bottom = group_sum(mism);
+    __syncthreads();
+    const uint32_t n = min(cs_count[g], a.cap);
+
+    uint32_t n_max = max(n, (uint32_t)__shfl_xor((int)n, 16));
+    n_max = max(n_max, (uint32_t)__shfl_xor((int)n_max, 32));
+    uint32_t np = 2;
+    while (np < n_max) np <<= 1;
+    for (uint32_t i = n + gl; i < np; i += CS_LANES) rec[i] = 0xFFFFFFFFu;
+    __syncthreads();
+    for (uint32_t k = 2; k <= np; k <<= 1)
+        for (uint32_t j = k >> 1; j >= 1; j >>= 1) {
+            for (uint32_t t = gl; t < np / 2; t += CS_LANES) {
+                const uint32_t i = ((t & ~(j - 1)) << 1) | (t & (j - 1)), l = i | j;
+                const uint32_t x = rec[i], y = rec[l];
+                if ((x > y) == ((i & k) == 0)) { rec[i] = y; rec[l] = x; }
+            }
+            __syncthreads();
+        }
+
+    {
+        const uint32_t per = max(np / CS_LANES, 1u), b = gl * per, e = min(b + per, n);
+        int sum = 0;
+        for (uint32_t i = b; i < e; i++) sum += coarse_rec_shift(rec[i]);
+        int run = sum;
+#pragma unroll
+        for (int d = 1; d < CS_LANES; d <<= 1) { const int v = __shfl_up(run, d, CS_LANES); if ((int)gl >= d) run += v; }
+        run -= sum;
+        for (uint32_t i = b; i < e; i++) { run += coarse_rec_shift(rec[i]); pre[i] = (int16_t)run; }
+    }
+    __syncthreads();
+
+    uint32_t best = kCoarseNoKey;
+    for (uint32_t i = gl; i <= n; i += CS_LANES) {
+        const uint32_t r0 = i ? rec[i - 1] : 0u, r1 = i < n ? rec[i] : 0u;
+        const uint32_t lo = i ? coarse_rec_pos(r0) + (coarse_rec_is_start(r0) ? 1u : 0u) : 0u;
+        const uint32_t hi = i < n ? coarse_rec_pos(r1) : a.n_nodes;
+        const int before = i ? (int)pre[i - 1] : 0;
+        best = min(best, coarse_range_candidate(a.rmq, a.n_nodes, lo, min(hi, a.n_nodes), before + d_bottom));
+        if (i < n && coarse_rec_is_start(r1) && (i == 0 || (r0 >> kCoarseKeyShift) != (r1 >> kCoarseKeyShift))) {
+            int sum_shift = 0, sum_dneg = 0, sum_dcom = 0;
+            for (uint32_t k = i; k < n; k++) {
+                const uint32_t rk = rec[k];
+                if ((rk >> kCoarseKeyShift) != (r1 >> kCoarseKeyShift)) break;
+                sum_shift += coarse_rec_shift(rk); sum_dneg += coarse_rec_dneg(rk); sum_dcom += coarse_rec_dcom(rk);
+            }
+            const uint32_t d = min(coarse_rec_pos(r1), a.n_nodes - 1);
+            const uint2 nd = a.node[d];
+            best = min(best, coarse_node_candidate(nd.x, nd.y, d, coarse_rec_root(r1), d_bottom, before, sum_shift, sum_dneg, sum_dcom));
+        }
+    }
+
+    best = group_min(best);
+    if (live && gl == 0) a.out[q] = ugp_result{(int32_t)(best >> 16), 1u, a.dfs2bfs[min(best & 0xFFFFu, a.n_nodes - 1)], 0u};
+}
+
+size_t coarse_sparse_lds_bytes(uint32_t cap) { return (size_t)CS_GROUPS * cap * 6; }
+
+hipError_t launch_coarse_sparse(const CoarseSparseArgs &a, hipStream_t s) {
+    if (!a.n_queries) return hipSuccess;
+    if (a.cap < 2 || (a.cap & (a.cap - 1)) || a.cap > 2 * kCoarseSparseMaxEvents || !a.n_nodes || a.n_nodes > kCoarseSparseMaxNodes) return hipErrorInvalidValue;
+    if (2 * a.max_rows * a.max_per_pos > a.cap) return hipErrorInvalidValue;
+    hipLaunchKernelGGL(k_coarse_sparse, dim3((a.n_queries + CS_GROUPS - 1) / CS_GROUPS), dim3(64), coarse_sparse_lds_bytes(a.cap), s, a);
+    return hipGetLastError();
+}
+
+}
diff --git a/usher_amd/csrc/ugp_coarse.hpp b/usher_amd/csrc/ugp_coarse.hpp
--- /dev/null
+++ b/usher_amd/csrc/ugp_coarse.hpp
@@ -0,0 +1,200 @@
+#pragma once
+#include <stdint.h>
+
+#include <algorithm>
+#include <vector>
+
+#if defined(__HIPCC__)
+#define UGP_COARSE_HD __host__ __device__ __forceinline__
+#else
+#define UGP_COARSE_HD inline
+#endif
+
+namespace ugp {
+
+constexpr uint32_t kCoarseSparseMaxNodes = 65536;
+constexpr uint32_t kCoarseSparseMaxEvents = 512;
+constexpr uint32_t kCoarseNoKey = 0xFFFFFFFFu;
+
+UGP_COARSE_HD uint32_t coarse_event_w0(uint32_t d, uint32_t last) { return d | (last << 16); }
+UGP_COARSE_HD uint32_t coarse_event_w1(uint32_t mut, uint32_t prev, uint32_t ref, bool after_mask, bool root) {
+    return (mut & 15u) | ((prev & 15u) << 4) | ((ref & 15u) << 8) | (after_mask ? 1u << 12 : 0u) | (root ? 1u << 13 : 0u);
+}
+constexpr uint32_t kCoarseKeyShift = 14;
+UGP_COARSE_HD void coarse_boundaries(uint32_t w0, uint32_t w1, uint32_t S , uint32_t &start, uint32_t &end) {
+    const uint32_t mut = w1 & 15u, prev = (w1 >> 4) & 15u, ref = (w1 >> 8) & 15u;
+    const int c = (S & mut) ? 1 : 0, pr = (S & prev) ? 1 : 0, c_ref = (ref & mut) ? 1 : 0, pr_ref = (ref & prev) ? 1 : 0;
+    const int delta = pr - c, delta_ref = pr_ref - c_ref, shift = delta - delta_ref;
+    const bool counted = !((w1 >> 12) & 1u);
+    const int dneg = counted ? (delta < 0 ? delta : 0) - (delta_ref < 0 ? delta_ref : 0) : 0, dcom = counted ? c - c_ref : 0;
+    const uint32_t d = w0 & 0xFFFFu, last = w0 >> 16;
+    start = ((d * 2u + 1u) << kCoarseKeyShift) | (uint32_t)(shift + 2) | ((uint32_t)(dneg + 1) << 3) | ((uint32_t)(dcom + 1) << 5) | (((w1 >> 13) & 1u) << 7);
+    end = (((last + 1u) * 2u) << kCoarseKeyShift) | (uint32_t)(2 - shift);
+}
+UGP_COARSE_HD uint32_t coarse_rec_pos(uint32_t r) { return r >> (kCoarseKeyShift + 1); }
+UGP_COARSE_HD bool coarse_rec_is_start(uint32_t r) { return (r >> kCoarseKeyShift) & 1u; }
+UGP_COARSE_HD int coarse_rec_shift(uint32_t r) { return (int)(r & 7u) - 2; }
+UGP_COARSE_HD int coarse_rec_dneg(uint32_t r) { return (int)((r >> 3) & 3u) - 1; }
+UGP_COARSE_HD int coarse_rec_dcom(uint32_t r) { return (int)((r >> 5) & 3u) - 1; }
+UGP_COARSE_HD bool coarse_rec_root(uint32_t r) { return (r >> 7) & 1u; }
+
+UGP_COARSE_HD uint32_t coarse_range_candidate(const uint32_t *rmq, uint32_t n_nodes, uint32_t lo, uint32_t hi, int add) {
+    if (lo >= hi) return kCoarseNoKey;
+    const uint32_t k = 31u - (uint32_t)__builtin_clz(hi - lo);
+    const uint32_t a = rmq[(size_t)k * n_nodes + lo], b = rmq[(size_t)k * n_nodes + hi - (1u << k)];
+    const uint32_t m = a < b ? a : b;
+    if (m == kCoarseNoKey) return kCoarseNoKey;
+    return ((uint32_t)((int)(m >> 16) + add) << 16) | (m & 0xFFFFu);
+}
+UGP_COARSE_HD uint32_t coarse_node_candidate(uint32_t n0, uint32_t n1, uint32_t d, bool root, int d_bottom, int shift_before, int sum_shift, int sum_dneg, int sum_dcom) {
+    const int base = (int)(n0 & 0xFFFFu), common_ref = (int)(n0 >> 16), neg_abs = (int)(n1 & 0x7FFFu);
+    if (root) return ((uint32_t)(d_bottom + base + sum_shift) << 16) | d;
+    if (common_ref + sum_dcom <= 0) return kCoarseNoKey;
+    return ((uint32_t)(d_bottom + base + shift_before - neg_abs + sum_dneg) << 16) | d;
+}
+
+inline uint32_t coarse_levels(uint32_t n_nodes) { uint32_t l = 1; while ((2ull << (l - 1)) <= n_nodes) l++; return l; }
+
+struct CoarseTables {
+    uint32_t n_nodes = 0;
+    uint32_t max_per_pos = 0;
+    std::vector<uint32_t> node;
+    std::vector<uint32_t> rmq;
+    std::vector<uint32_t> site_off;
+    std::vector<uint32_t> events;
+    bool usable() const { return n_nodes != 0; }
+    void clear() { *this = CoarseTables(); }
+};
+
+inline bool coarse_tables_consistent(const CoarseTables &t, uint64_t n_nodes, uint64_t n_sites) {
+    if (!t.n_nodes) return t.node.empty() && t.rmq.empty() && t.site_off.empty() && t.events.empty();
+    if (t.n_nodes != n_nodes || t.n_nodes > kCoarseSparseMaxNodes) return false;
+    if (t.node.size() != (size_t)t.n_nodes * 2 || t.rmq.size() != (size_t)coarse_levels(t.n_nodes) * t.n_nodes || t.site_off.size() != n_sites + 1 || (t.events.size() & 1)) return false;
+    if (t.site_off[0] != 0 || t.site_off[n_sites] != t.events.size() / 2) return false;
+    for (uint64_t s = 0; s < n_sites; s++)
+        if (t.site_off[s + 1] < t.site_off[s] || t.site_off[s + 1] - t.site_off[s] > t.max_per_pos) return false;
+    for (size_t e = 0; e < t.events.size(); e += 2) {
+        const uint32_t d = t.events[e] & 0xFFFFu, last = t.events[e] >> 16;
+        if (d >= t.n_nodes || last >= t.n_nodes || last < d) return false;
+    }
+    for (uint32_t v : t.rmq) if (v != kCoarseNoKey && (v & 0xFFFFu) >= t.n_nodes) return false;
+    return true;
+}
+
+inline void build_coarse_tables(uint64_t n_nodes, const uint32_t *parent, const uint64_t *mut_off, const int32_t *mut_pos, const uint8_t *mut_ref, const uint8_t *mut_nuc,
+                                const uint32_t *dfs2bfs, const int32_t *pos2site, uint64_t max_pos, uint64_t n_sites, CoarseTables &t) {
+    t.clear();
+    if (n_nodes == 0 || n_nodes > kCoarseSparseMaxNodes) return;
+    const uint32_t N = (uint32_t)n_nodes;
+    std::vector<uint32_t> d_of(N), last(N), pd(N, 0);
+    std::vector<uint8_t> has_child(N, 0);
+    for (uint32_t d = 0; d < N; d++) d_of[dfs2bfs[d]] = d;
+    for (uint32_t d = 0; d < N; d++) last[d] = d;
+    for (uint32_t d = N - 1; d >= 1; d--) {
+        pd[d] = d_of[parent[dfs2bfs[d]]];
+        if (pd[d] >= d) return;
+        last[pd[d]] = std::max(last[pd[d]], last[d]);
+        has_child[pd[d]] = 1;
+    }
+    struct Ev { uint32_t site, w0, w1; };
+    std::vector<Ev> evs;
+    std::vector<uint8_t> state(n_sites, 0);
+    struct Undo { uint32_t site; uint8_t old; };
+    std::vector<Undo> undo;
+    std::vector<uint32_t> open_d, open_undo;
+    std::vector<int32_t> dref(N, 0);
+    std::vector<uint32_t> key(N);
+    t.node.assign((size_t)N * 2, 0);
+    for (uint32_t d = 0; d < N; d++) {
+        while (!open_d.empty() && d > last[open_d.back()]) {
+            for (size_t u = undo.size(); u > open_undo.back(); u--) state[undo[u - 1].site] = undo[u - 1].old;
+            undo.resize(open_undo.back());
+            open_d.pop_back(); open_undo.pop_back();
+        }
+        open_d.push_back(d); open_undo.push_back((uint32_t)undo.size());
+        const uint32_t j = dfs2bfs[d];
+        const int d_par = d ? dref[pd[d]] : 0;
+        int tsum = 0, neg = 0, common = 0;
+        bool masked = false;
+        for (uint64_t i = mut_off[j]; i < mut_off[j + 1]; i++) {
+            const int32_t p = mut_pos[i];
+            if (p < 0) { masked = true; continue; }
+            if ((uint64_t)p > max_pos || pos2site[p] < 0 || (uint64_t)pos2site[p] >= n_sites) { t.clear(); return; }
+            const uint32_t site = (uint32_t)pos2site[p];
+            const uint8_t nuc = mut_nuc[i], ref = mut_ref[i];
+            if (nuc == 0 || (nuc & (nuc - 1)) || nuc > 8 || ref == 0 || (ref & (ref - 1)) || ref > 8) { t.clear(); return; }
+            const uint8_t prev = state[site] ? state[site] : ref;
+            const int c = (ref & nuc) ? 1 : 0, pr = (ref & prev) ? 1 : 0, delta = pr - c;
+            tsum += delta;
+            if (!masked) { common += c; neg += std::min(delta, 0); }
+            evs.push_back({site, coarse_event_w0(d, last[d]), coarse_event_w1(nuc, prev, ref, masked, d == 0)});
+            undo.push_back({site, state[site]});
+            state[site] = nuc;
+        }
+        dref[d] = d_par + tsum;
+        const bool elig = d == 0 || common > 0 || (has_child[d] && mut_off[j + 1] == mut_off[j]);
+        const int base = d ? d_par : dref[d], cost = d ? d_par + neg : dref[d];
+        if (base < 0 || base > 0xFFFF || common > 0xFFFF || -neg > 0x7FFF || cost < 0 || cost > 0xFFFE) { t.clear(); return; }
+        t.node[(size_t)d * 2] = (uint32_t)base | ((uint32_t)common << 16);
+        t.node[(size_t)d * 2 + 1] = (uint32_t)(-neg);
+        key[d] = elig ? ((uint32_t)cost << 16) | d : kCoarseNoKey;
+    }
+    t.site_off.assign(n_sites + 1, 0);
+    for (const Ev &e : evs) t.site_off[e.site + 1]++;
+    for (uint64_t s = 0; s < n_sites; s++) { t.max_per_pos = std::max(t.max_per_pos, t.site_off[s + 1]); t.site_off[s + 1] += t.site_off[s]; }
+    t.events.resize(evs.size() * 2);
+    {
+        std::vector<uint32_t> at(t.site_off.begin(), t.site_off.end() - 1);
+        for (const Ev &e : evs) { const uint32_t k = at[e.site]++; t.events[(size_t)k * 2] = e.w0; t.events[(size_t)k * 2 + 1] = e.w1; }
+    }
+    const uint32_t levels = coarse_levels(N);
+    t.rmq.resize((size_t)levels * N);
+    std::copy(key.begin(), key.end(), t.rmq.begin());
+    for (uint32_t k = 1; k < levels; k++) {
+        const uint32_t half = 1u << (k - 1);
+        const uint32_t *below = &t.rmq[(size_t)(k - 1) * N];
+        uint32_t *lvl = &t.rmq[(size_t)k * N];
+        for (uint32_t i = 0; i < N; i++) lvl[i] = std::min(below[i], below[std::min(i + half, N - 1)]);
+    }
+    t.n_nodes = N;
+}
+
+inline uint32_t coarse_sparse_host(const CoarseTables &t, const int32_t *pos2site, uint64_t max_pos, uint64_t n_rows, const int32_t *pos, const uint8_t *ref,
+                                   const uint8_t *nuc, const uint8_t *is_missing) {
+    int d_bottom = 0;
+    std::vector<uint32_t> rec;
+    for (uint64_t r = 0; r < n_rows; r++) {
+        const uint32_t S = is_missing[r] ? 15u : nuc[r];
+        if (!is_missing[r] && (nuc[r] & ref[r]) == 0) d_bottom++;
+        const int32_t p = pos[r];
+        const int32_t site = (p >= 0 && (uint64_t)p <= max_pos) ? pos2site[p] : -1;
+        if (site < 0) continue;
+        for (uint32_t e = t.site_off[site]; e < t.site_off[site + 1]; e++) {
+            uint32_t s, en;
+            coarse_boundaries(t.events[(size_t)e * 2], t.events[(size_t)e * 2 + 1], S, s, en);
+            rec.push_back(s); rec.push_back(en);
+        }
+    }
+    std::sort(rec.begin(), rec.end());
+    const uint32_t n = (uint32_t)rec.size();
+    std::vector<int> pre(n);
+    for (uint32_t i = 0, run = 0; i < n; i++) { run += (uint32_t)coarse_rec_shift(rec[i]); pre[i] = (int)run; }
+    uint32_t best = kCoarseNoKey;
+    for (uint32_t i = 0; i <= n; i++) {
+        const uint32_t lo = i ? coarse_rec_pos(rec[i - 1]) + (coarse_rec_is_start(rec[i - 1]) ? 1u : 0u) : 0u;
+        const uint32_t hi = i < n ? coarse_rec_pos(rec[i]) : t.n_nodes;
+        const int before = i ? pre[i - 1] : 0;
+        best = std::min(best, coarse_range_candidate(t.rmq.data(), t.n_nodes, lo, hi, before + d_bottom));
+        if (i < n && coarse_rec_is_start(rec[i]) && (i == 0 || (rec[i - 1] >> kCoarseKeyShift) != (rec[i] >> kCoarseKeyShift))) {
+            int sum_shift = 0, sum_dneg = 0, sum_dcom = 0;
+            for (uint32_t k = i; k < n && (rec[k] >> kCoarseKeyShift) == (rec[i] >> kCoarseKeyShift); k++) {
+                sum_shift += coarse_rec_shift(rec[k]); sum_dneg += coarse_rec_dneg(rec[k]); sum_dcom += coarse_rec_dcom(rec[k]);
+            }
+            const uint32_t d = coarse_rec_pos(rec[i]);
+            best = std::min(best, coarse_node_candidate(t.node[(size_t)d * 2], t.node[(size_t)d * 2 + 1], d, coarse_rec_root(rec[i]), d_bottom, before, sum_shift, sum_dneg, sum_dcom));
+        }
+    }
+    return best;
+}
+
+}
diff --git a/usher_amd/csrc/ugp_flatten.hpp b/usher_amd/csrc/ugp_flatten.hpp
--- a/usher_amd/csrc/ugp_flatten.hpp
+++ b/usher_amd/csrc/ugp_flatten.hpp
@@ -39,7 +39,7 @@
 constexpr uint32_t B3_GROUP_SHIFT = 8, B3_GROUP_BLOCKS = 1u << B3_GROUP_SHIFT;
 inline uint32_t b3_blocks(uint64_t stream8_words) { return (uint32_t)((((stream8_words + B3_BLOCK_WORDS - 1) >> B3_BLOCK_SHIFT) + 1u + B3_GROUP_BLOCKS - 1u) & ~(uint64_t)(B3_GROUP_BLOCKS - 1u)); }
 constexpr uint32_t MAX_SITES = 1u << 22;
-constexpr uint32_t FLAT_FORMAT_VERSION = 6;
+constexpr uint32_t FLAT_FORMAT_VERSION = 7;
 constexpr uint32_t MAX_NODE_MUTS = 65534;
 
 struct Options {
diff --git a/usher_amd/csrc/ugp_kernels.hpp b/usher_amd/csrc/ugp_kernels.hpp
--- a/usher_amd/csrc/ugp_kernels.hpp
+++ b/usher_amd/csrc/ugp_kernels.hpp
@@ -87,6 +87,20 @@
 hipError_t launch_coarse_result(const uint32_t *lbest, const uint32_t *lpos, const uint32_t *list, const uint32_t *list_n, uint32_t n_chunks, uint32_t n_tiles512,
                                 uint32_t n_queries, const uint32_t *chunk_node_off, const uint32_t *chunk8_body_off, const uint32_t *node_pos8,
                                 const uint32_t *dfs2bfs, ugp_result *out, hipStream_t s);
+struct CoarseSparseArgs {
+    const uint64_t *ent_off; const int32_t *pos; const uint8_t *ref, *nuc, *is_missing;
+    const unsigned long long *err;
+    const int32_t *pos2site;
+    uint32_t max_pos, n_nodes, n_queries;
+    uint64_t n_ent, max_rows;
+    uint32_t max_per_pos;
+    uint32_t cap;
+    const uint32_t *site_off; const uint2 *events; const uint2 *node; const uint32_t *rmq;
+    const uint32_t *dfs2bfs;
+    ugp_result *out;
+};
+size_t coarse_sparse_lds_bytes(uint32_t cap);
+hipError_t launch_coarse_sparse(const CoarseSparseArgs &a, hipStream_t s);
 hipError_t launch_phase2_packed(const Best8Args &b1, const uint32_t *list, const uint32_t *list_n, uint32_t *gbest_part, uint32_t *gbest, uint32_t n_tiles512,
                                 void *units, uint32_t *info, uint32_t *cnt, uint32_t *key, const uint32_t *node_pos8, const uint32_t *rank_dfs,
                                 const uint32_t *chunk_node_off, const uint32_t *rank2bfs, uint32_t n_queries, ugp_result *out, const uint32_t *order,
diff --git a/usher_amd/csrc/ugp_plan.hpp b/usher_amd/csrc/ugp_plan.hpp
--- a/usher_amd/csrc/ugp_plan.hpp
+++ b/usher_amd/csrc/ugp_plan.hpp
@@ -3,6 +3,7 @@
 
 #include <algorithm>
 
+#include "ugp_coarse.hpp"
 #include "ugp_flatten.hpp"
 #include "ugp_knobs.hpp"
 #include "ugp_tuner.hpp"
@@ -18,6 +19,10 @@
     bool coarse = false;
     bool b3_events = false;
     bool wide_descent = false;
+    uint64_t coarse_nodes = 0;
+    uint32_t coarse_max_per_pos = 0;
+    bool coarse_excluded = false;
+    bool coarse_masked = false;
 };
 struct PlanEx {
     bool given = false, packed = false, mask = false, skip = false, skip_chunk = false, scores = false;
@@ -36,6 +41,8 @@
 struct CallPlan {
     uint32_t n_sites = 1, active_words = 1, useful_words = 1;
     bool ex_packable = false, ex_skip = false, packed_ok = false, sorted = false, can_fork = false, fill_ahead = false;
+    bool coarse_sparse = false;
+    uint32_t coarse_cap = 0;
     uint64_t sub_tiles = kMaxTilesPerLaunch;
 };
 
@@ -48,6 +55,10 @@
     p.ex_skip = p.ex_packable && c.ex.skip;
     p.packed_ok = (c.mode == 0) && (!c.ex.given || p.ex_packable) && !K.force_v1 && !t.mask_not_first && (c.max_rows + t.max_path_muts + 2 < 0x7F7Full);
     p.sorted = p.packed_ok && t.coarse && c.Q > 512 && !K.no_sort && !K.no_prune;
+    p.coarse_sparse = p.sorted && (!c.ex.given || (c.ex.packed && !c.ex.mask && !c.ex.scores)) && !K.coarse_phase2 && t.coarse_nodes != 0 &&
+                      t.coarse_nodes <= kCoarseSparseMaxNodes && !t.coarse_excluded && !t.coarse_masked &&
+                      c.max_rows * (uint64_t)t.coarse_max_per_pos <= kCoarseSparseMaxEvents;
+    if (p.coarse_sparse) for (p.coarse_cap = 32; p.coarse_cap < 2 * c.max_rows * (uint64_t)t.coarse_max_per_pos; p.coarse_cap *= 2) {}
     p.can_fork = p.sorted && !c.coarse_only && !K.no_fork && !c.sharing;
     p.fill_ahead = p.can_fork && !(c.nmask && p.n_sites) && K.tile_build <= 0 && t.n_sites && std::min<uint64_t>(c.Q, (uint64_t)kMaxTilesPerLaunch * 64) == c.Q;
     if (t.n_chunks) p.sub_tiles = std::min<uint64_t>(p.sub_tiles, std::max<uint64_t>(8, ((K.lbest_gib ? (uint64_t)K.lbest_gib : 24ull) << 30) / ((uint64_t)t.n_chunks * 128) & ~7ull));
diff --git a/usher_amd/placement.py b/usher_amd/placement.py
--- a/usher_amd/placement.py
+++ b/usher_amd/placement.py
@@ -543,6 +543,16 @@
     def free_qset(self, h) -> None:
         self._L.ugp_qset_destroy(h)
 
+    def coarse_pass(self, qset, method: str):
+        Q = int(self._L.ugp_qset_size(qset))
+        cost = np.zeros(Q, np.int32); node = np.zeros(Q, np.uint32); kept = np.zeros(self.n_nodes, np.uint32)
+        n = C.c_uint64()
+        self._ck(self._L.ugp_debug_coarse_pass(self._h, qset, {"walked": 0, "sparse": 1}[method], _ptr(cost), _ptr(node), _ptr(kept), len(kept), C.byref(n)))
+        return cost, node, kept[:int(n.value)].copy()
+
+    def last_prepass(self) -> str:
+        return ("none", "walked", "sparse")[int(self._L.ugp_debug_last_prepass(self._h))]
+
     def place_device(self, qset, d_out_ptr: int, stream: int = 0) -> None:
         self._ck(self._L.ugp_place_device(self._h, qset, C.c_void_p(d_out_ptr), C.c_void_p(stream)))
 
```
